# yang-0201/MAF-YOLO

Hardware: AMD Instinct MI355X
Metric: images/sec MAF-YOLO-n 640x640 bs=32 infer (Model.forward + non_max_suppression) (higher is better)
Workload: dtype f16

## Files before the change

include/mafyolo_hip.h:

```cpp
#ifndef MAFYOLO_HIP_H
#define MAFYOLO_HIP_H

#include <stdint.h>

#ifdef __cplusplus
extern "C" {
#endif

typedef void* maf_stream_t;

enum { MAF_F16 = 0, MAF_F32 = 1, MAF_U8 = 2 };
enum { MAF_ACT_NONE = 0, MAF_ACT_RELU = 1, MAF_ACT_SILU = 2, MAF_ACT_SIGMOID = 3 };
enum { MAF_SRC_DIRECT = 0,
       MAF_SRC_UP2 = 1,
       MAF_SRC_POOL2 = 2,
       MAF_SRC_SUB2 = 3,
       MAF_SRC_PAIRS = 4 };
enum { MAF_OP_STEM = 0,
       MAF_OP_CONV1X1 = 1,
       MAF_OP_CONV3X3S2 = 2,
       MAF_OP_DWCONV = 3,
       MAF_OP_SPPF_POOL = 4,
       MAF_OP_DECODE = 5,
       MAF_OP_BOTTLENECK = 6,
       MAF_OP_CONV1DW = 7,
       MAF_OP_HEADTAIL = 8,
       MAF_OP_STEM2 = 9,
       MAF_OP_CONV3X3S2_DGRAD = 10 };
enum { MAF_CONV_GENERIC = 1,
       MAF_CONV_LDS = 2,
       MAF_CONV_STREAM = 3,
       MAF_CONV_SPLITK = 4,
       MAF_CONV_STREAM_LDS = 5,
       MAF_CONV3_LDS = 6,
       MAF_CONV3_WREG = 7,
       MAF_CONV_DMA = 8 };
enum { MAF_DW_MFMA = -1, MAF_DW_DOT2 = -2, MAF_DW_PAIRS = -4 };
enum { MAF_DW_P2_STAGED = 128 };
#define MAF_DW_TILE_ROWS(tile_k) ((tile_k) >> 8)
enum { MAF_E_ARG = -1, MAF_E_UNSUPPORTED = -2, MAF_E_HIP = -3 };

typedef struct {
    const void* ptr;
    int32_t C;
    int32_t stride;
    int32_t coff;
    int32_t mode;
} maf_src_t;

typedef struct {
    int32_t kind, dtype, in_dtype, act;
    int32_t B, H, W;
    int32_t Hin, Win;
    int32_t Cin, Cout, ksize;
    int32_t nsrc;
    maf_src_t src[4];
    void* out;
    int32_t out_stride, out_coff;
    int32_t out_f32;
    int32_t tile_p, tile_c;
    int32_t tile_k;
    const void* w;
    const float* bias;
    const void* reg[3];
    int32_t lvl_h[3], lvl_w[3];
    int32_t reg_stride, nc, reg_max;
    float lvl_stride[3];
    const void* aux[4];
    int32_t lane;
    int32_t n_wait;
    int32_t wait[8];
    int32_t out_pairs;
    int32_t reserved0;
} maf_op_t;

const char* maf_last_error(void);
int maf_version(void);
int maf_op_size(void);
int64_t maf_bottleneck_record_bytes(int32_t k, int32_t Cin, int32_t Cout);
int64_t maf_bottleneck_tail_record_bytes(int32_t c, int32_t nsrc, int32_t C3);
int maf_bottleneck_tail_supported(int32_t k, int32_t c, int32_t nsrc, int32_t C3);
int64_t maf_conv1dw_record_bytes(int32_t k, int32_t Cin);
int64_t maf_head_tail_record_bytes(int32_t C);
int64_t maf_stem2_record_bytes(int32_t C0, int32_t C1, int32_t C3);
int64_t maf_conv3s2_lds_record_bytes(int32_t Cin, int32_t Cout);
int64_t maf_mprep_lds_record_bytes(int32_t Cin, int32_t Cout, int32_t C1);
int64_t maf_mprep_wreg_record_bytes(int32_t Cin, int32_t Cout, int32_t C1);
int64_t maf_conv3s2_wreg_record_bytes(int32_t Cin, int32_t Cout);
int maf_conv1x1_stats_supported(int32_t ksteps, int32_t tile_c);

int maf_op_launch(const maf_op_t* op, maf_stream_t stream);

typedef struct maf_engine maf_engine_t;
int maf_engine_create(const maf_op_t* ops, int32_t n_ops, maf_engine_t** out);
int maf_engine_num_ops(const maf_engine_t* e);
int maf_engine_run(maf_engine_t* e, const void* image, void* pred, maf_stream_t stream);
int maf_engine_run_filtered(maf_engine_t* e, const void* image, void* pred, maf_stream_t stream, void* nms_workspace, double conf_thres);
int maf_engine_run_graph(maf_engine_t* e, const void* image, void* pred, maf_stream_t stream);
int maf_engine_run_timed(maf_engine_t* e, const void* image, void* pred, maf_stream_t stream, float* ms_per_op);
void maf_engine_destroy(maf_engine_t* e);

enum { MAF_NMS_FLOAT_THRESHOLD = 1, MAF_NMS_SINGLE_LAUNCH = 2, MAF_NMS_PRECOLLECTED = 4, MAF_NMS_MATRIX = 8 };
enum { MAF_NMS_CNT_STRIDE = 64 };
int64_t maf_nms_workspace_bytes(int32_t B, int32_t N, int32_t nc);
int maf_nms(const float* pred, int32_t B, int32_t N, int32_t nc, double conf_thres, double iou_thres,
            const int32_t* classes, int32_t n_classes, int32_t agnostic, int32_t multi_label,
            int32_t max_det, void* workspace, int64_t workspace_bytes,
            float* out_rows, int64_t* out_idx, int32_t* out_count, maf_stream_t stream);
int maf_nms_ex(const float* pred, int32_t B, int32_t N, int32_t nc, double conf_thres, double iou_thres,
               const int32_t* classes, int32_t n_classes, int32_t agnostic, int32_t multi_label,
               int32_t max_det, void* workspace, int64_t workspace_bytes,
               float* out_rows, int64_t* out_idx, int32_t* out_count, int32_t flags, maf_stream_t stream);

int64_t maf_pack_w1x1_bytes(int32_t Cout, int32_t Cin, int32_t transpose, int32_t dtype, int32_t tile_c);
int maf_pack_w1x1(const float* w, int32_t Cout, int32_t Cin, int32_t transpose, int32_t dtype, int32_t tile_c, void* out, maf_stream_t stream);
int maf_pack_dw(const float* w, int32_t C, int32_t k, int32_t flip, int32_t dtype, void* out, maf_stream_t stream);
int maf_tal_targets(const float* targets, int32_t T, int32_t B, float img_size, float* gts, int32_t* gt_image, int32_t* offsets, maf_stream_t stream);
int maf_tal_assign(const void* pd_scores, int32_t score_dtype, const float* pd_bboxes, const float* anchor_points, const float* gts,
                   const int32_t* gt_image, const int32_t* offsets, int32_t T, int32_t B, int32_t A, int32_t nc, int32_t topk,
                   float alpha, float beta, float eps, int32_t n_levels, const int32_t* level_hw, const float* level_stride, float cell_offset,
                   int32_t* cand_scratch, int32_t* out_gt, float* out_norm, maf_stream_t stream);
int maf_atss_assign(const float* pd_bboxes, const float* anchor_points, const float* gts, const int32_t* gt_image, const int32_t* offsets,
                    int32_t T, int32_t B, int32_t A, int32_t topk, int32_t n_levels, const int32_t* level_hw, const float* level_stride,
                    float cell_offset, float cell_size, int32_t* cand_scratch, int32_t* out_gt, float* out_norm, maf_stream_t stream);
int64_t maf_loss_partial_rows(int32_t B, int32_t A, int32_t nc);
int maf_loss_decode(const void* pred_distri, int32_t dtype, const float* anchor_points, const float* anchor_strides, int32_t B, int32_t A,
                    int32_t reg_max, float* out_boxes, maf_stream_t stream);
int maf_loss_terms(const void* pred_scores, const void* pred_distri, int32_t dtype, const float* anchor_points, const float* anchor_strides,
                   const float* gts, const int32_t* assigned_gt, const float* norm, int32_t B, int32_t A, int32_t nc, int32_t reg_max,
                   float w_cls, float w_iou, float w_dfl, float* partials, float* out, const float* upstream, void* grad_scores,
                   void* grad_distri, maf_stream_t stream);

int maf_bn_forward(const void* x, int32_t x_stride, int32_t M, int32_t C, int32_t dtype, const float* gamma, const float* beta,
                   float eps, float momentum, float* running_mean, float* running_var, int64_t* num_batches_tracked, int32_t act, void* y,
                   int32_t y_stride, float* save_mean, float* save_rstd, float* part, int32_t R, int32_t phase, const void* residual, int32_t res_stride,
                   maf_stream_t stream);
int maf_bn_backward(const void* x, int32_t x_stride, const void* dz, int32_t dz_stride, int32_t M, int32_t C, int32_t dtype,
                    const float* gamma, const float* beta, const float* save_mean, const float* save_rstd, int32_t act,
                    void* dx, int32_t dx_stride, float* dgamma, float* dbeta, float* part, int32_t R, int32_t phase,
                    const void* residual, int32_t res_stride, void* dres, int32_t dres_stride, maf_stream_t stream);
int maf_dw_branches_stats(const void* const* src, const int32_t* src_stride, void* const* dst, const int32_t* dst_stride, const void* const* w,
                          int32_t nb, int32_t k0, int32_t B, int32_t H, int32_t W, int32_t C, int32_t dtype, float* const* stats, int32_t replicas, maf_stream_t stream);
int maf_dw_branches(const void* const* src, const int32_t* src_stride, void* const* dst, const int32_t* dst_stride, const void* const* w,
                    int32_t nb, int32_t k0, int32_t B, int32_t H, int32_t W, int32_t C, int32_t dtype, int32_t dgrad, maf_stream_t stream);
int maf_bn_forward_ex(const void* x, int32_t x_stride, int32_t M, int32_t C, int32_t dtype, const float* gamma, const float* beta,
                      float eps, float momentum, float* running_mean, float* running_var, int64_t* num_batches_tracked, int32_t act, void* y,
                      int32_t y_stride, float* save_mean, float* save_rstd, float* part, int32_t R, int32_t phase, const void* residual, int32_t res_stride,
                      int32_t stats_ready, maf_stream_t stream);
int32_t maf_bn_replicas(int32_t C, int32_t R);
int maf_bn_stats(const void* x, int32_t x_stride, int32_t M, int32_t C, int32_t dtype, float* part, int32_t R, int32_t phase, maf_stream_t stream);
int maf_bn_sum_forward(const void* const* z, const int32_t* z_stride, int32_t nb, int32_t M, int32_t C, int32_t dtype,
                       const float* const* gamma, const float* const* beta, float eps, float momentum,
                       float* const* running_mean, float* const* running_var, int64_t* const* num_batches_tracked,
                       void* out, int32_t out_stride, float* const* save_mean, float* const* save_rstd,
                       float* const* part, int32_t R, const int32_t* phase, int32_t act, maf_stream_t stream);
int maf_bn_sum_forward_stats(const void* const* z, const int32_t* z_stride, int32_t nb, int32_t M, int32_t C, int32_t dtype,
                             const float* const* gamma, const float* const* beta, float eps, float momentum,
                             float* const* running_mean, float* const* running_var, int64_t* const* num_batches_tracked,
                             void* out, int32_t out_stride, float* const* save_mean, float* const* save_rstd,
                             float* const* part, int32_t R, const int32_t* phase, int32_t act,
                             float* next_part, int32_t next_R, int32_t next_phase, maf_stream_t stream);
int maf_bn_sum_backward(const void* dy, int32_t dy_stride, const void* const* z, const int32_t* z_stride, int32_t nb, int32_t M, int32_t C, int32_t dtype,
                        const float* const* gamma, const float* const* beta, const float* const* save_mean, const float* const* save_rstd,
                        void* const* dz, const int32_t* dz_stride, float* const* dgamma, float* const* dbeta, int32_t accumulate_affine,
                        float* bpart, int32_t R, int32_t phase, int32_t act, maf_stream_t stream);
int maf_bn_backward_acc(const void* x, int32_t x_stride, const void* dz, int32_t dz_stride, int32_t M, int32_t C, int32_t dtype,
                        const float* gamma, const float* beta, const float* save_mean, const float* save_rstd, int32_t act,
                        void* dx, int32_t dx_stride, float* dgamma, float* dbeta, float* part, int32_t R, int32_t phase,
                        const void* residual, int32_t res_stride, void* dres, int32_t dres_stride, int32_t accumulate_affine, maf_stream_t stream);
int maf_set_deterministic(int32_t on);
int maf_conv1x1_wgrad(const void* x, int32_t x_stride, const void* dy, int32_t dy_stride, int32_t M, int32_t Cin, int32_t Cout,
                      int32_t dtype, float* dw, maf_stream_t stream);
int maf_conv_wgrad(const void* x, int32_t x_stride, const void* dy, int32_t dy_stride, int32_t B, int32_t Ho, int32_t Wo, int32_t Hs, int32_t Ws,
                   int32_t Cin, int32_t Cout, int32_t ksize, int32_t stride, int32_t dtype, float* dw, maf_stream_t stream);
int maf_dw_wgrad(const void* x, int32_t x_stride, const void* dy, int32_t dy_stride, int32_t B, int32_t H, int32_t W, int32_t C,
                 int32_t k, int32_t dtype, float* dw, int32_t replicas, maf_stream_t stream);
int maf_stem_train(const void* img, int32_t img_stride, int32_t B, int32_t Hin, int32_t Win, const float* w3, const float* w1, int32_t Cout,
                   void* z3, void* z1, maf_stream_t stream);
int maf_image_to_nhwc8(const void* x, int32_t dtype, int32_t B, int32_t H, int32_t W, void* out, maf_stream_t stream);
int maf_dw_wgrad31(const void* x, int32_t x_stride, const void* dya, int32_t dya_stride, const void* dyb, int32_t dyb_stride, const void* dy1, int32_t dy1_stride,
                   int32_t B, int32_t H, int32_t W, int32_t C, int32_t dtype, float* dwa, float* dwb, float* dw1, int32_t replicas, maf_stream_t stream);

int maf_grad_fold(const float* src, int32_t taps, int32_t Cout_p, int32_t Cin_p, float* dst, int32_t Cout, int32_t Cin, int32_t accumulate,
                  maf_stream_t stream);
int maf_add_sub2(const void* src, int32_t src_stride, void* dst, int32_t dst_stride, int32_t B, int32_t Ho, int32_t Wo, int32_t C, int32_t dtype, maf_stream_t stream);
int maf_colsum(const void* x, int32_t x_stride, int64_t M, int32_t C, int32_t dtype, float* out, maf_stream_t stream);

int maf_zero(void* p, int64_t bytes, maf_stream_t stream);

int maf_maxpool_forward(const void* x, int32_t x_stride, int32_t B, int32_t H, int32_t W, int32_t C, int32_t k, int32_t stride, int32_t pad,
                        int32_t dtype, void* y, int32_t y_stride, uint8_t* idx, maf_stream_t stream);
int maf_maxpool_backward(const void* dy, int32_t dy_stride, const uint8_t* idx, int32_t B, int32_t H, int32_t W, int32_t C, int32_t k,
                         int32_t stride, int32_t pad, int32_t dtype, void* dx, int32_t dx_stride, maf_stream_t stream);
int maf_upsample2x_forward(const void* x, int32_t x_stride, int32_t B, int32_t H, int32_t W, int32_t C, int32_t dtype, void* y, int32_t y_stride, maf_stream_t stream);
int maf_upsample2x_backward(const void* dy, int32_t dy_stride, int32_t B, int32_t H, int32_t W, int32_t C, int32_t dtype, void* dx, int32_t dx_stride, maf_stream_t stream);

typedef struct maf_pack_desc {
    const void* src; void* dst;
    int64_t total;
    int32_t kind, dtype;
    int32_t Cout, Cin, taps, transpose;
    int32_t CT, steps, Kp, flip;
    int32_t block0, reserved;
} maf_pack_desc_t;
int maf_pack_batch(const maf_pack_desc_t* descs_dev, int32_t n, int32_t nblocks, maf_stream_t stream);
int32_t maf_pack_desc_size(void);

typedef struct maf_ema_desc {
    void* dst; const void* src;
    int64_t total;
    int32_t block0, reserved;
} maf_ema_desc_t;
int maf_ema_update(const maf_ema_desc_t* descs_dev, int32_t n, int32_t nblocks, float decay, float one_minus_decay, maf_stream_t stream);
int32_t maf_ema_desc_size(void);

#define MAF_SGD_MAX_GROUPS 8
typedef struct maf_sgd_desc {
    void* param; void* grad; void* buf;
    int64_t total;
    int32_t block0, group;
} maf_sgd_desc_t;
int maf_sgd_update(const maf_sgd_desc_t* descs_dev, int32_t n, int32_t nblocks, int32_t ngroups, const double* lr, const double* weight_decay, const double* momentum,
                   const int32_t* nesterov, const float* found_inf, const float* grad_scale, maf_stream_t stream);
int32_t maf_sgd_desc_size(void);

typedef struct maf_range_desc {
    const void* ptr;
    int64_t total;
    int32_t block0, reserved;
} maf_range_desc_t;
int maf_nonfinite_check(const maf_range_desc_t* descs_dev, int32_t n, int32_t nblocks, float* found_inf, maf_stream_t stream);
int32_t maf_range_desc_size(void);


int maf_nhwc_sum(const void* const* src, const int32_t* src_stride, int32_t n, void* dst, int32_t dst_stride, int64_t M, int32_t C, int32_t dtype,
                 int32_t accumulate, maf_stream_t stream);
int maf_detect_join(const void* const* cls, const int32_t* cls_stride, const void* const* reg, const int32_t* reg_stride, const int32_t* level_pixels,
                    int32_t n_levels, int32_t B, int32_t nc, int32_t nreg, int32_t dtype, void* cls_out, void* reg_out, maf_stream_t stream);
int maf_detect_join_backward(const void* d_cls, const void* d_reg, const void* cls_out, const int32_t* level_pixels, int32_t n_levels, int32_t B, int32_t nc,
                             int32_t nreg, int32_t dtype, void* const* dcls, const int32_t* dcls_stride, void* const* dreg, const int32_t* dreg_stride,
                             int32_t nc_pad, int32_t nreg_pad, maf_stream_t stream);
int maf_stream_fork(maf_stream_t main, maf_stream_t side);
int maf_stream_join(maf_stream_t main, maf_stream_t side);

int maf_stream_create_masked(const uint32_t* mask_words, int32_t n_words, maf_stream_t* out);
int maf_stream_destroy(maf_stream_t s);

#define MAF_TAPE_MAX_ARGS 28
#define MAF_TAPE_FORK (-1)
typedef struct maf_tape_rec {
    int32_t fn, stream;
    uint64_t a[MAF_TAPE_MAX_ARGS];
} maf_tape_rec_t;
typedef struct maf_tape_toggle {
    void* addr; uint64_t mask; int32_t width, reserved;
} maf_tape_toggle_t;
int32_t maf_tape_fn_id(const char* name);
int32_t maf_tape_fn_nargs(int32_t fn);
int32_t maf_tape_rec_size(void);
int maf_tape_run(const maf_tape_rec_t* recs, int32_t first, int32_t last, const maf_stream_t* streams, int32_t n_streams, int32_t* failed_at);
int maf_tape_toggle(const maf_tape_toggle_t* t, int32_t n);

int maf_coco_rows(const float* rows, const int32_t* count, int32_t B, int32_t max_det, const float* img_params,
                  const int32_t* ids, int32_t n_ids, float* out, int32_t* out_total, maf_stream_t stream);

#define MAF_LETTERBOX_KARG_MAX 64
typedef struct {
    const uint8_t* ptr; int64_t pitch;
    int32_t h, w;
    int32_t new_h, new_w, top, left;
} maf_letterbox_image_t;
int64_t maf_letterbox_lds_bytes(const maf_letterbox_image_t* imgs, int32_t B, int32_t W);
int maf_letterbox(const maf_letterbox_image_t* imgs, const maf_letterbox_image_t* imgs_dev, int32_t B, int32_t H, int32_t W,
                  const uint8_t* color, int32_t bgr, uint8_t* out, maf_stream_t stream);

int maf_rescale_boxes(float* rows, const int32_t* count, int32_t B, int32_t max_det, int32_t row_stride, const float* params,
                      int32_t do_round, maf_stream_t stream);

typedef struct {
    const uint8_t* src; int64_t src_pitch;
    int32_t h, w;
    uint8_t* dst;
    int32_t new_h, new_w;
} maf_augment_frame_t;
int maf_augment_resize(const maf_augment_frame_t* frames, const maf_augment_frame_t* frames_dev, int32_t n, maf_stream_t stream);

#define MAF_AUGMENT_MAX_TILES 4
typedef struct {
    const uint8_t* ptr; int64_t pitch;
    int32_t h, w;
    int32_t x0, y0, x1, y1;
    int32_t dx, dy;
} maf_augment_tile_t;
typedef struct {
    double minv[2][6];
    double r;
    int32_t ntiles[2];
    int32_t hsv, flipud, fliplr, reserved;
    maf_augment_tile_t tile[2][MAF_AUGMENT_MAX_TILES];
    uint8_t lut[3][256];
} maf_augment_sample_t;
int32_t maf_augment_sample_size(void);
int maf_mosaic_affine(const maf_augment_sample_t* samples, const maf_augment_sample_t* samples_dev, int32_t B, int32_t S, uint8_t* out,
                      maf_stream_t stream);

#define MAF_AREA_FAST2 0
#define MAF_AREA_FASTN 1
#define MAF_AREA_GENERAL 2
typedef struct {
    const uint8_t* src; int64_t src_pitch;
    int32_t h, w;
    uint8_t* dst;
    int32_t new_h, new_w;
    int32_t path;
    int32_t iscale_x, iscale_y;
    float inv_area;
    int32_t x_start, x_pairs;
    int32_t y_start, y_pairs;
} maf_area_frame_t;
int maf_area_struct_sizes(int32_t* frame_size);
int maf_resize_area(const maf_area_frame_t* frames, const maf_area_frame_t* frames_dev, int32_t n, const void* tables, const void* tables_dev,
                    int64_t table_words, maf_stream_t stream);

#define MAF_PR_MAX_DET 1024
#define MAF_PR_MAX_LABELS 1024
#define MAF_PR_MAX_CLASSES 1024
#define MAF_PR_HEADER 16
#define MAF_PR_LABELS_XYXY 1
#define MAF_PR_CONFUSION 2
#define MAF_PR_ERR_CLASS 1
#define MAF_PR_ERR_LABELS 2
#define MAF_PR_ERR_CAPACITY 4
int64_t maf_pr_state_ints(int32_t nc);
int64_t maf_pr_out_doubles(int32_t nc, int32_t niou);
int64_t maf_pr_workspace_bytes(int32_t nc, int32_t niou, int64_t capacity);
int maf_pr_match(const float* rows, const int32_t* count, int32_t B, int32_t max_det, const float* targets, int32_t n_targets,
                 const float* img_params, int32_t H, int32_t W, const float* iouv, int32_t niou, int32_t nc, int32_t flags,
                 float cm_conf, float cm_iou, const int64_t* offs_in, int64_t* offs_out, int64_t* keys, uint16_t* masks,
                 int64_t capacity, int32_t* state, maf_stream_t stream);
int maf_pr_curves(const int64_t* sorted_keys, const int64_t* perm, const uint16_t* masks, int64_t capacity, const int32_t* state,
                  int32_t nc, int32_t niou, void* workspace, int64_t workspace_bytes, double* out, maf_stream_t stream);

#define MAF_COCO_T 10
#define MAF_COCO_R 101
#define MAF_COCO_A 4
#define MAF_COCO_M 3
#define MAF_COCO_MAX_DETS 100
#define MAF_COCO_MAX_GT 256
#define MAF_COCO_GT_CROWD 1
#define MAF_COCO_GT_IDNZ 2
int maf_coco_append(const float* packed, const int32_t* total, int64_t rows, const int32_t* img_index, int32_t B, const int32_t* cat_lut,
                    int32_t n_lut, int32_t* det_img, int32_t* det_cat, double* det_box, double* det_score, maf_stream_t stream);
int maf_coco_match(const double* gt_box, const double* gt_area, const uint8_t* gt_flags, const int64_t* gt_off, const int64_t* cell_keys,
                   const int64_t* order, const double* det_box, int64_t n, const uint8_t* img_sel, const int32_t* cat_map, int32_t I, int32_t K,
                   const double* iou_thrs, const double* area_rng, int32_t* rank, uint64_t* mbits, uint64_t* ibits, int32_t* npig,
                   maf_stream_t stream);
int maf_coco_accumulate(const int64_t* cat_keys, const int32_t* rank, const uint64_t* mbits, const uint64_t* ibits, const double* score, int64_t n,
                        const int32_t* npig, const uint8_t* img_sel, const int32_t* cat_of, int32_t I, int32_t K, int32_t Kp,
                        const double* rec_thrs, const int32_t* max_dets, double* precision, double* recall, double* scores, maf_stream_t stream);

#define MAF_JPEG_GROUP 64
#define MAF_JPEG_SCAN_PAD 64
#define MAF_JPEG_HUFF_TABLE_BYTES 1424
#define MAF_JPEG_ST_BAD_CODE 1
#define MAF_JPEG_ST_BAD_INDEX 2
#define MAF_JPEG_ST_SHORT_SCAN 4
#define MAF_JPEG_ST_REFINE_PAST_SE 8
#define MAF_JPEG_STAGE_ENTROPY 1
#define MAF_JPEG_STAGE_IDCT 2
#define MAF_JPEG_STAGE_COLOR 4
#define MAF_JPEG_STAGE_ALL 7
typedef struct {
    int32_t n_images, n_lanes, n_tabsets;
    int32_t group;
    int64_t images_off, lanes_off, huff_off, quant_off, scan_off;
    int64_t scan_bytes;
    int64_t total_bytes;
    int64_t coef_elems, plane_bytes, out_bytes;
    int32_t n_scans, n_slanes, n_rounds;
    int32_t sgroup;
    int64_t scans_off, slanes_off, rounds_off;
} maf_jpeg_header_t;
typedef struct {
    int64_t coef_off;
    int64_t plane_off;
    int64_t out_off;
    int32_t w, h, ncomp;
    int32_t hs, vs;
    int32_t mcux, mcuy;
    int32_t quant;
    int32_t dc_tab[3], ac_tab[3];
    int32_t reserved[2];
} maf_jpeg_image_t;
typedef struct {
    int64_t begin, end;
    int32_t image;
    int32_t first_mcu, n_mcu;
    int32_t tabset;
} maf_jpeg_lane_t;
typedef struct {
    int32_t image;
    int32_t round;
    int32_t ncomp;
    int32_t comp[3];
    int32_t ss, se, ah, al;
    int32_t dc_tab[3];
    int32_t ac_tab;
    int32_t bw, bh;
} maf_jpeg_scan_t;
int maf_jpeg_struct_sizes(int32_t* header_image_lane);
int maf_jpeg_progressive_struct_sizes(int32_t* scan);
int maf_jpeg_decode(const void* blob_host, const void* blob_dev, int16_t* coef, uint8_t* planes, uint8_t* out, int32_t* status,
                    int32_t stages, maf_stream_t stream);

int maf_nms_debug(uint64_t* host8);

int maf_timer_create(void** timer);
int maf_timer_start(void* timer, maf_stream_t stream);
int maf_timer_stop(void* timer, maf_stream_t stream);
int maf_timer_elapsed_ms(void* timer, float* ms);
void maf_timer_destroy(void* timer);

#ifdef __cplusplus
}
#endif
#endif
```

maf-yolo_amd/config.py:

```python
import os

SWITCHES = {
    "dw_stage":          ("MAF_DW_STAGE", True, "tuner: offer dwconv_p2's staged-store form (tile_k + 128) as a candidate"),
    "fuse_mprep":        ("MAF_FUSE_MPREP", True, "MPRep's two branches as one launch where the kernel exists (tuned plans)"),
    "fuse_tail":         ("MAF_FUSE_TAIL", 1, "what Model.fuse_tail = 'auto' means: 0 off, 1 blocks of one bottleneck (default), 3 every instantiation (s / m opt-in)"),
    "split_cat":         ("MAF_SPLIT_CAT", True, "RepHDW behind the fused stem: one dense tensor per concat slot"),
    "mprep_wreg_min":    ("MAF_MPREP_WREG_MIN", 65536, "output pixels from which MPRep takes the register-weight 3x3 kernel"),
    "head_tail_256_max": ("MAF_HEAD_TAIL_256_MAX", 16384, "largest level (B * H * W pixels) whose 256-channel head runs as the fused tail (weights streamed through LDS per 16-pixel unit)"),
    "nms_single_max_batch": ("MAF_NMS_SINGLE_MAX_BATCH", 0, "largest batch the single-launch NMS kernel serves (0: never — the seven-launch path is faster, DESIGN.md 8)"),
    "nms_matrix":        ("MAF_NMS_MATRIX", "auto", "all-pairs NMS: 1 = suppression matrix + row scan, 0 = kept-list scan, auto = kept-list under other work (async), matrix alone up to 32 images"),
    "step_tape":         ("MAF_STEP_TAPE", True, "replay the recorded launch lists of a train step (tape.py) once a batch shape has been seen three times"),
    "stage_native":      ("MAF_STAGE_NATIVE", True, "step tape: the image batch into the static NHWC8 input by one native pass"),
    "train_lanes":       ("MAF_TRAIN_LANES", 2, "lanes (extra streams) a recorded step may put independent branches on"),
    "wgrad_stream":      ("MAF_WGRAD_STREAM", True, "weight gradients on a side stream"),
    "bn_affine_direct":  ("MAF_BN_AFFINE_DIRECT", True, "BatchNorm dgamma / dbeta straight into the exchange's bucket slices"),
    "conv_bn_stats":     ("MAF_CONV_BN_STATS", True, "BatchNorm statistics out of the 1x1 conv's epilogue"),
    "train_tune":        ("MAF_TRAIN_TUNE", True, "time the conv tile variants per shape on first use"),
    "train_tune3":       ("MAF_TRAIN_TUNE3", True, "... the 3x3 stride-2 launches too"),
    "stem_train":        ("MAF_STEM_TRAIN", True, "the image's two RepVGG convs as one direct-conv launch"),
    "dw_wgrad31":        ("MAF_DW_WGRAD31", True, "the 3x3 (+3x3) + 1x1 depth-wise branches' weight gradients as one launch"),
    "dw_branches":       ("MAF_DW_BRANCHES", True, "one launch per direction for the branches of a DilatedReparamBlock"),
    "dw_branch_stats":   ("MAF_DW_BRANCH_STATS", True, "the branches' BatchNorm statistics out of the depth-wise kernel's epilogue"),
    "cat_free":          ("MAF_CAT_FREE", True, "concat nodes without a copy (producers store into their slot)"),
    "bn_sum":            ("MAF_BN_SUM", True, "the branch BatchNorms of a DilatedReparamBlock as one apply pass per direction"),
    "bn_sum_stats":      ("MAF_BN_SUM_STATS", True, "that pass accumulates the statistics of the BatchNorm behind it"),
    "ema_native":        ("MAF_EMA_NATIVE", True, "ModelEMA.update as one launch"),
    "sgd_native":        ("MAF_SGD_NATIVE", True, "the SGD step as one launch"),
    "inf_check_native":  ("MAF_INF_CHECK_NATIVE", True, "GradScaler's inf check as one launch"),
    "exchange_debug":    ("MAF_EXCHANGE_DEBUG", False, "GradExchange keeps the Python stack of every gradient arrival"),
    "hip_lib":           ("MAF_HIP_LIB", "", "path of another build of libmafyolo_hip.so (make prof / ko / var); empty: the in-tree product library"),
}


LIBRARY_SWEEP_HOOKS = {
    "MAF_WGRAD_GX / MAF_WGRAD_R / MAF_WGRAD_TAP_PER_WG": "csrc/wgrad.hip: grid width / replica count / one tap per workgroup of the conv weight gradient (tools/wgrad_sweep.py)",
    "MAF_WGRAD3_GX / MAF_WGRAD3_R / MAF_WGRAD3_PATCH": "csrc/wgrad.hip: the same for the 3x3 patch kernel",
    "MAF_DWWG / MAF_DWWG31 / MAF_DWWG_MFMA / MAF_DWMF_WG": "csrc/train_ops.hip, dw_wgrad_mfma.hip: tiles of the depth-wise weight gradients (tools/dw_wgrad_sweep.py, dw_wgrad31_sweep.py, dw_wgrad_ab.py)",
    "MAF_DWB_TILE / MAF_DWB_TILE_DGRAD": "csrc/dw_branches.hip: tile of the merged depth-wise branches (tools/dwb_sweep.py)",
    "MAF_DGRAD3_ALL_TAPS": "csrc/conv_mfma.hip: A/B of the 3x3 data gradient's tap split",
}


class Config:
    def __init__(self, environ=None):
        environ = os.environ if environ is None else environ
        for attr, (env, default, _) in SWITCHES.items():
            raw = environ.get(env)
            if raw is None:
                val = default
            elif isinstance(default, bool):
                val = raw != "0"
            elif isinstance(default, int):
                val = int(raw)
            else:
                val = raw
            setattr(self, attr, val)

    def overridden(self):
        return {a: getattr(self, a) for a, (_, d, _m) in SWITCHES.items() if getattr(self, a) != d}

    def table(self):
        rows = ["%-22s %-26s %-10s %s" % ("attribute", "environment", "value", "meaning")]
        for a, (env, d, meaning) in SWITCHES.items():
            v = getattr(self, a)
            rows.append("%-22s %-26s %-10s %s%s" % (a, env, repr(v), meaning, "" if v == d else "   [default %r]" % (d,)))
        return "\n".join(rows)


cfg = Config()

if __name__ == "__main__":
    print(cfg.table())
```

maf-yolo_amd/csrc/capi.hip:

```cpp
#include <vector>
#include <string>
#include "maf_common.h"

static thread_local std::string g_err;

void maf_set_error(const std::string& msg) { g_err = msg; }

int maf_check_hip(hipError_t e, const char* what) {
    if (e == hipSuccess) return 0;
    g_err = std::string(what) + ": " + hipGetErrorString(e);
    return MAF_E_HIP;
}

extern "C" const char* maf_last_error(void) { return g_err.c_str(); }
extern "C" int maf_zero(void* p, int64_t bytes, maf_stream_t stream) {
    MAF_REQUIRE(p && bytes >= 0, "maf_zero: bad arguments");
    return maf_check_hip(hipMemsetAsync(p, 0, (size_t)bytes, static_cast<hipStream_t>(stream)), "maf_zero");
}

extern "C" int maf_version(void) { return 200; }
extern "C" int maf_op_size(void) { return (int)sizeof(maf_op_t); }

extern "C" int maf_op_launch(const maf_op_t* op, maf_stream_t stream) {
    if (!op) { maf_set_error("maf_op_launch: null op"); return MAF_E_ARG; }
    hipStream_t s = static_cast<hipStream_t>(stream);
    switch (op->kind) {
        case MAF_OP_STEM: return maf_launch_stem(op, s);
        case MAF_OP_CONV1X1:
        case MAF_OP_CONV3X3S2:
        case MAF_OP_CONV3X3S2_DGRAD: return maf_launch_conv_mfma(op, s);
        case MAF_OP_DWCONV: return maf_launch_dwconv(op, s);
        case MAF_OP_SPPF_POOL: return maf_launch_sppf_pool(op, s);
        case MAF_OP_DECODE: return maf_launch_decode(op, s);
        case MAF_OP_BOTTLENECK: return maf_launch_bottleneck(op, s);
        case MAF_OP_CONV1DW: return maf_launch_conv1dw(op, s);
        case MAF_OP_HEADTAIL: return maf_launch_head_tail(op, s);
        case MAF_OP_STEM2: return maf_launch_stem2(op, s);
        default: maf_set_error("maf_op_launch: unknown op kind"); return MAF_E_UNSUPPORTED;
    }
}

constexpr int kMaxLanes = 8;

struct maf_engine {
    std::vector<maf_op_t> ops;
    hipGraph_t graph = nullptr;
    hipGraphExec_t exec = nullptr;
    const void* g_image = nullptr;
    void* g_pred = nullptr;
    int n_lanes = 1;
    hipStream_t side[kMaxLanes] = {};
    std::vector<hipEvent_t> done;
    std::vector<char> signal;
    hipEvent_t fork = nullptr, join[kMaxLanes] = {};
    bool lanes_ready = false;
};

static int engine_prepare_lanes(maf_engine* e) {
    if (e->lanes_ready) return 0;
    const size_t n = e->ops.size();
    e->signal.assign(n, 0);
    e->done.assign(n, nullptr);
    e->n_lanes = 1;
    for (size_t i = 0; i < n; ++i) {
        const maf_op_t& o = e->ops[i];
        if (o.lane < 0 || o.lane >= kMaxLanes) { maf_set_error("engine: op lane out of range (0..7)"); return MAF_E_ARG; }
        if (o.n_wait < 0 || o.n_wait > 8) { maf_set_error("engine: n_wait out of range (0..8)"); return MAF_E_ARG; }
        if (o.lane + 1 > e->n_lanes) e->n_lanes = o.lane + 1;
        for (int k = 0; k < o.n_wait; ++k) {
            if (o.wait[k] < 0 || (size_t)o.wait[k] >= i) { maf_set_error("engine: an op may only wait for earlier ops"); return MAF_E_ARG; }
            e->signal[o.wait[k]] = 1;
        }
    }
    int rc = 0;
    for (int l = 1; l < e->n_lanes && !rc; ++l) {
        rc = maf_check_hip(hipStreamCreateWithFlags(&e->side[l], hipStreamNonBlocking), "hipStreamCreate");
        if (!rc) rc = maf_check_hip(hipEventCreateWithFlags(&e->join[l], hipEventDisableTiming), "hipEventCreate");
    }
    if (!rc && e->n_lanes > 1) rc = maf_check_hip(hipEventCreateWithFlags(&e->fork, hipEventDisableTiming), "hipEventCreate");
    for (size_t i = 0; i < n && !rc; ++i)
        if (e->signal[i]) rc = maf_check_hip(hipEventCreateWithFlags(&e->done[i], hipEventDisableTiming), "hipEventCreate");
    if (!rc) e->lanes_ready = true;
    return rc;
}

extern "C" int maf_engine_create(const maf_op_t* ops, int32_t n_ops, maf_engine_t** out) {
    if (!ops || n_ops <= 0 || !out) { maf_set_error("maf_engine_create: bad arguments"); return MAF_E_ARG; }
    maf_engine* e = new maf_engine();
    e->ops.assign(ops, ops + n_ops);
    *out = e;
    return 0;
}

extern "C" int maf_engine_num_ops(const maf_engine_t* e) { return e ? (int)e->ops.size() : 0; }

static long long nms_cap_pow2(long long v) { long long p = 1; while (p < v) p <<= 1; return p; }

static int engine_launch_all(maf_engine* e, const void* image, void* pred, hipStream_t s, void* cand_ws = nullptr, float cand_conf = 0.f, bool one_stream = false) {
    int rc = engine_prepare_lanes(e);
    if (rc) return rc;
    const bool multi = e->n_lanes > 1 && !one_stream;
    int* cand_cnt = nullptr; unsigned long long* cand_keys = nullptr; long long cand_cap = 0;
    if (cand_ws) {
        int B = 0, A = 0, nc = 0, tails = 0;
        for (const maf_op_t& o : e->ops) {
            if (o.kind == MAF_OP_DECODE) { maf_set_error("maf_engine_run_filtered: a level of this plan is decoded by MAF_OP_DECODE (no fused tail)"); return MAF_E_UNSUPPORTED; }
            if (o.kind == MAF_OP_HEADTAIL) { B = o.B; A = o.Win; nc = o.nc; ++tails; }
        }
        if (!tails) { maf_set_error("maf_engine_run_filtered: the plan has no MAF_OP_HEADTAIL"); return MAF_E_UNSUPPORTED; }
        cand_cnt = static_cast<int*>(cand_ws);
        cand_keys = reinterpret_cast<unsigned long long*>(static_cast<char*>(cand_ws) + 256 + (long long)B * MAF_NMS_CNT_STRIDE * 4);
        cand_cap = nms_cap_pow2((long long)A * nc);
        rc = maf_check_hip(hipMemsetAsync(cand_cnt, 0, (size_t)B * MAF_NMS_CNT_STRIDE * 4, s), "candidate counter reset");
        if (rc) return rc;
    }
    if (multi) {
        rc = maf_check_hip(hipEventRecord(e->fork, s), "hipEventRecord(fork)");
        for (int l = 1; l < e->n_lanes && !rc; ++l) rc = maf_check_hip(hipStreamWaitEvent(e->side[l], e->fork, 0), "hipStreamWaitEvent(fork)");
        if (rc) return rc;
    }
    for (size_t i = 0; i < e->ops.size(); ++i) {
        maf_op_t op = e->ops[i];
        if ((op.kind == MAF_OP_STEM || op.kind == MAF_OP_STEM2) && image) op.src[0].ptr = image;
        if ((op.kind == MAF_OP_DECODE || op.kind == MAF_OP_HEADTAIL) && pred) op.out = pred;
        if (op.kind == MAF_OP_HEADTAIL && cand_ws) { op.aux[1] = cand_cnt; op.aux[2] = cand_keys; op.lvl_h[0] = (int32_t)cand_cap; op.lvl_stride[1] = cand_conf; }
        hipStream_t st = (op.lane == 0 || one_stream) ? s : e->side[op.lane];
        for (int k = 0; k < op.n_wait && !one_stream && !rc; ++k) rc = maf_check_hip(hipStreamWaitEvent(st, e->done[op.wait[k]], 0), "hipStreamWaitEvent");
        if (!rc) rc = maf_op_launch(&op, st);
        if (!rc && !one_stream && e->signal[i]) rc = maf_check_hip(hipEventRecord(e->done[i], st), "hipEventRecord");
        if (rc) {
            g_err = "op " + std::to_string(i) + ": " + g_err;
            return rc;
        }
    }
    if (multi) {
        for (int l = 1; l < e->n_lanes && !rc; ++l) {
            rc = maf_check_hip(hipEventRecord(e->join[l], e->side[l]), "hipEventRecord(join)");
            if (!rc) rc = maf_check_hip(hipStreamWaitEvent(s, e->join[l], 0), "hipStreamWaitEvent(join)");
        }
    }
    return rc;
}

extern "C" int maf_engine_run(maf_engine_t* e, const void* image, void* pred, maf_stream_t stream) {
    if (!e) { maf_set_error("maf_engine_run: null engine"); return MAF_E_ARG; }
    return engine_launch_all(e, image, pred, static_cast<hipStream_t>(stream));
}

extern "C" int maf_engine_run_filtered(maf_engine_t* e, const void* image, void* pred, maf_stream_t stream, void* nms_workspace, double conf_thres) {
    if (!e || !nms_workspace || !pred) { maf_set_error("maf_engine_run_filtered: null argument"); return MAF_E_ARG; }
    if (!(conf_thres >= 0.0 && conf_thres < 1.0)) { maf_set_error("maf_engine_run_filtered: conf_thres must be in [0, 1)"); return MAF_E_ARG; }
    return engine_launch_all(e, image, pred, static_cast<hipStream_t>(stream), nms_workspace, (float)conf_thres);
}

extern "C" int maf_engine_run_graph(maf_engine_t* e, const void* image, void* pred, maf_stream_t stream) {
    if (!e) { maf_set_error("maf_engine_run_graph: null engine"); return MAF_E_ARG; }
    hipStream_t s = static_cast<hipStream_t>(stream);
    if (e->exec && (e->g_image != image || e->g_pred != pred)) {
        (void)hipGraphExecDestroy(e->exec); (void)hipGraphDestroy(e->graph);
        e->exec = nullptr; e->graph = nullptr;
    }
    if (!e->exec) {
        int rc = maf_check_hip(hipStreamBeginCapture(s, hipStreamCaptureModeThreadLocal), "hipStreamBeginCapture");
        if (rc) return rc;
        rc = engine_launch_all(e, image, pred, s, nullptr, 0.f, true);
        hipError_t ce = hipStreamEndCapture(s, &e->graph);
        if (rc) return rc;
        rc = maf_check_hip(ce, "hipStreamEndCapture");
        if (rc) return rc;
        rc = maf_check_hip(hipGraphInstantiate(&e->exec, e->graph, nullptr, nullptr, 0), "hipGraphInstantiate");
        if (rc) return rc;
        e->g_image = image; e->g_pred = pred;
    }
    return maf_check_hip(hipGraphLaunch(e->exec, s), "hipGraphLaunch");
}

extern "C" int maf_engine_run_timed(maf_engine_t* e, const void* image, void* pred, maf_stream_t stream, float* ms_per_op) {
    if (!e || !ms_per_op) { maf_set_error("maf_engine_run_timed: bad arguments"); return MAF_E_ARG; }
    hipStream_t s = static_cast<hipStream_t>(stream);
    const size_t n = e->ops.size();
    std::vector<hipEvent_t> ev(n + 1);
    int rc = 0;
    for (size_t i = 0; i <= n && !rc; ++i) rc = maf_check_hip(hipEventCreate(&ev[i]), "hipEventCreate");
    if (!rc) rc = maf_check_hip(hipEventRecord(ev[0], s), "hipEventRecord");
    for (size_t i = 0; i < n && !rc; ++i) {
        maf_op_t op = e->ops[i];
        if ((op.kind == MAF_OP_STEM || op.kind == MAF_OP_STEM2) && image) op.src[0].ptr = image;
        if ((op.kind == MAF_OP_DECODE || op.kind == MAF_OP_HEADTAIL) && pred) op.out = pred;
        rc = maf_op_launch(&op, s);
        if (!rc) rc = maf_check_hip(hipEventRecord(ev[i + 1], s), "hipEventRecord");
    }
    if (!rc) rc = maf_check_hip(hipEventSynchronize(ev[n]), "hipEventSynchronize");
    for (size_t i = 0; i < n && !rc; ++i) rc = maf_check_hip(hipEventElapsedTime(&ms_per_op[i], ev[i], ev[i + 1]), "hipEventElapsedTime");
    for (size_t i = 0; i <= n; ++i) (void)hipEventDestroy(ev[i]);
    return rc;
}

extern "C" void maf_engine_destroy(maf_engine_t* e) {
    if (!e) return;
    if (e->exec) (void)hipGraphExecDestroy(e->exec);
    if (e->graph) (void)hipGraphDestroy(e->graph);
    for (int l = 1; l < kMaxLanes; ++l) {
        if (e->join[l]) (void)hipEventDestroy(e->join[l]);
        if (e->side[l]) (void)hipStreamDestroy(e->side[l]);
    }
    if (e->fork) (void)hipEventDestroy(e->fork);
    for (hipEvent_t ev : e->done) if (ev) (void)hipEventDestroy(ev);
    delete e;
}

struct maf_timer { hipEvent_t a, b; };

extern "C" int maf_timer_create(void** t) {
    if (!t) return MAF_E_ARG;
    maf_timer* m = new maf_timer();
    int rc = maf_check_hip(hipEventCreate(&m->a), "hipEventCreate");
    if (!rc) rc = maf_check_hip(hipEventCreate(&m->b), "hipEventCreate");
    if (rc) { delete m; return rc; }
    *t = m;
    return 0;
}
extern "C" int maf_timer_start(void* t, maf_stream_t s) { return maf_check_hip(hipEventRecord(static_cast<maf_timer*>(t)->a, static_cast<hipStream_t>(s)), "hipEventRecord"); }
extern "C" int maf_timer_stop(void* t, maf_stream_t s) { return maf_check_hip(hipEventRecord(static_cast<maf_timer*>(t)->b, static_cast<hipStream_t>(s)), "hipEventRecord"); }
extern "C" int maf_timer_elapsed_ms(void* t, float* ms) {
    maf_timer* m = static_cast<maf_timer*>(t);
    int rc = maf_check_hip(hipEventSynchronize(m->b), "hipEventSynchronize");
    if (rc) return rc;
    return maf_check_hip(hipEventElapsedTime(ms, m->a, m->b), "hipEventElapsedTime");
}
extern "C" void maf_timer_destroy(void* t) {
    maf_timer* m = static_cast<maf_timer*>(t);
    if (!m) return;
    (void)hipEventDestroy(m->a); (void)hipEventDestroy(m->b);
    delete m;
}

extern "C" int maf_stream_create_masked(const uint32_t* mask_words, int32_t n_words, maf_stream_t* out) {
    if (!mask_words || n_words <= 0 || !out) { maf_set_error("stream_create_masked: bad arguments"); return MAF_E_ARG; }
    hipStream_t s = nullptr;
    if (int rc = maf_check_hip(hipExtStreamCreateWithCUMask(&s, (uint32_t)n_words, mask_words), "hipExtStreamCreateWithCUMask")) return rc;
    *out = s;
    return 0;
}
extern "C" int maf_stream_destroy(maf_stream_t s) { return maf_check_hip(hipStreamDestroy(static_cast<hipStream_t>(s)), "hipStreamDestroy"); }
```

maf-yolo_amd/csrc/maf_common.h:

```cpp
#pragma once
#include <hip/hip_runtime.h>
#include <stdint.h>
#include <string>
#include "../../include/mafyolo_hip.h"

typedef _Float16 half_t;
typedef _Float16 half8_t __attribute__((ext_vector_type(8)));
typedef _Float16 half4_t __attribute__((ext_vector_type(4)));
typedef _Float16 half2_t __attribute__((ext_vector_type(2)));
typedef float f32x4_t __attribute__((ext_vector_type(4)));
typedef float f32x2_t __attribute__((ext_vector_type(2)));
typedef uint32_t u32x4_t __attribute__((ext_vector_type(4)));
typedef uint32_t u32x2_t __attribute__((ext_vector_type(2)));

void maf_set_error(const std::string& msg);
int maf_check_hip(hipError_t e, const char* what);

#define MAF_REQUIRE(cond, msg)                          \
    do {                                                \
        if (!(cond)) {                                  \
            maf_set_error(std::string(msg));            \
            return MAF_E_ARG;                           \
        }                                               \
    } while (0)

int maf_launch_conv_mfma(const maf_op_t* op, hipStream_t s);
int maf_launch_stem(const maf_op_t* op, hipStream_t s);
int maf_launch_dwconv(const maf_op_t* op, hipStream_t s);
int maf_launch_sppf_pool(const maf_op_t* op, hipStream_t s);
int maf_launch_decode(const maf_op_t* op, hipStream_t s);
int maf_launch_bottleneck(const maf_op_t* op, hipStream_t s);
int maf_launch_conv1dw(const maf_op_t* op, hipStream_t s);
int maf_launch_head_tail(const maf_op_t* op, hipStream_t s);
int maf_launch_stem2(const maf_op_t* op, hipStream_t s);
int maf_launch_conv3s2_lds(const maf_op_t* op, hipStream_t s);
int maf_launch_conv3s2_wreg(const maf_op_t* op, hipStream_t s);
int maf_dw_wgrad_mfma(const void* x, int x_stride, const void* dy, int dy_stride, int B, int H, int W, int C, int k, float* dw, int replicas, hipStream_t s);

template <int ACT>
__device__ __forceinline__ float maf_act(float x) {
    if (ACT == MAF_ACT_RELU) return x > 0.f ? x : 0.f;
    if (ACT == MAF_ACT_SILU) return x * __builtin_amdgcn_rcpf(1.f + __expf(-x));
    if (ACT == MAF_ACT_SIGMOID) return __builtin_amdgcn_rcpf(1.f + __expf(-x));
    return x;
}
__device__ __forceinline__ float maf_act_rt(float x, int act) {
    switch (act) {
        case MAF_ACT_RELU: return x > 0.f ? x : 0.f;
        case MAF_ACT_SILU: return x * __builtin_amdgcn_rcpf(1.f + __expf(-x));
        case MAF_ACT_SIGMOID: return __builtin_amdgcn_rcpf(1.f + __expf(-x));
        default: return x;
    }
}

static inline int maf_cdiv(int a, int b) { return (a + b - 1) / b; }
```

maf-yolo_amd/engine.py:

```python
import ctypes as C
import os

import torch

from .config import cfg
from . import lib, pack
from .layers import (RepVGGBlock, RepHDW, MPRep, SPPF, ConvWrapper, Head_DepthUni)

_ESIZE = {lib.F16: 2, lib.F32: 4}


from .conv_variants import stream_lds_ok
from .tuner import _TUNE_CACHE, choose_fusion, save_tune_cache, load_tune_cache, p2_wave_bytes
from . import tuner as _tuner, plan_report as _report

_TORCH_DT = {lib.F16: torch.float16, lib.F32: torch.float32}


def _raw(*ts):
    return tuple(t.detach().float().cpu() for t in ts)


class Buf:

    def __init__(self, off, H, W, stride, esize, C=None):
        self.off, self.H, self.W, self.stride, self.esize = off, H, W, stride, esize
        self.C = stride if C is None else C


class Seg:
    def __init__(self, buf, C, coff=0, mode=lib.SRC_DIRECT):
        self.buf, self.C, self.coff, self.mode = buf, C, coff, mode


class TV:

    def __init__(self, segs, H, W):
        self.segs, self.H, self.W = segs, H, W

    @property
    def C(self):
        return sum(s.C for s in self.segs)


class Plan:
    def __init__(self, model, B, Hin, Win, dtype, in_dtype, device, fuse=None, fuse_head=None, fuse_tail=None):
        assert Hin % 32 == 0 and Win % 32 == 0, "image sides must be multiples of 32 (stride of P5)"
        self.B, self.Hin, self.Win, self.dtype, self.in_dtype, self.device = B, Hin, Win, dtype, in_dtype, device
        self.es = _ESIZE[dtype]
        self._arena_size = 0
        self._wblobs = []
        self._wsize = 0
        self._ops = []
        self.nc = model.nc
        self.reg_max = model.detect.reg_max
        self.strides = [float(s) for s in model.detect.stride.tolist()]
        self.fuse = getattr(model, "fuse_bottlenecks", "auto") if fuse is None else fuse
        fh = getattr(model, "fuse_head", "auto") if fuse_head is None else fuse_head
        self.fuse_head = bool(fh) and dtype == lib.F16 and model.nc == 80 and model.detect.reg_max == 16
        fs = getattr(model, "fuse_stem", True)
        self.fuse_stem = (2 if fs is True else int(fs or 0)) if dtype == lib.F16 else 0
        self._stem2 = self._stem3 = None
        fm = getattr(model, "fuse_mprep", "auto")
        self.fuse_mprep = (bool(getattr(model, "autotune", False)) if fm == "auto" else bool(fm)) and cfg.fuse_mprep
        ft = getattr(model, "fuse_tail", "auto") if fuse_tail is None else fuse_tail
        env_ft = str(cfg.fuse_tail)
        deep = 3 if env_ft == "3" else 1
        self.fuse_tail = (deep if ft == "auto" else 3 if ft else 0) if (env_ft != "0" and dtype == lib.F16) else 0
        self.split_cat = bool(getattr(model, "split_cat", cfg.split_cat))
        self.lanes = getattr(model, "multi_stream", False)
        if isinstance(self.lanes, bool):
            self.lanes = 2 if self.lanes else 0
        with torch.no_grad():
            self._build(model)
        self._finalize()

    def _fuse_mode(self, name, k, c):
        if self.dtype != lib.F16 or c % 8:
            return 0
        f = self.fuse
        if isinstance(f, dict):
            m = f.get(name, 0)
        elif isinstance(f, (set, frozenset, list, tuple)):
            m = 1 if name in f else 0
        elif f == "auto":
            m = 1 if k <= 5 else 0
        elif f is True:
            m = 1
        else:
            m = int(f or 0)
        if m == 1 and c > 64:
            m = 2 if (f is True or isinstance(f, dict)) else 0
        if m == 2 and c > 512:
            m = 0
        return m

    def _alloc(self, H, W, C, esize=None):
        esize = esize or self.es
        off = self._arena_size
        self._arena_size += (self.B * H * W * C * esize + 255) // 256 * 256
        return Buf(off, H, W, C, esize)

    def _wput(self, t):
        t = t.contiguous()
        off = self._wsize
        self._wsize += (t.numel() * t.element_size() + 255) // 256 * 256
        self._wblobs.append((off, t))
        return off

    def _conv1x1(self, name, w, b, src, out, out_coff, act, out_f32=False):
        cout = w.shape[0]
        M = self.B * src.H * src.W
        pt, ct = pack.tile_for(cout, M)
        srcC = [s.C for s in src.segs]
        assert len(src.segs) <= 4, "%s: more than 4 concat sources" % name
        self._ops.append(dict(kind=lib.OP_CONV1X1, name=name, act=act, H=src.H, W=src.W, Cin=src.C, Cout=cout, raw=(w.detach().float().cpu(), b.detach().float().cpu(), srcC),
                              segs=src.segs, out=out, out_coff=out_coff, out_f32=int(out_f32), pt=pt, ct=ct,
                              w=self._wput(pack.pack_conv1x1(w, srcC, ct, self.dtype)), b=self._wput(pack.pack_bias(b, ct))))

    def _conv3x3s2(self, name, w, b, src, out, out_coff, act, twin=None):
        assert len(src.segs) == 1 and src.segs[0].mode == lib.SRC_DIRECT, "%s: 3x3 s2 conv needs a materialised input" % name
        cout = w.shape[0]
        H, W = src.H // 2, src.W // 2
        pt, ct = pack.tile_for(cout, self.B * H * W)
        rec = dict(kind=lib.OP_CONV3X3S2, name=name, act=act, H=H, W=W, Hin=src.H, Win=src.W, Cin=src.C, Cout=cout, raw=(w.detach().float().cpu(), b.detach().float().cpu(), None),
                   segs=src.segs, out=out, out_coff=out_coff, out_f32=0, pt=pt, ct=ct,
                   w=self._wput(pack.pack_conv3x3(w, ct, self.dtype)), b=self._wput(pack.pack_bias(b, ct)))
        if twin is not None:
            name2, w2, b2, src2, out2 = twin
            s1, s2 = src.segs[0], src2.segs[0]
            assert len(src2.segs) == 1 and s2.mode == lib.SRC_DIRECT and (s2.buf.stride, s2.coff, s2.C) == (s1.buf.stride, s1.coff, s1.C) and w2.shape == w.shape \
                and (out2.stride, out2.H, out2.W) == (out.stride, out.H, out.W) and out_coff == 0
            rec.update(name=name + "+" + name2, twin=dict(seg=s2, out=out2, raw=(w2.detach().float().cpu(), b2.detach().float().cpu()),
                                                          w=self._wput(pack.pack_conv3x3(w2, ct, self.dtype)), b=self._wput(pack.pack_bias(b2, ct))))
        self._ops.append(rec)

    def _dw(self, name, w, b, src, out, act):
        assert len(src.segs) == 1 and src.segs[0].mode == lib.SRC_DIRECT
        self._ops.append(dict(kind=lib.OP_DWCONV, name=name, act=act, H=src.H, W=src.W, Cin=src.C, Cout=src.C, ksize=w.shape[-1], raw=(w.detach().float().cpu(), b.detach().float().cpu()),
                              segs=src.segs, out=out, out_coff=0, w=self._wput(pack.pack_dw(w, self.dtype)),
                              b=self._wput(b.float().cpu()),
                              aux=[self._wput(pack.pack_dw_toeplitz(w)), self._wput(pack.pack_dw_pairs(w)) if src.C % 8 == 0 else None] if self.dtype == lib.F16 else []))

    def _build(self, model):
        B = self.B
        y = []
        self.head_bufs = []
        self.fuse_head = self.fuse_head and not self.lanes
        n_side = n_head = 0
        twins_done = {}
        for node, m in zip(model.nodes, model.backbone):
            if node.i > 0:
                self._tag(tag_from, tag_node, tag_lane, tag_after)
            tag_from, tag_node, tag_lane, tag_after = len(self._ops), node.i, 0, None
            p = "backbone.%d" % node.i
            srcs = [y[j] for j in node.sources()] if node.i > 0 else None
            x = srcs[0] if srcs else None
            if self.lanes >= 2 and node.kind == "cw" and node.sources()[0] != node.i - 1:
                tag_lane = 1 + (n_side % 2)
                n_side += 1
            if self.lanes and node.kind == "head":
                tag_lane = (3, 5, 0)[n_head % 3]
                tag_after = node.sources()[0]
                n_head += 1
            if node.kind == "repvgg" and node.i == 1 and self._stem2 is not None:
                w0, b0, c0 = self._stem2
                w, b = m.fused()
                nxt = model.nodes[2] if len(model.nodes) > 2 else None
                m2 = model.backbone[2] if nxt is not None else None
                if (nxt is not None and nxt.kind == "rephdw" and list(nxt.sources()) == [1] and not any(1 in n_.sources() for n_ in model.nodes[3:])
                        and m2.conv1.fused()[0].shape[0] == node.cout and self.fuse_stem >= 2):
                    self._stem3 = (w0, b0, c0, w, b, node.cout)
                    y.append(TV([], self.Hin // 4, self.Win // 4))
                    continue
                out = self._alloc(self.Hin // 4, self.Win // 4, node.cout)
                self._ops.append(dict(kind=lib.OP_STEM2, name="backbone.0+1", act=lib.ACT_RELU, H=out.H, W=out.W, Hin=self.Hin, Win=self.Win,
                                      Cin=3, Cout=node.cout, ksize=c0, segs=[], out=out, out_coff=0, raw=_raw(w0, b0, w, b),
                                      w=self._wput(pack.pack_stem2(w0, b0, w, b)), b=0))
                y.append(TV([Seg(out, node.cout)], out.H, out.W))
            elif node.kind == "repvgg":
                w, b = m.fused()
                if node.i == 0 and self.fuse_stem and len(model.nodes) > 1 and model.nodes[1].kind == "repvgg" and list(model.nodes[1].sources()) == [0] \
                        and (node.cout, model.nodes[1].cout) in ((24, 48), (32, 64), (48, 96)) and not any(0 in n_.sources() for n_ in model.nodes[2:]):
                    self._stem2 = (w, b, node.cout)
                    y.append(None)
                    continue
                if node.i == 0:
                    H, W = self.Hin // 2, self.Win // 2
                    out = self._alloc(H, W, node.cout)
                    self._ops.append(dict(kind=lib.OP_STEM, name=p, act=lib.ACT_RELU, H=H, W=W, Hin=self.Hin, Win=self.Win,
                                          Cin=3, Cout=node.cout, segs=[], out=out, out_coff=0,
                                          w=self._wput(pack.pack_stem(w)), b=self._wput(b.float().cpu())))
                else:
                    out = self._alloc(x.H // 2, x.W // 2, node.cout)
                    self._conv3x3s2(p, w, b, x, out, 0, lib.ACT_RELU)
                y.append(TV([Seg(out, node.cout)], out.H, out.W))
            elif node.kind == "rephdw":
                c_, depth = m.c_, len(m.m)
                split = (node.i == 2 and self._stem3 is not None and self.split_cat and depth + 2 <= 4 and c_ % 8 == 0
                         and (c_ * self.es) % 128 != 0 and m.conv1.fused()[0].shape[0] == 2 * c_)
                kl = m.m[-1].conv2.dwconv.kernel_size
                tail = (depth <= self.fuse_tail and self._fuse_mode("%s.m.%d" % (p, depth - 1), kl, c_) == 1 and 2 <= depth + 1 <= 3
                        and m.conv2.fused()[0].shape[1] == (depth + 2) * c_
                        and lib.load().maf_bottleneck_tail_supported(kl, c_, depth + 1, node.cout) == 1)
                nslot = depth + 1 if tail else depth + 2
                if split:
                    slot = [(self._alloc(x.H, x.W, c_), 0) for _ in range(nslot)]
                else:
                    cat = self._alloc(x.H, x.W, c_ * nslot)
                    slot = [(cat, j * c_) for j in range(nslot)]
                if node.i == 2 and self._stem3 is not None:
                    w0, b0, c0, w1_, b1_, c1 = self._stem3
                    w3, b3 = m.conv1.fused()
                    self._ops.append(dict(kind=lib.OP_STEM2, name="backbone.0+1+2.conv1", act=lib.ACT_RELU, H=x.H, W=x.W, Hin=self.Hin, Win=self.Win,
                                          Cin=3, Cout=c1, ksize=c0, c3=w3.shape[0], segs=[], out=slot[0][0], out_coff=0, raw=_raw(w0, b0, w1_, b1_, w3, b3),
                                          w=self._wput(pack.pack_stem2(w0, b0, w1_, b1_, w3, b3)), b=0))
                    if split:
                        self._ops[-1]["out2"] = slot[1][0]
                else:
                    self._conv1x1(p + ".conv1", *m.conv1.fused(), x, cat, 0, lib.ACT_SILU)
                for d, blk in enumerate(m.m):
                    mid = blk.conv1.conv.out_channels
                    q = "%s.m.%d" % (p, d)
                    mode = self._fuse_mode(q, blk.conv2.dwconv.kernel_size, c_)
                    (ib, ic) = slot[d + 1]
                    if tail and d == depth - 1:
                        rec, b2p, nmb, ct2 = pack.pack_bottleneck(*blk.conv1.fused(), *blk.conv2.fused(), *blk.one_conv.fused())
                        w3, b3 = m.conv2.fused()
                        out = self._alloc(x.H, x.W, node.cout)
                        self._ops.append(dict(kind=lib.OP_BOTTLENECK, name=q + "+conv2", act=lib.ACT_SILU, H=x.H, W=x.W, Cin=c_, Cout=c_, ksize=kl, mid=mid,
                                              segs=[Seg(ib, c_, ic)] + [Seg(slot[j][0], c_, slot[j][1]) for j in range(depth)], out=out, out_coff=0, pt=16, ct=16, tk=nmb,
                                              tail_c3=node.cout, raw=_raw(*blk.conv1.fused(), *blk.conv2.fused(), *blk.one_conv.fused(), w3, b3),
                                              w=self._wput(rec), b=self._wput(b2p), aux=[self._wput(pack.pack_bottleneck_tail(w3, b3, c_, depth + 1))]))
                        continue
                    (ob, oc) = slot[d + 2]
                    if mode == 2:
                        rec, nmb = pack.pack_conv1dw(*blk.conv1.fused(), *blk.conv2.fused())
                        t2 = self._alloc(x.H, x.W, mid)
                        self._ops.append(dict(kind=lib.OP_CONV1DW, name=q + ".conv1dw", act=lib.ACT_SILU, H=x.H, W=x.W, Cin=c_, Cout=mid,
                                              ksize=blk.conv2.dwconv.kernel_size, segs=[Seg(ib, c_, ic)], out=t2, out_coff=0, raw=_raw(*blk.conv1.fused(), *blk.conv2.fused()), w=self._wput(rec),
                                              b=self._wput(torch.zeros(8))))
                        self._conv1x1(q + ".one_conv", *blk.one_conv.fused(), TV([Seg(t2, mid)], x.H, x.W), ob, oc, lib.ACT_SILU)
                        continue
                    if mode == 1:
                        rec, b2p, nmb, ct2 = pack.pack_bottleneck(*blk.conv1.fused(), *blk.conv2.fused(), *blk.one_conv.fused())
                        k = blk.conv2.dwconv.kernel_size
                        th, tw = 16, 16
                        self._ops.append(dict(kind=lib.OP_BOTTLENECK, name=q, act=lib.ACT_SILU, H=x.H, W=x.W, Cin=c_, Cout=c_, ksize=k, mid=mid,
                                              segs=[Seg(ib, c_, ic)], out=ob, out_coff=oc, pt=th, ct=tw, tk=nmb, raw=_raw(*blk.conv1.fused(), *blk.conv2.fused(), *blk.one_conv.fused()),
                                              w=self._wput(rec), b=self._wput(b2p), aux=[]))
                        continue
                    t1, t2 = self._alloc(x.H, x.W, mid), self._alloc(x.H, x.W, mid)
                    self._conv1x1(q + ".conv1", *blk.conv1.fused(), TV([Seg(ib, c_, ic)], x.H, x.W), t1, 0, lib.ACT_SILU)
                    self._dw(q + ".conv2", *blk.conv2.fused(), TV([Seg(t1, mid)], x.H, x.W), t2, lib.ACT_SILU)
                    self._conv1x1(q + ".one_conv", *blk.one_conv.fused(), TV([Seg(t2, mid)], x.H, x.W), ob, oc, lib.ACT_SILU)
                if not tail:
                    out = self._alloc(x.H, x.W, node.cout)
                    cat_tv = TV([Seg(b_, c_, 0) for b_, _ in slot], x.H, x.W) if split else TV([Seg(cat, c_ * (depth + 2))], x.H, x.W)
                    self._conv1x1(p + ".conv2", *m.conv2.fused(), cat_tv, out, 0, lib.ACT_SILU)
                y.append(TV([Seg(out, node.cout)], x.H, x.W))
            elif node.kind == "mprep":
                assert len(x.segs) == 1 and x.segs[0].mode == lib.SRC_DIRECT
                c_ = node.cout // 2
                out = self._alloc(x.H // 2, x.W // 2, node.cout)
                s0 = x.segs[0]
                w1_, b1_ = m.conv1.fused()
                if self.fuse_mprep and self.dtype == lib.F16 and (x.C, c_, w1_.shape[0]) in ((48, 48, 48), (64, 64, 64)) and x.H % 2 == 0 and x.W % 2 == 0 \
                        and self.B * (x.H // 2) * (x.W // 2) >= 65536:
                    w2_, b2_ = m.conv2.fused()
                    self._ops.append(dict(kind=lib.OP_CONV3X3S2, name=p + ".conv1+conv2", act=lib.ACT_RELU, H=x.H // 2, W=x.W // 2, Hin=x.H, Win=x.W, Cin=x.C, Cout=c_,
                                          raw=(w2_.detach().float().cpu(), b2_.detach().float().cpu(), None), pool1=(w1_.detach().float().cpu(), b1_.detach().float().cpu()),
                                          segs=x.segs, out=out, out_coff=c_, out_f32=0, pt=4, ct=4, w=self._wput(pack.pack_mprep_lds(w2_, b2_, w1_, b1_)), b=0))
                    y.append(TV([Seg(out, node.cout)], out.H, out.W))
                    continue
                if self.fuse_mprep and self.dtype == lib.F16 and (x.C, c_, w1_.shape[0]) == (96, 96, 96) and x.H % 2 == 0 and x.W % 2 == 0 \
                        and self.B * (x.H // 2) * (x.W // 2) >= cfg.mprep_wreg_min:
                    w2_, b2_ = m.conv2.fused()
                    self._ops.append(dict(kind=lib.OP_CONV3X3S2, name=p + ".conv1+conv2", act=lib.ACT_RELU, H=x.H // 2, W=x.W // 2, Hin=x.H, Win=x.W, Cin=x.C, Cout=c_,
                                          raw=(w2_.detach().float().cpu(), b2_.detach().float().cpu(), None), pool1=(w1_.detach().float().cpu(), b1_.detach().float().cpu()), pool1_tk=lib.CONV3_WREG,
                                          segs=x.segs, out=out, out_coff=c_, out_f32=0, pt=2, ct=8, w=self._wput(pack.pack_mprep_wreg(w2_, b2_, w1_, b1_)), b=0))
                    y.append(TV([Seg(out, node.cout)], out.H, out.W))
                    continue
                pooled = TV([Seg(s0.buf, s0.C, s0.coff, lib.SRC_POOL2)], x.H // 2, x.W // 2)
                self._conv1x1(p + ".conv1", *m.conv1.fused(), pooled, out, 0, lib.ACT_SILU)
                self._conv3x3s2(p + ".conv2", *m.conv2.fused(), x, out, c_, lib.ACT_RELU)
                y.append(TV([Seg(out, node.cout)], out.H, out.W))
            elif node.kind == "sppf":
                c_ = m.cv1.conv.out_channels
                cat = self._alloc(x.H, x.W, 4 * c_)
                self._conv1x1(p + ".cv1", *m.cv1.fused(), x, cat, 0, lib.ACT_SILU)
                self._ops.append(dict(kind=lib.OP_SPPF_POOL, name=p + ".m", act=0, H=x.H, W=x.W, Cin=c_, Cout=3 * c_,
                                      segs=[Seg(cat, c_, 0)], out=cat, out_coff=c_, raw=()))
                out = self._alloc(x.H, x.W, node.cout)
                self._conv1x1(p + ".cv2", *m.cv2.fused(), TV([Seg(cat, 4 * c_)], x.H, x.W), out, 0, lib.ACT_SILU)
                y.append(TV([Seg(out, node.cout)], x.H, x.W))
            elif node.kind == "cw":
                if node.i in twins_done:
                    y.append(twins_done.pop(node.i))
                    continue
                out = self._alloc(x.H // 2, x.W // 2, node.cout)
                twin = None
                nxt = model.nodes[node.i + 1] if node.i + 1 < len(model.nodes) else None
                if getattr(model, "twin_convs", True) and not self.lanes and nxt is not None and nxt.kind == "cw" and (nxt.cin, nxt.cout) == (node.cin, node.cout) \
                        and node.i not in nxt.sources() and all(j < node.i for j in nxt.sources()):
                    x2 = y[nxt.sources()[0]]
                    if (x2.H, x2.W) == (x.H, x.W) and len(x2.segs) == 1 and len(x.segs) == 1 and x2.segs[0].mode == x.segs[0].mode == lib.SRC_DIRECT \
                            and (x2.segs[0].buf.stride, x2.segs[0].coff) == (x.segs[0].buf.stride, x.segs[0].coff):
                        out2 = self._alloc(x.H // 2, x.W // 2, nxt.cout)
                        twin = ("backbone.%d.block" % nxt.i, *model.backbone[nxt.i].block.fused(), x2, out2)
                        twins_done[nxt.i] = TV([Seg(out2, nxt.cout)], out2.H, out2.W)
                self._conv3x3s2(p + ".block", *m.block.fused(), x, out, 0, lib.ACT_SILU, twin=twin)
                y.append(TV([Seg(out, node.cout)], out.H, out.W))
            elif node.kind == "concat":
                H, W = srcs[0].H, srcs[0].W
                segs = []
                for s in srcs:
                    assert (s.H, s.W) == (H, W), "concat of different grids at node %d" % node.i
                    segs += s.segs
                y.append(TV(segs, H, W))
            elif node.kind == "up":
                assert all(s.mode == lib.SRC_DIRECT for s in x.segs), "upsample of a non-materialised tensor"
                y.append(TV([Seg(s.buf, s.C, s.coff, lib.SRC_UP2) for s in x.segs], x.H * 2, x.W * 2))
            elif node.kind == "head":
                c = node.cout
                t = self._alloc(x.H, x.W, c)
                self._conv1x1(p + ".stem", *m.stem.fused(), x, t, 0, lib.ACT_SILU)
                tv = TV([Seg(t, c)], x.H, x.W)
                if self.fuse_head and (c in (64, 128, 192) or (c == 256 and self.B * x.H * x.W <= cfg.head_tail_256_max)):
                    (wc, bc), (wr, brg) = m.cls_conv.fused(), m.reg_conv.fused()
                    assert wc.shape == wr.shape
                    u = self._alloc(x.H, x.W, 2 * c)
                    self._ops.append(dict(kind=lib.OP_DWCONV, name=p + ".cls_reg_conv", act=lib.ACT_NONE, H=x.H, W=x.W, Cin=c, Cout=2 * c, ksize=wc.shape[-1],
                                          raw=(torch.cat([wc, wr], 0).detach().float().cpu(), torch.cat([bc, brg], 0).detach().float().cpu()),
                                          segs=tv.segs, out=u, out_coff=0, w=self._wput(pack.pack_dw(torch.cat([wc, wr], 0), self.dtype)),
                                          b=self._wput(torch.cat([bc, brg], 0).float().cpu()),
                                          aux=[None, self._wput(pack.pack_dw_pairs(torch.cat([wc, wr], 0)))] if self.dtype == lib.F16 and c % 8 == 0 else []))
                    us = [(u, 0), (u, c)]
                    recs = [pack.pack_head_tail(*getattr(m, br + "_conv_s").fused(), pr.weight.detach(), pr.bias.detach())
                            for br, pr in (("cls", m.cls_pred), ("reg", m.reg_pred))]
                    raw = sum((_raw(*getattr(m, br + "_conv_s").fused(), pr.weight, pr.bias) for br, pr in (("cls", m.cls_pred), ("reg", m.reg_pred))), ())
                    self._ops.append(dict(kind=lib.OP_HEADTAIL, name=p + ".tail", act=0, H=x.H, W=x.W, Cin=c, Cout=5 + self.nc,
                                          segs=[Seg(us[0][0], c, us[0][1]), Seg(us[1][0], c, us[1][1])], out=None, out_coff=0, w=self._wput(recs[0]), b=0,
                                          aux=[self._wput(recs[1])], level=len(self.head_bufs), raw=raw))
                    self.head_bufs.append((t, None, None))
                    y.append(None)
                    continue
                outs = []
                u2 = None
                if self.dtype == lib.F16 and c % 8 == 0:
                    (wc, bc), (wr, brg) = m.cls_conv.fused(), m.reg_conv.fused()
                    if wc.shape == wr.shape:
                        u2 = self._alloc(x.H, x.W, 2 * c)
                        self._ops.append(dict(kind=lib.OP_DWCONV, name=p + ".cls_reg_conv", act=lib.ACT_NONE, H=x.H, W=x.W, Cin=c, Cout=2 * c, ksize=wc.shape[-1],
                                              raw=(torch.cat([wc, wr], 0).detach().float().cpu(), torch.cat([bc, brg], 0).detach().float().cpu()),
                                              segs=tv.segs, out=u2, out_coff=0, w=self._wput(pack.pack_dw(torch.cat([wc, wr], 0), self.dtype)),
                                              b=self._wput(torch.cat([bc, brg], 0).float().cpu()),
                                              aux=[None, self._wput(pack.pack_dw_pairs(torch.cat([wc, wr], 0)))]))
                for bi, (br, pred, act, cpred) in enumerate((("cls", m.cls_pred, lib.ACT_SIGMOID, self.nc), ("reg", m.reg_pred, lib.ACT_NONE, 4 * (self.reg_max + 1)))):
                    u, v = (None if u2 is not None else self._alloc(x.H, x.W, c)), self._alloc(x.H, x.W, c)
                    cpad = -(-cpred // 4) * 4
                    o = self._alloc(x.H, x.W, cpad, 4)
                    o.C = cpred
                    pw, pb = pred.weight.detach(), pred.bias.detach()
                    if cpad != cpred:
                        pw = torch.cat([pw, pw.new_zeros(cpad - cpred, *pw.shape[1:])], 0)
                        pb = torch.cat([pb, pb.new_zeros(cpad - cpred)], 0)
                    if u2 is None:
                        self._dw("%s.%s_conv" % (p, br), *getattr(m, br + "_conv").fused(), tv, u, lib.ACT_NONE)
                    self._conv1x1("%s.%s_conv_s" % (p, br), *getattr(m, br + "_conv_s").fused(),
                                  TV([Seg(u, c)] if u2 is None else [Seg(u2, c, bi * c)], x.H, x.W), v, 0, lib.ACT_SILU)
                    self._conv1x1("%s.%s_pred" % (p, br), pw, pb, TV([Seg(v, c)], x.H, x.W), o, 0, act, out_f32=True)
                    outs.append(o)
                self.head_bufs.append((t, outs[0], outs[1]))
                y.append(None)
            elif node.kind == "out":
                y.append(None)
            else:
                raise NotImplementedError(node.kind)
        self._tag(tag_from, tag_node, tag_lane, tag_after)
        assert len(self.head_bufs) == 3, "MAF-YOLO has three detection levels"
        self.A = sum(t.H * t.W for t, _, _ in self.head_bufs)
        fused = [c is None for _, c, _ in self.head_bufs]
        if not all(fused):
            self._ops.append(dict(kind=lib.OP_DECODE, name="detect", act=0, H=0, W=0, Cin=0, Cout=0, segs=[], out=None, out_coff=0))

    def _tag(self, first, node_i, lane, after):
        for r in self._ops[first:]:
            r["node"], r["after"] = node_i, after
            r["lane"] = lane
            if lane is not None and ".reg_" in r["name"] and self.lanes:
                r["lane"] = 7 if lane == 0 else lane + 1

    def _schedule(self):
        ops = self._ops
        if self.lanes:
            rest = [r for r in ops if r.get("after") is None]
            for src_node in sorted({r["after"] for r in ops if r.get("after") is not None}):
                grp = [r for r in ops if r.get("after") == src_node]
                anchor = max(i for i, q in enumerate(rest) if q.get("node") == src_node)
                rest[anchor + 1:anchor + 1] = grp
            ops = self._ops = rest
        writes = {}
        seen = {}
        last_on_lane = {}
        for i, r in enumerate(ops):
            lane = r.get("lane", 0) if self.lanes else 0
            r["lane"] = lane
            deps = set()
            if r["kind"] == lib.OP_DECODE:
                deps = set(last_on_lane.values())
            for s_ in r["segs"]:
                for lo, hi, j in writes.get(id(s_.buf), []):
                    if lo < s_.coff + s_.C and s_.coff < hi:
                        deps.add(j)
            latest = {}
            for j in deps:
                lj = ops[j]["lane"]
                if lj != lane and j > seen.setdefault(lane, {}).get(lj, -1):
                    latest[lj] = max(latest.get(lj, -1), j)
            for lj, j in latest.items():
                seen[lane][lj] = j
                for lk, jk in seen.get(lj, {}).items():
                    if lk != lane:
                        seen[lane][lk] = max(seen[lane].get(lk, -1), min(jk, j))
            r["wait"] = sorted(latest.values())
            assert len(r["wait"]) <= 8
            if r["out"] is not None:
                writes.setdefault(id(r["out"]), []).append((r["out_coff"], r["out_coff"] + r["Cout"], i))
            if "twin" in r:
                writes.setdefault(id(r["twin"]["out"]), []).append((0, r["Cout"], i))
            if "out2" in r:
                writes.setdefault(id(r["out2"]), []).append((0, r["Cout"], i))
            if "pool1" in r:
                writes.setdefault(id(r["out"]), []).append((0, r["pool1"][0].shape[0], i))
            last_on_lane[lane] = i

    def _finalize(self):
        self._schedule()
        dev = self.device
        self.arena = torch.empty(self._arena_size + 256, dtype=torch.uint8, device=dev)
        wcpu = torch.zeros(self._wsize + 256, dtype=torch.uint8)
        for off, t in self._wblobs:
            wcpu[off:off + t.numel() * t.element_size()] = t.reshape(-1).view(torch.uint8)
        self.weights = wcpu.to(dev)
        self._wblobs = None
        abase, wbase = self.arena.data_ptr(), self.weights.data_ptr()
        abase += (-abase) % 256
        self._abase = abase
        ops = (lib.MafOp * len(self._ops))()
        for o, r in zip(ops, self._ops):
            o.kind, o.dtype, o.in_dtype, o.act = r["kind"], self.dtype, self.in_dtype, r["act"]
            o.B, o.H, o.W = self.B, r["H"], r["W"]
            o.Hin, o.Win = r.get("Hin", 0), r.get("Win", 0)
            o.Cin, o.Cout, o.ksize = r["Cin"], r["Cout"], r.get("ksize", 0)
            o.nsrc = len(r["segs"])
            for i, s in enumerate(r["segs"]):
                o.src[i].ptr = abase + s.buf.off
                o.src[i].C, o.src[i].stride, o.src[i].coff, o.src[i].mode = s.C, s.buf.stride, s.coff, s.mode
            if r["out"] is not None:
                o.out = abase + r["out"].off
                o.out_stride = r["out"].stride
            o.out_coff = r["out_coff"]
            o.out_f32 = r.get("out_f32", 0)
            o.tile_p, o.tile_c, o.tile_k = r.get("pt", 0), r.get("ct", 0), (lib.CONV_GENERIC if r["kind"] in (lib.OP_CONV1X1, lib.OP_CONV3X3S2) else 0)
            o.ksize = r.get("ksize", 0)
            if "w" in r:
                o.w = wbase + r["w"]
                o.bias = wbase + r["b"]
            if r["kind"] == lib.OP_BOTTLENECK:
                o.tile_k = r["tk"]
                o.nc = r.get("tail_c3", 0)
            if "pool1" in r:
                o.tile_k, o.nc, o.reg_stride = r.get("pool1_tk", lib.CONV3_LDS), r["pool1"][0].shape[0], 0
            for k_, off in enumerate(r.get("aux", [])):
                if off is not None:
                    o.aux[k_] = wbase + off
            if "twin" in r:
                tw = r["twin"]
                o.aux[0], o.aux[1], o.aux[2], o.aux[3] = abase + tw["seg"].buf.off, wbase + tw["w"], wbase + tw["b"], abase + tw["out"].off
            o.lane, o.n_wait = r["lane"], len(r["wait"])
            for k_, j in enumerate(r["wait"]):
                o.wait[k_] = j
            if r["kind"] in (lib.OP_STEM, lib.OP_STEM2):
                o.nsrc = 1
                o.src[0].ptr = 0
                o.src[0].C = 3
            if r["kind"] == lib.OP_STEM2:
                o.nc = r.get("c3", 0)
                if "out2" in r:
                    o.aux[0] = abase + r["out2"].off
                    o.reg_stride = r["out2"].stride
            if r["kind"] == lib.OP_HEADTAIL:
                lvl = r["level"]
                o.Hin, o.Win = sum(t.H * t.W for t, _, _ in self.head_bufs[:lvl]), self.A
                o.lvl_stride[0], o.nc, o.reg_max = self.strides[lvl], self.nc, self.reg_max
            if r["kind"] == lib.OP_DECODE:
                o.nsrc = 3
                for l, (t, cls, reg) in enumerate(self.head_bufs):
                    if cls is not None:
                        o.src[l].ptr = abase + cls.off
                        o.src[l].stride = cls.stride
                        o.reg[l] = abase + reg.off
                    o.lvl_h[l], o.lvl_w[l], o.lvl_stride[l] = t.H, t.W, self.strides[l]
                o.reg_stride, o.nc, o.reg_max = -(-4 * (self.reg_max + 1) // 4) * 4, self.nc, self.reg_max
        self.ops = ops
        self.op_names = [r["name"] for r in self._ops]
        h = C.c_void_p()
        lib.check(lib.load().maf_engine_create(ops, len(self._ops), C.byref(h)))
        self._engine = h

    def _pairs_producer(self, i):
        o = self.ops[i]
        if i == 0 or self.dtype != lib.F16 or o.kind != lib.OP_DWCONV or not o.aux[1] or o.W % 2 or o.Cin % 8 or o.nsrc != 1 or o.src[0].mode not in (lib.SRC_DIRECT, lib.SRC_PAIRS):
            return None
        p = self.ops[i - 1]
        if p.kind != lib.OP_CONV1X1 or p.tile_k != lib.CONV_STREAM_LDS or p.out_f32 or "twin" in self._ops[i - 1] or p.out != o.src[0].ptr or p.out_coff or o.src[0].coff \
                or p.Cout != o.Cin or p.out_stride != o.src[0].stride or p.out_stride % 4 or (p.B, p.H, p.W) != (o.B, o.H, o.W):
            return None
        for j, q in enumerate(self.ops):
            if j in (i, i - 1):
                continue
            if q.out == p.out or any(q.src[k].ptr == p.out for k in range(q.nsrc)) or any(q.aux[k] == p.out for k in range(4)):
                return None
        return p

    def autotune(self, x, reps=5, verbose=False):
        return _tuner.autotune(self, x, reps, verbose)

    def run(self, x, graph=False):
        pred = torch.empty(self.B, self.A, 5 + self.nc, dtype=torch.float32, device=self.device)
        return self.run_into(x, pred, graph)

    def filter_ok(self):
        tails = [o for o in self.ops if o.kind == lib.OP_HEADTAIL]
        return len(tails) == 3 and not any(o.kind == lib.OP_DECODE for o in self.ops) and all((o.H * o.W) % 16 == 0 for o in tails)

    def run_into(self, x, pred, graph=False, cand=None):
        cur = torch.cuda.current_stream(self.device)
        if not graph:
            if cand is not None:
                lib.check(lib.load().maf_engine_run_filtered(self._engine, x.data_ptr(), pred.data_ptr(), cur.cuda_stream, cand[0].data_ptr(), float(cand[1])))
            else:
                lib.check(lib.load().maf_engine_run(self._engine, x.data_ptr(), pred.data_ptr(), cur.cuda_stream))
            return pred
        gs = getattr(self, "_gstream", None)
        if gs is None:
            gs = self._gstream = torch.cuda.Stream(self.device)
        gs.wait_stream(cur)
        lib.check(lib.load().maf_engine_run_graph(self._engine, x.data_ptr(), pred.data_ptr(), gs.cuda_stream))
        cur.wait_stream(gs)
        return pred

    def run_timed(self, x, pred):
        ms = (C.c_float * len(self.ops))()
        stream = torch.cuda.current_stream(self.device).cuda_stream
        lib.check(lib.load().maf_engine_run_timed(self._engine, x.data_ptr(), pred.data_ptr(), stream, ms))
        return list(ms)

    def kernel_name(self, idx):
        return _report.kernel_name(self, idx)

    def algorithmic_bytes(self, idx):
        return _report.algorithmic_bytes(self, idx)

    def flops(self, idx):
        return _report.flops(self, idx)

    def launch_op(self, idx, image_ptr=None, pred_ptr=None):
        op = self.ops[idx]
        if op.kind in (lib.OP_STEM, lib.OP_STEM2) and image_ptr is not None:
            op.src[0].ptr = image_ptr
        if op.kind in (lib.OP_DECODE, lib.OP_HEADTAIL) and pred_ptr is not None:
            op.out = pred_ptr
        stream = torch.cuda.current_stream(self.device).cuda_stream
        lib.check(lib.load().maf_op_launch(C.byref(op), stream))

    def view(self, buf):
        dt = torch.float32 if buf.esize == 4 else torch.float16
        start = buf.off + (self._abase - self.arena.data_ptr())
        n = self.B * buf.H * buf.W * buf.stride * buf.esize
        return self.arena[start:start + n].view(dt).view(self.B, buf.H, buf.W, buf.stride)

    def featmaps(self):
        return [tuple(None if b is None else self.view(b)[..., :b.C].permute(0, 3, 1, 2) for b in hb) for hb in self.head_bufs]

    def __del__(self):
        try:
            if getattr(self, "_engine", None):
                lib.load().maf_engine_destroy(self._engine)
        except Exception:
            pass
```

maf-yolo_amd/lib.py:

```python
import ctypes as C
import os

from .config import cfg

_HERE = os.path.dirname(os.path.abspath(__file__))
LIB_PATH = cfg.hip_lib or os.path.join(_HERE, "libmafyolo_hip.so")

F16, F32, U8 = 0, 1, 2
NMS_FLOAT_THRESHOLD = 1
NMS_PRECOLLECTED = 4
NMS_CNT_STRIDE = 64
NMS_MATRIX = 8
NMS_SINGLE_LAUNCH = 2
ACT_NONE, ACT_RELU, ACT_SILU, ACT_SIGMOID = 0, 1, 2, 3
SRC_DIRECT, SRC_UP2, SRC_POOL2, SRC_SUB2, SRC_PAIRS = 0, 1, 2, 3, 4
OP_STEM, OP_CONV1X1, OP_CONV3X3S2, OP_DWCONV, OP_SPPF_POOL, OP_DECODE, OP_BOTTLENECK, OP_CONV1DW, OP_HEADTAIL, OP_STEM2, OP_CONV3X3S2_DGRAD = range(11)
CONV_GENERIC, CONV_LDS, CONV_STREAM, CONV_SPLITK, CONV_STREAM_LDS, CONV3_LDS, CONV3_WREG, CONV_DMA = range(1, 9)
CONV_VARIANT_NAMES = {CONV_GENERIC: "generic", CONV_LDS: "lds", CONV_STREAM: "stream", CONV_SPLITK: "k4", CONV_STREAM_LDS: "streamlds", CONV3_LDS: "ldsall",
                      CONV3_WREG: "wreg", CONV_DMA: "dma"}
DW_MFMA, DW_DOT2, DW_PAIRS = -1, -2, -4
DW_P2_STAGED = 128


def dw_tile_k(rows, low, staged=False):
    return rows * 256 + low + (DW_P2_STAGED if staged else 0)


def dw_tile_k_split(tile_k):
    return tile_k >> 8, tile_k & (DW_P2_STAGED - 1), bool(tile_k & DW_P2_STAGED)


class MafSrc(C.Structure):
    _fields_ = [("ptr", C.c_void_p), ("C", C.c_int32), ("stride", C.c_int32), ("coff", C.c_int32), ("mode", C.c_int32)]


class MafPackDesc(C.Structure):
    _fields_ = [("src", C.c_void_p), ("dst", C.c_void_p), ("total", C.c_int64), ("kind", C.c_int32), ("dtype", C.c_int32),
                ("Cout", C.c_int32), ("Cin", C.c_int32), ("taps", C.c_int32), ("transpose", C.c_int32),
                ("CT", C.c_int32), ("steps", C.c_int32), ("Kp", C.c_int32), ("flip", C.c_int32), ("block0", C.c_int32), ("reserved", C.c_int32)]


class MafLetterboxImage(C.Structure):
    _fields_ = [("ptr", C.c_void_p), ("pitch", C.c_int64), ("h", C.c_int32), ("w", C.c_int32),
                ("new_h", C.c_int32), ("new_w", C.c_int32), ("top", C.c_int32), ("left", C.c_int32)]


LETTERBOX_KARG_MAX = 64


class MafAugmentFrame(C.Structure):
    _fields_ = [("src", C.c_void_p), ("src_pitch", C.c_int64), ("h", C.c_int32), ("w", C.c_int32),
                ("dst", C.c_void_p), ("new_h", C.c_int32), ("new_w", C.c_int32)]


AREA_FAST2, AREA_FASTN, AREA_GENERAL = 0, 1, 2
AUGMENT_MAX_TILES = 4


class MafAugmentTile(C.Structure):
    _fields_ = [("ptr", C.c_void_p), ("pitch", C.c_int64), ("h", C.c_int32), ("w", C.c_int32),
                ("x0", C.c_int32), ("y0", C.c_int32), ("x1", C.c_int32), ("y1", C.c_int32), ("dx", C.c_int32), ("dy", C.c_int32)]


class MafAugmentSample(C.Structure):
    _fields_ = [("minv", (C.c_double * 6) * 2), ("r", C.c_double), ("ntiles", C.c_int32 * 2), ("hsv", C.c_int32), ("flipud", C.c_int32),
                ("fliplr", C.c_int32), ("reserved", C.c_int32), ("tile", (MafAugmentTile * AUGMENT_MAX_TILES) * 2), ("lut", (C.c_uint8 * 256) * 3)]


PR_MAX_DET = 1024
PR_MAX_LABELS = 1024
PR_MAX_CLASSES = 1024
PR_HEADER = 16
PR_LABELS_XYXY, PR_CONFUSION = 1, 2
PR_ERR_CLASS, PR_ERR_LABELS, PR_ERR_CAPACITY = 1, 2, 4
COCO_T, COCO_R, COCO_A, COCO_M = 10, 101, 4, 3
COCO_MAX_DETS = 100
COCO_MAX_GT = 256
COCO_GT_CROWD, COCO_GT_IDNZ = 1, 2


class MafEmaDesc(C.Structure):
    _fields_ = [("dst", C.c_void_p), ("src", C.c_void_p), ("total", C.c_int64), ("block0", C.c_int32), ("reserved", C.c_int32)]


class MafSgdDesc(C.Structure):
    _fields_ = [("param", C.c_void_p), ("grad", C.c_void_p), ("buf", C.c_void_p), ("total", C.c_int64), ("block0", C.c_int32), ("group", C.c_int32)]


class MafRangeDesc(C.Structure):
    _fields_ = [("ptr", C.c_void_p), ("total", C.c_int64), ("block0", C.c_int32), ("reserved", C.c_int32)]


class Phase(int):
    """The `phase` argument of a BatchNorm scratch (csrc/bn_act.hip: which half this call accumulates into) as a step tape sees it: a word that alternates
    from replay to replay (tape.py registers a toggle for the argument slot it is passed in)."""


TAPE_MAX_ARGS = 28


class MafTapeRec(C.Structure):
    _fields_ = [("fn", C.c_int32), ("stream", C.c_int32), ("a", C.c_uint64 * TAPE_MAX_ARGS)]


class MafTapeToggle(C.Structure):
    _fields_ = [("addr", C.c_void_p), ("mask", C.c_uint64), ("width", C.c_int32), ("reserved", C.c_int32)]


class MafOp(C.Structure):
    _fields_ = [("kind", C.c_int32), ("dtype", C.c_int32), ("in_dtype", C.c_int32), ("act", C.c_int32),
                ("B", C.c_int32), ("H", C.c_int32), ("W", C.c_int32), ("Hin", C.c_int32), ("Win", C.c_int32),
                ("Cin", C.c_int32), ("Cout", C.c_int32), ("ksize", C.c_int32), ("nsrc", C.c_int32),
                ("src", MafSrc * 4), ("out", C.c_void_p), ("out_stride", C.c_int32), ("out_coff", C.c_int32),
                ("out_f32", C.c_int32), ("tile_p", C.c_int32), ("tile_c", C.c_int32), ("tile_k", C.c_int32),
                ("w", C.c_void_p), ("bias", C.c_void_p),
                ("reg", C.c_void_p * 3), ("lvl_h", C.c_int32 * 3), ("lvl_w", C.c_int32 * 3),
                ("reg_stride", C.c_int32), ("nc", C.c_int32), ("reg_max", C.c_int32), ("lvl_stride", C.c_float * 3),
                ("aux", C.c_void_p * 4), ("lane", C.c_int32), ("n_wait", C.c_int32), ("wait", C.c_int32 * 8),
                ("out_pairs", C.c_int32), ("reserved0", C.c_int32)]


EXPORTS = ["maf_last_error", "maf_version", "maf_op_size", "maf_op_launch", "maf_engine_create", "maf_engine_num_ops",
           "maf_engine_run", "maf_engine_run_filtered", "maf_engine_run_graph", "maf_engine_run_timed", "maf_engine_destroy", "maf_nms_workspace_bytes", "maf_nms", "maf_nms_ex", "maf_nms_debug", "maf_pack_w1x1_bytes", "maf_pack_w1x1", "maf_pack_dw", "maf_pack_batch", "maf_pack_desc_size", "maf_ema_update", "maf_ema_desc_size", "maf_sgd_update", "maf_sgd_desc_size", "maf_nonfinite_check", "maf_range_desc_size", "maf_maxpool_forward", "maf_maxpool_backward", "maf_upsample2x_forward", "maf_upsample2x_backward", "maf_zero", "maf_grad_fold", "maf_add_sub2", "maf_colsum", "maf_dw_wgrad", "maf_dw_wgrad31", "maf_stem_train", "maf_image_to_nhwc8", "maf_bottleneck_record_bytes", "maf_bottleneck_tail_record_bytes", "maf_bottleneck_tail_supported", "maf_conv1dw_record_bytes", "maf_head_tail_record_bytes", "maf_stem2_record_bytes", "maf_conv3s2_lds_record_bytes", "maf_mprep_lds_record_bytes", "maf_mprep_wreg_record_bytes", "maf_conv3s2_wreg_record_bytes", "maf_conv1x1_stats_supported", "maf_coco_rows", "maf_conv1x1_wgrad", "maf_conv_wgrad", "maf_bn_forward", "maf_bn_backward", "maf_bn_backward_acc", "maf_set_deterministic", "maf_dw_branches", "maf_dw_branches_stats", "maf_bn_forward_ex", "maf_bn_replicas", "maf_bn_stats", "maf_bn_sum_forward", "maf_bn_sum_forward_stats", "maf_bn_sum_backward", "maf_tal_targets", "maf_tal_assign", "maf_atss_assign", "maf_loss_partial_rows", "maf_loss_decode", "maf_loss_terms",
           "maf_detect_join", "maf_detect_join_backward", "maf_nhwc_sum", "maf_stream_fork", "maf_stream_join", "maf_tape_fn_id", "maf_tape_fn_nargs", "maf_tape_rec_size", "maf_tape_run", "maf_tape_toggle",
           "maf_stream_create_masked", "maf_stream_destroy", "maf_letterbox", "maf_letterbox_lds_bytes", "maf_rescale_boxes",
           "maf_augment_resize", "maf_mosaic_affine", "maf_augment_sample_size", "maf_area_struct_sizes", "maf_resize_area",
           "maf_pr_state_ints", "maf_pr_out_doubles", "maf_pr_workspace_bytes", "maf_pr_match", "maf_pr_curves",
           "maf_coco_append", "maf_coco_match", "maf_coco_accumulate", "maf_jpeg_struct_sizes", "maf_jpeg_progressive_struct_sizes", "maf_jpeg_decode",
           "maf_timer_create", "maf_timer_start", "maf_timer_stop", "maf_timer_elapsed_ms", "maf_timer_destroy"]

_lib = None
_recorder = None


class MafError(RuntimeError):
    pass


def load():
    global _lib
    if _recorder is not None:
        return _recorder
    if _lib is not None:
        return _lib
    if not os.path.exists(LIB_PATH):
        raise MafError("libmafyolo_hip.so not found at %s — the HIP extension is not built; "
                       "run `python -c 'import __graft_entry__ as g; g.build()'` (there is no CPU fallback)" % LIB_PATH)
    lib = C.CDLL(LIB_PATH)
    lib.maf_last_error.restype = C.c_char_p
    lib.maf_version.restype = C.c_int
    if not hasattr(lib, "maf_op_size") or lib.maf_op_size() != C.sizeof(MafOp):
        raise MafError("libmafyolo_hip.so was built for a maf_op_t of %s bytes, this binding declares %d: rebuild (__graft_entry__.build())"
                       % (lib.maf_op_size() if hasattr(lib, "maf_op_size") else "?", C.sizeof(MafOp)))
    lib.maf_op_launch.argtypes = [C.POINTER(MafOp), C.c_void_p]
    lib.maf_engine_create.argtypes = [C.POINTER(MafOp), C.c_int32, C.POINTER(C.c_void_p)]
    lib.maf_engine_num_ops.argtypes = [C.c_void_p]
    lib.maf_engine_run.argtypes = [C.c_void_p, C.c_void_p, C.c_void_p, C.c_void_p]
    lib.maf_engine_run_graph.argtypes = [C.c_void_p, C.c_void_p, C.c_void_p, C.c_void_p]
    lib.maf_engine_run_timed.argtypes = [C.c_void_p, C.c_void_p, C.c_void_p, C.c_void_p, C.POINTER(C.c_float)]
    lib.maf_engine_destroy.argtypes = [C.c_void_p]
    lib.maf_engine_destroy.restype = None
    lib.maf_engine_run_filtered.argtypes = [C.c_void_p, C.c_void_p, C.c_void_p, C.c_void_p, C.c_void_p, C.c_double]
    lib.maf_nms_workspace_bytes.argtypes = [C.c_int32, C.c_int32, C.c_int32]
    lib.maf_nms_workspace_bytes.restype = C.c_int64
    lib.maf_nms.argtypes = [C.c_void_p, C.c_int32, C.c_int32, C.c_int32, C.c_double, C.c_double, C.c_void_p, C.c_int32,
                            C.c_int32, C.c_int32, C.c_int32, C.c_void_p, C.c_int64, C.c_void_p, C.c_void_p, C.c_void_p,
                            C.c_void_p]
    lib.maf_nms_ex.argtypes = [C.c_void_p, C.c_int32, C.c_int32, C.c_int32, C.c_double, C.c_double, C.c_void_p, C.c_int32,
                               C.c_int32, C.c_int32, C.c_int32, C.c_void_p, C.c_int64, C.c_void_p, C.c_void_p, C.c_void_p, C.c_int32, C.c_void_p]
    lib.maf_nms_debug.argtypes = [C.POINTER(C.c_uint64)]
    lib.maf_conv1x1_wgrad.argtypes = [C.c_void_p, C.c_int32, C.c_void_p, C.c_int32, C.c_int32, C.c_int32, C.c_int32, C.c_int32, C.c_void_p, C.c_void_p]
    lib.maf_conv_wgrad.argtypes = [C.c_void_p, C.c_int32, C.c_void_p, C.c_int32] + [C.c_int32] * 10 + [C.c_void_p, C.c_void_p]
    lib.maf_tal_assign.argtypes = ([C.c_void_p, C.c_int32] + [C.c_void_p] * 5 + [C.c_int32] * 5 + [C.c_float] * 3 + [C.c_int32, C.c_void_p, C.c_void_p, C.c_float]
                                   + [C.c_void_p] * 4)
    lib.maf_atss_assign.argtypes = [C.c_void_p] * 5 + [C.c_int32] * 5 + [C.c_void_p, C.c_void_p, C.c_float, C.c_float] + [C.c_void_p] * 4
    lib.maf_loss_partial_rows.argtypes = [C.c_int32] * 3
    lib.maf_loss_partial_rows.restype = C.c_int64
    lib.maf_loss_decode.argtypes = [C.c_void_p, C.c_int32, C.c_void_p, C.c_void_p] + [C.c_int32] * 3 + [C.c_void_p] * 2
    lib.maf_loss_terms.argtypes = [C.c_void_p, C.c_void_p, C.c_int32] + [C.c_void_p] * 5 + [C.c_int32] * 4 + [C.c_float] * 3 + [C.c_void_p] * 6
    lib.maf_tal_targets.argtypes = [C.c_void_p, C.c_int32, C.c_int32, C.c_float] + [C.c_void_p] * 4
    lib.maf_bn_forward.argtypes = [C.c_void_p, C.c_int32, C.c_int32, C.c_int32, C.c_int32, C.c_void_p, C.c_void_p, C.c_float, C.c_float, C.c_void_p, C.c_void_p,
                                   C.c_void_p, C.c_int32, C.c_void_p, C.c_int32, C.c_void_p, C.c_void_p, C.c_void_p, C.c_int32, C.c_int32, C.c_void_p, C.c_int32, C.c_void_p]
    lib.maf_bn_backward.argtypes = [C.c_void_p, C.c_int32, C.c_void_p, C.c_int32, C.c_int32, C.c_int32, C.c_int32, C.c_void_p, C.c_void_p, C.c_void_p, C.c_void_p,
                                    C.c_int32, C.c_void_p, C.c_int32, C.c_void_p, C.c_void_p, C.c_void_p, C.c_int32, C.c_int32, C.c_void_p, C.c_int32, C.c_void_p, C.c_int32, C.c_void_p]
    lib.maf_bn_backward_acc.argtypes = [C.c_void_p, C.c_int32, C.c_void_p, C.c_int32, C.c_int32, C.c_int32, C.c_int32, C.c_void_p, C.c_void_p, C.c_void_p, C.c_void_p,
                                        C.c_int32, C.c_void_p, C.c_int32, C.c_void_p, C.c_void_p, C.c_void_p, C.c_int32, C.c_int32, C.c_void_p, C.c_int32, C.c_void_p, C.c_int32, C.c_int32, C.c_void_p]
    lib.maf_set_deterministic.argtypes = [C.c_int32]
    lib.maf_dw_branches.argtypes = [C.c_void_p] * 5 + [C.c_int32] * 8 + [C.c_void_p]
    lib.maf_dw_branches_stats.argtypes = [C.c_void_p] * 5 + [C.c_int32] * 7 + [C.c_void_p, C.c_int32, C.c_void_p]
    lib.maf_bn_forward_ex.argtypes = [C.c_void_p, C.c_int32, C.c_int32, C.c_int32, C.c_int32, C.c_void_p, C.c_void_p, C.c_float, C.c_float, C.c_void_p, C.c_void_p,
                                      C.c_void_p, C.c_int32, C.c_void_p, C.c_int32, C.c_void_p, C.c_void_p, C.c_void_p, C.c_int32, C.c_int32, C.c_void_p, C.c_int32, C.c_int32, C.c_void_p]
    lib.maf_bn_stats.argtypes = [C.c_void_p, C.c_int32, C.c_int32, C.c_int32, C.c_int32, C.c_void_p, C.c_int32, C.c_int32, C.c_void_p]
    lib.maf_bn_sum_forward.argtypes = [C.c_void_p, C.c_void_p, C.c_int32, C.c_int32, C.c_int32, C.c_int32, C.c_void_p, C.c_void_p, C.c_float, C.c_float,
                                       C.c_void_p, C.c_void_p, C.c_void_p, C.c_void_p, C.c_int32, C.c_void_p, C.c_void_p, C.c_void_p, C.c_int32, C.c_void_p, C.c_int32, C.c_void_p]
    lib.maf_bn_sum_forward_stats.argtypes = [C.c_void_p, C.c_void_p, C.c_int32, C.c_int32, C.c_int32, C.c_int32, C.c_void_p, C.c_void_p, C.c_float, C.c_float,
                                             C.c_void_p, C.c_void_p, C.c_void_p, C.c_void_p, C.c_int32, C.c_void_p, C.c_void_p, C.c_void_p, C.c_int32, C.c_void_p, C.c_int32,
                                             C.c_void_p, C.c_int32, C.c_int32, C.c_void_p]
    lib.maf_bn_sum_backward.argtypes = [C.c_void_p, C.c_int32, C.c_void_p, C.c_void_p, C.c_int32, C.c_int32, C.c_int32, C.c_int32, C.c_void_p, C.c_void_p, C.c_void_p, C.c_void_p,
                                        C.c_void_p, C.c_void_p, C.c_void_p, C.c_void_p, C.c_int32, C.c_void_p, C.c_int32, C.c_int32, C.c_int32, C.c_void_p]
    lib.maf_bn_replicas.argtypes = [C.c_int32, C.c_int32]
    lib.maf_bn_replicas.restype = C.c_int32
    lib.maf_conv1x1_stats_supported.argtypes = [C.c_int32, C.c_int32]
    lib.maf_conv1x1_stats_supported.restype = C.c_int
    lib.maf_coco_rows.argtypes = [C.c_void_p, C.c_void_p, C.c_int32, C.c_int32, C.c_void_p, C.c_void_p, C.c_int32, C.c_void_p, C.c_void_p, C.c_void_p]
    lib.maf_conv1dw_record_bytes.argtypes = [C.c_int32] * 2
    lib.maf_conv1dw_record_bytes.restype = C.c_int64
    lib.maf_head_tail_record_bytes.argtypes = [C.c_int32]
    lib.maf_head_tail_record_bytes.restype = C.c_int64
    lib.maf_stem2_record_bytes.argtypes = [C.c_int32, C.c_int32, C.c_int32]
    lib.maf_stem2_record_bytes.restype = C.c_int64
    lib.maf_conv3s2_lds_record_bytes.argtypes = [C.c_int32, C.c_int32]
    lib.maf_conv3s2_lds_record_bytes.restype = C.c_int64
    lib.maf_mprep_lds_record_bytes.argtypes = [C.c_int32, C.c_int32, C.c_int32]
    lib.maf_mprep_lds_record_bytes.restype = C.c_int64
    lib.maf_mprep_wreg_record_bytes.argtypes = [C.c_int32, C.c_int32, C.c_int32]
    lib.maf_mprep_wreg_record_bytes.restype = C.c_int64
    lib.maf_conv3s2_wreg_record_bytes.argtypes = [C.c_int32, C.c_int32]
    lib.maf_conv3s2_wreg_record_bytes.restype = C.c_int64
    lib.maf_bottleneck_record_bytes.argtypes = [C.c_int32] * 3
    lib.maf_bottleneck_record_bytes.restype = C.c_int64
    lib.maf_bottleneck_tail_record_bytes.argtypes = [C.c_int32] * 3
    lib.maf_bottleneck_tail_record_bytes.restype = C.c_int64
    lib.maf_bottleneck_tail_supported.argtypes = [C.c_int32] * 4
    lib.maf_pack_w1x1_bytes.argtypes = [C.c_int32] * 5
    lib.maf_pack_w1x1_bytes.restype = C.c_int64
    lib.maf_pack_w1x1.argtypes = [C.c_void_p, C.c_int32, C.c_int32, C.c_int32, C.c_int32, C.c_int32, C.c_void_p, C.c_void_p]
    lib.maf_pack_dw.argtypes = [C.c_void_p, C.c_int32, C.c_int32, C.c_int32, C.c_int32, C.c_void_p, C.c_void_p]
    lib.maf_pack_batch.argtypes = [C.c_void_p, C.c_int32, C.c_int32, C.c_void_p]
    lib.maf_pack_desc_size.argtypes = []
    lib.maf_ema_update.argtypes = [C.c_void_p, C.c_int32, C.c_int32, C.c_float, C.c_float, C.c_void_p]
    lib.maf_ema_desc_size.argtypes = []
    lib.maf_sgd_update.argtypes = [C.c_void_p, C.c_int32, C.c_int32, C.c_int32, C.POINTER(C.c_double), C.POINTER(C.c_double), C.POINTER(C.c_double), C.POINTER(C.c_int32),
                                   C.c_void_p, C.c_void_p, C.c_void_p]
    lib.maf_sgd_desc_size.argtypes = []
    lib.maf_nonfinite_check.argtypes = [C.c_void_p, C.c_int32, C.c_int32, C.c_void_p, C.c_void_p]
    lib.maf_range_desc_size.argtypes = []
    lib.maf_zero.argtypes = [C.c_void_p, C.c_int64, C.c_void_p]
    lib.maf_grad_fold.argtypes = [C.c_void_p, C.c_int32, C.c_int32, C.c_int32, C.c_void_p, C.c_int32, C.c_int32, C.c_int32, C.c_void_p]
    lib.maf_upsample2x_forward.argtypes = [C.c_void_p] + [C.c_int32] * 6 + [C.c_void_p, C.c_int32, C.c_void_p]
    lib.maf_upsample2x_backward.argtypes = [C.c_void_p] + [C.c_int32] * 6 + [C.c_void_p, C.c_int32, C.c_void_p]
    lib.maf_add_sub2.argtypes = [C.c_void_p, C.c_int32, C.c_void_p] + [C.c_int32] * 6 + [C.c_void_p]
    lib.maf_colsum.argtypes = [C.c_void_p, C.c_int32, C.c_int64, C.c_int32, C.c_int32, C.c_void_p, C.c_void_p]
    lib.maf_maxpool_forward.argtypes = [C.c_void_p] + [C.c_int32] * 9 + [C.c_void_p, C.c_int32, C.c_void_p, C.c_void_p]
    lib.maf_maxpool_backward.argtypes = [C.c_void_p, C.c_int32, C.c_void_p] + [C.c_int32] * 8 + [C.c_void_p, C.c_int32, C.c_void_p]
    lib.maf_pack_desc_size.restype = C.c_int32
    lib.maf_ema_desc_size.restype = C.c_int32
    lib.maf_sgd_desc_size.restype = C.c_int32
    lib.maf_range_desc_size.restype = C.c_int32
    lib.maf_dw_wgrad.argtypes = [C.c_void_p, C.c_int32, C.c_void_p, C.c_int32, C.c_int32, C.c_int32, C.c_int32, C.c_int32, C.c_int32, C.c_int32, C.c_void_p, C.c_int32, C.c_void_p]
    lib.maf_image_to_nhwc8.argtypes = [C.c_void_p, C.c_int32, C.c_int32, C.c_int32, C.c_int32, C.c_void_p, C.c_void_p]
    lib.maf_stem_train.argtypes = [C.c_void_p, C.c_int32, C.c_int32, C.c_int32, C.c_int32, C.c_void_p, C.c_void_p, C.c_int32, C.c_void_p, C.c_void_p, C.c_void_p]
    lib.maf_dw_wgrad31.argtypes = [C.c_void_p, C.c_int32] * 4 + [C.c_int32] * 5 + [C.c_void_p] * 3 + [C.c_int32, C.c_void_p]
    lib.maf_detect_join.argtypes = [C.c_void_p, C.c_void_p, C.c_void_p, C.c_void_p, C.c_void_p] + [C.c_int32] * 5 + [C.c_void_p] * 3
    lib.maf_detect_join_backward.argtypes = [C.c_void_p, C.c_void_p, C.c_void_p, C.c_void_p] + [C.c_int32] * 5 + [C.c_void_p] * 4 + [C.c_int32, C.c_int32, C.c_void_p]
    lib.maf_nhwc_sum.argtypes = [C.c_void_p, C.c_void_p, C.c_int32, C.c_void_p, C.c_int32, C.c_int64, C.c_int32, C.c_int32, C.c_int32, C.c_void_p]
    lib.maf_stream_fork.argtypes = [C.c_void_p, C.c_void_p]
    lib.maf_stream_join.argtypes = [C.c_void_p, C.c_void_p]
    lib.maf_stream_create_masked.argtypes = [C.c_void_p, C.c_int32, C.POINTER(C.c_void_p)]
    lib.maf_stream_destroy.argtypes = [C.c_void_p]
    lib.maf_tape_fn_id.argtypes = [C.c_char_p]
    lib.maf_tape_fn_id.restype = C.c_int32
    lib.maf_tape_fn_nargs.argtypes = [C.c_int32]
    lib.maf_tape_fn_nargs.restype = C.c_int32
    lib.maf_tape_rec_size.restype = C.c_int32
    lib.maf_tape_run.argtypes = [C.c_void_p, C.c_int32, C.c_int32, C.c_void_p, C.c_int32, C.POINTER(C.c_int32)]
    lib.maf_tape_toggle.argtypes = [C.c_void_p, C.c_int32]
    if lib.maf_tape_rec_size() != C.sizeof(MafTapeRec):
        raise MafError("libmafyolo_hip.so was built for a maf_tape_rec_t of %d bytes, this binding declares %d: rebuild" % (lib.maf_tape_rec_size(), C.sizeof(MafTapeRec)))
    lib.maf_letterbox.argtypes = [C.POINTER(MafLetterboxImage), C.c_void_p, C.c_int32, C.c_int32, C.c_int32, C.POINTER(C.c_uint8), C.c_int32, C.c_void_p, C.c_void_p]
    lib.maf_letterbox_lds_bytes.argtypes = [C.POINTER(MafLetterboxImage), C.c_int32, C.c_int32]
    lib.maf_letterbox_lds_bytes.restype = C.c_int64
    lib.maf_rescale_boxes.argtypes = [C.c_void_p, C.c_void_p, C.c_int32, C.c_int32, C.c_int32, C.c_void_p, C.c_int32, C.c_void_p]
    lib.maf_augment_resize.argtypes = [C.c_void_p, C.c_void_p, C.c_int32, C.c_void_p]
    lib.maf_mosaic_affine.argtypes = [C.c_void_p, C.c_void_p, C.c_int32, C.c_int32, C.c_void_p, C.c_void_p]
    lib.maf_augment_sample_size.restype = C.c_int32
    if lib.maf_augment_sample_size() != C.sizeof(MafAugmentSample):
        raise MafError("libmafyolo_hip.so was built for a maf_augment_sample_t of %d bytes, this binding declares %d: rebuild" % (lib.maf_augment_sample_size(), C.sizeof(MafAugmentSample)))
    lib.maf_area_struct_sizes.argtypes = [C.POINTER(C.c_int32)]
    lib.maf_resize_area.argtypes = [C.c_void_p, C.c_void_p, C.c_int32, C.c_void_p, C.c_void_p, C.c_int64, C.c_void_p]
    lib.maf_pr_state_ints.argtypes = [C.c_int32]
    lib.maf_pr_state_ints.restype = C.c_int64
    lib.maf_pr_out_doubles.argtypes = [C.c_int32, C.c_int32]
    lib.maf_pr_out_doubles.restype = C.c_int64
    lib.maf_pr_workspace_bytes.argtypes = [C.c_int32, C.c_int32, C.c_int64]
    lib.maf_pr_workspace_bytes.restype = C.c_int64
    lib.maf_pr_match.argtypes = [C.c_void_p, C.c_void_p, C.c_int32, C.c_int32, C.c_void_p, C.c_int32, C.c_void_p, C.c_int32, C.c_int32,
                                 C.c_void_p, C.c_int32, C.c_int32, C.c_int32, C.c_float, C.c_float, C.c_void_p, C.c_void_p, C.c_void_p,
                                 C.c_void_p, C.c_int64, C.c_void_p, C.c_void_p]
    lib.maf_pr_curves.argtypes = [C.c_void_p, C.c_void_p, C.c_void_p, C.c_int64, C.c_void_p, C.c_int32, C.c_int32, C.c_void_p, C.c_int64,
                                  C.c_void_p, C.c_void_p]
    lib.maf_coco_append.argtypes = [C.c_void_p, C.c_void_p, C.c_int64, C.c_void_p, C.c_int32, C.c_void_p, C.c_int32, C.c_void_p, C.c_void_p,
                                    C.c_void_p, C.c_void_p, C.c_void_p]
    lib.maf_coco_match.argtypes = [C.c_void_p, C.c_void_p, C.c_void_p, C.c_void_p, C.c_void_p, C.c_void_p, C.c_void_p, C.c_int64, C.c_void_p,
                                   C.c_void_p, C.c_int32, C.c_int32, C.c_void_p, C.c_void_p, C.c_void_p, C.c_void_p, C.c_void_p, C.c_void_p,
                                   C.c_void_p]
    lib.maf_coco_accumulate.argtypes = [C.c_void_p, C.c_void_p, C.c_void_p, C.c_void_p, C.c_void_p, C.c_int64, C.c_void_p, C.c_void_p,
                                        C.c_void_p, C.c_int32, C.c_int32, C.c_int32, C.c_void_p, C.c_void_p, C.c_void_p, C.c_void_p,
                                        C.c_void_p, C.c_void_p]
    lib.maf_jpeg_struct_sizes.argtypes = [C.POINTER(C.c_int32)]
    lib.maf_jpeg_progressive_struct_sizes.argtypes = [C.POINTER(C.c_int32)]
    lib.maf_jpeg_decode.argtypes = [C.c_void_p, C.c_void_p, C.c_void_p, C.c_void_p, C.c_void_p, C.c_void_p, C.c_int32, C.c_void_p]
    lib.maf_timer_create.argtypes = [C.POINTER(C.c_void_p)]
    lib.maf_timer_start.argtypes = [C.c_void_p, C.c_void_p]
    lib.maf_timer_stop.argtypes = [C.c_void_p, C.c_void_p]
    lib.maf_timer_elapsed_ms.argtypes = [C.c_void_p, C.POINTER(C.c_float)]
    lib.maf_timer_destroy.argtypes = [C.c_void_p]
    lib.maf_timer_destroy.restype = None
    _lib = lib
    return lib


def check(rc):
    if rc != 0:
        raise MafError("libmafyolo_hip: %s (code %d)" % (load().maf_last_error().decode(), rc))


class Timer:

    def __init__(self):
        self._h = C.c_void_p()
        check(load().maf_timer_create(C.byref(self._h)))

    def start(self, stream):
        check(load().maf_timer_start(self._h, stream))

    def stop(self, stream):
        check(load().maf_timer_stop(self._h, stream))

    def elapsed_ms(self):
        ms = C.c_float()
        check(load().maf_timer_elapsed_ms(self._h, C.byref(ms)))
        return ms.value

    def __del__(self):
        try:
            if self._h:
                load().maf_timer_destroy(self._h)
        except Exception:
            pass
```

maf-yolo_amd/model.py:

```python
import copy
import itertools
from operator import attrgetter

import torch
import torch.nn as nn

from .config import cfg
from . import arch, lib, train_ops
from .engine import Plan
from .layers import (RepVGGBlock, RepHDW, MPRep, SPPF, ConvWrapper, Concat, Head_DepthUni, Out)


class Upsample(nn.Upsample):

    def forward(self, x, out=None):
        if self.scale_factor == 2 and self.mode == "nearest" and x.is_cuda:
            return train_ops.upsample2x(x, out=out)
        with torch.autocast(device_type=x.device.type, enabled=False):
            return super().forward(x)


class Detect_yaml(nn.Module):

    def __init__(self, num_classes=80, anchors=1, num_layers=3, use_dfl=True, reg_max=16, stride=(8, 16, 32)):
        super().__init__()
        self.nc, self.no, self.nl = num_classes, num_classes + 5, num_layers
        self.na = anchors if not isinstance(anchors, (list, tuple)) else len(anchors[0]) // 2
        self.use_dfl, self.reg_max = use_dfl, reg_max
        self.register_buffer("stride", torch.tensor(list(stride), dtype=torch.float32), persistent=False)
        self.proj_conv = nn.Conv2d(reg_max + 1, 1, 1, bias=False)
        self.initialize_biases()

    def initialize_biases(self):
        self.proj = nn.Parameter(torch.linspace(0, self.reg_max, self.reg_max + 1), requires_grad=False)
        self.proj_conv.weight = nn.Parameter(self.proj.view(1, self.reg_max + 1, 1, 1).clone().detach(), requires_grad=False)

    def forward(self, heads, val_loss=False, logits=False):
        if logits:
            cls, reg = train_ops.detect_join(heads)
        else:
            cls = torch.cat([h[1].flatten(2).permute(0, 2, 1) for h in heads], 1)
            reg = torch.cat([h[2].flatten(2).permute(0, 2, 1) for h in heads], 1)
        return [h[0] for h in heads], cls, reg

    @staticmethod
    def level_views(feats, cls, reg):
        out, a0 = [], 0
        for f in feats:
            h, w = f.shape[-2:]
            out.append((f, cls[:, a0:a0 + h * w].permute(0, 2, 1).unflatten(2, (h, w)), reg[:, a0:a0 + h * w].permute(0, 2, 1).unflatten(2, (h, w))))
            a0 += h * w
        return out


def _nodes_from_config(config, num_classes):
    if isinstance(config, str) and config in ("n", "s", "m"):
        return arch.builtin(config, num_classes), dict(strides=(8, 16, 32), reg_max=16, use_dfl=True)
    if isinstance(config, dict) and "backbone" in config:
        return arch.nodes_from_yaml_dict(copy.deepcopy(config), 3, num_classes), dict(strides=(8, 16, 32), reg_max=16, use_dfl=True)
    model_cfg = getattr(config, "model", None)
    if model_cfg is not None and getattr(model_cfg, "yaml_file", None):
        import yaml
        with open(model_cfg.yaml_file, encoding="ascii", errors="ignore") as f:
            d = yaml.safe_load(f)
        head = model_cfg.head
        return (arch.nodes_from_yaml_dict(d, d.get("ch", 3), num_classes),
                dict(strides=tuple(head.strides), reg_max=getattr(head, "reg_max", 16), use_dfl=getattr(head, "use_dfl", True)))
    raise ValueError("Model(config): pass 'n' | 's' | 'm', a YAML dict in the reference's schema, or the reference's config object")


_VERSION = attrgetter("_version")


class _Aliases(list):
    """The aliases train_ops.fanout made of a node's output: every reader pops one."""


class Model(nn.Module):
    def __init__(self, config="n", channels=3, num_classes=80, anchors=1, precision=None, dispatch="engine"):
        super().__init__()
        self._maf_apply_gen = 0
        assert channels == 3, "MAF-YOLO takes 3-channel images"
        self.nodes, hcfg = _nodes_from_config(config, num_classes)
        assert hcfg["use_dfl"] and hcfg["reg_max"] == 16 or hcfg["use_dfl"], "DFL head expected (configs/MAF-YOLO-n.py:15-16)"
        layers = []
        for nd in self.nodes:
            a = nd.args
            if nd.kind == "repvgg":
                m = RepVGGBlock(nd.cin, nd.cout)
            elif nd.kind == "rephdw":
                m = RepHDW(nd.cin, nd.cout, a["depth"], a["expansion"], a["k"], a["depth_expansion"])
            elif nd.kind == "mprep":
                m = MPRep(nd.cin, nd.cout)
            elif nd.kind == "sppf":
                m = SPPF(nd.cin, nd.cout, a["k"])
            elif nd.kind == "cw":
                m = ConvWrapper(nd.cin, nd.cout, 3, 2)
            elif nd.kind == "concat":
                m = Concat(1)
            elif nd.kind == "up":
                m = Upsample(None, 2, "nearest")
            elif nd.kind == "head":
                m = Head_DepthUni(nd.cin, nd.cout, a["reg_max"], a["k"], a["nc"])
            elif nd.kind == "out":
                m = Out()
            else:
                raise NotImplementedError(nd.kind)
            m.i, m.f, m.type = nd.i, nd.f, type(m).__name__
            layers.append(m)
        self.backbone = nn.Sequential(*layers)
        self.save = sorted({s for nd in self.nodes for s in nd.sources() if nd.i > 0 and s != nd.i - 1} |
                           {s for nd in self.nodes if isinstance(nd.f, list) for s in nd.sources()})
        self.detect = Detect_yaml(num_classes, anchors, 3, hcfg["use_dfl"], hcfg["reg_max"], hcfg["strides"])
        self.nc = num_classes
        self.names = [str(i) for i in range(num_classes)]
        self.build_type = "yaml"
        self.precision = precision
        self._plans = {}
        self._plans_version = None
        self._fp_tensors = None
        self.fuse_bottlenecks = "auto"
        self.fuse_stem = True
        self.fuse_head = "auto"
        self.fuse_tail = "auto"
        self.fuse_mprep = "auto"
        self.twin_convs = True
        self.autotune = False
        self.multi_stream = False
        self.step_tape = "auto" if cfg.step_tape else False
        assert dispatch in ("engine", "ops")
        self.dispatch = dispatch

    @property
    def stride(self):
        return self.detect.stride

    def train(self, mode=True):
        if mode:
            self._plans = {}
        elif getattr(self, "training", False):
            self.release_tapes()
        return super().train(mode)

    def release_tapes(self):
        for ent in getattr(self, "_tapes", {}).values():
            tp = ent[1]
            if tp is not None:
                tp.release()
        self._tapes = {}

    def load_state_dict(self, *a, **k):
        self.invalidate()
        return super().load_state_dict(*a, **k)

    def invalidate(self):
        self._plans = {}
        self._plans_version = None
        self._fp_tensors = None
        self._pack_plan = None
        self.release_tapes()
        self._ops_weights = (None, None)

    def _apply(self, fn, *a, **k):
        self.invalidate()
        self._maf_apply_gen = getattr(self, "_maf_apply_gen", 0) + 1
        return super()._apply(fn, *a, **k)

    def weights_version(self):
        ts = self._fp_tensors
        if ts is None:
            ts = self._fp_tensors = list(itertools.chain(self.parameters(), self.buffers()))
        return sum(map(_VERSION, ts)) + len(ts)

    def half(self):
        self.precision = "fp16"
        return self

    def float(self):
        self.precision = None
        return super().float()

    def __deepcopy__(self, memo):
        plans, self._plans = self._plans, {}
        fpt, self._fp_tensors = self._fp_tensors, None
        pp, self._pack_plan = getattr(self, "_pack_plan", None), None
        tp, self._tapes = getattr(self, "_tapes", {}), {}
        try:
            cls = self.__class__
            new = cls.__new__(cls)
            memo[id(self)] = new
            for k, v in self.__dict__.items():
                new.__dict__[k] = copy.deepcopy(v, memo)
        finally:
            self._plans, self._fp_tensors, self._pack_plan, self._tapes = plans, fpt, pp, tp
        return new

    def __getstate__(self):
        d = dict(self.__dict__)
        d["_plans"] = {}
        d["_fp_tensors"] = d["_plans_version"] = d["_pack_plan"] = None
        d["_tapes"] = {}
        return d

    def _forward_train_form(self, x, raw_heads=False, logits=False):
        if getattr(self, "_pack_plan", None) is None:
            self._pack_plan = train_ops.PackPlan()
        train_ops.begin_step(self._pack_plan, x.device)
        res = getattr(self, "_cat_residents", None)
        if res is None:
            res = self._cat_residents = {}
            for nd, m in zip(self.nodes, self.backbone):
                if isinstance(m, Concat) and m.d == 1:
                    srcs = nd.sources()
                    widths = [self.nodes[s].cout for s in srcs]
                    for slot, s in enumerate(srcs):
                        if s not in res and isinstance(self.backbone[s], (ConvWrapper, RepHDW, SPPF, Upsample)) and srcs.count(s) == 1:
                            res[s] = (nd.i, slot, widths)
        bufs = {}

        def slot_of(j, slot, widths):
            def f(z):
                cb = bufs.get(j)
                if cb is None:
                    cb = bufs[j] = train_ops.CatBuffer(z, widths)
                return cb.slot(slot)
            return f

        uses = getattr(self, "_node_uses", None)
        if uses is None:
            uses = self._node_uses = {}
            for nd in self.nodes:
                if nd.i > 0:
                    for j in nd.sources():
                        uses[j] = uses.get(j, 0) + 1
        y = []
        n_head, n_cw, on_lane = 0, 0, {}
        for nd, m in zip(self.nodes, self.backbone):
            if nd.i > 0:
                for j in nd.sources():
                    if j in on_lane:
                        y[j] = train_ops.lane_join(y[j], on_lane.pop(j))
                src = [y[j].pop() if isinstance(y[j], _Aliases) else y[j] for j in nd.sources()]
                x = src if isinstance(nd.f, list) else src[0]
            r = res.get(nd.i) if train_ops.cat_free else None
            if raw_heads and isinstance(m, ConvWrapper) and isinstance(x, torch.Tensor):
                n_cw += 1
                out_ = None if r is None else slot_of(*r)
                x, ln = train_ops.lane_run(n_cw % 2, (lambda t, m=m, o=out_: m(t) if o is None else m(t, out=o)), x)
                if ln and uses.get(nd.i, 0) > 1:
                    x = train_ops.lane_join(x, ln)
                elif ln:
                    on_lane[nd.i] = ln
            elif r is not None:
                x = m(x, out=slot_of(*r))
            elif nd.i in bufs:
                x = train_ops.join(bufs.pop(nd.i), x)
            elif raw_heads and isinstance(m, Head_DepthUni):
                x = m(x, raw=True, lanes=(2 * n_head + 1, 2 * n_head + 2))
                n_head += 1
            elif logits and isinstance(m, Head_DepthUni):
                x = m(x, raw=True)
            else:
                x = m(x)
            n_use = uses.get(nd.i, 0)
            if n_use > 1 and isinstance(x, torch.Tensor) and x.is_cuda and x.requires_grad and train_ops.cat_free:
                x = _Aliases(train_ops.fanout(x, n_use))
            y.append(x)
        if raw_heads:
            x = [(h[0], train_ops.lane_join(h[1], h[3]), train_ops.lane_join(h[2], h[4])) for h in x]
        return x

    def _train_out(self, x):
        tape = self._tape_for(x)
        if tape is None:
            native = x.is_cuda and not train_ops.framework_ops
            if x.is_cuda:
                x = x.contiguous(memory_format=torch.channels_last)
            return tuple(self.detect(self._forward_train_form(x, logits=native), logits=native))
        if tape.ready:
            return tape.replay_forward(x)
        return tape.record_forward(self, x)

    def _tape_for(self, x):
        from . import exchange, tape as _tape
        ex = exchange.current
        if (not getattr(self, "step_tape", "auto") or ex is None or not x.is_cuda or x.dim() != 4 or x.shape[1] != 3 or not torch.is_grad_enabled()
                or train_ops.profile is not None or train_ops.framework_ops or train_ops._deterministic or not train_ops.cat_free or train_ops._rec is not None):
            return None
        half = x.dtype == torch.float16 or (torch.is_autocast_enabled("cuda") and torch.get_autocast_dtype("cuda") == torch.float16)
        if not half or x.dtype not in (torch.float16, torch.float32) or x.shape[2] % 32 or x.shape[3] % 32:
            return None
        if not hasattr(self, "_tapes"):
            self._tapes = {}
        key = (tuple(x.shape), x.dtype, x.device.index, id(ex), train_ops._stream(x.device), train_ops.wgrad_stream)
        ent = self._tapes.get(key)
        if ent is None:
            if len(self._tapes) >= 4:
                old = self._tapes.pop(next(iter(self._tapes)))
                if old[1] is not None:
                    old[1].release()
            ent = self._tapes[key] = [0, None, 0]
        ent[0] += 1
        tp = ent[1]
        if tp is not None:
            if tp.ready:
                if tp.pending_backward:
                    if tp.graph_alive():
                        train_ops.stats["tape_busy_eager"] = train_ops.stats.get("tape_busy_eager", 0) + 1
                        return None
                    tp.drop_pending()
                return tp
            if tp.failed is not None or tp.phase is not None:
                return None
            ent[1] = tp = None
        pp = getattr(self, "_pack_plan", None)
        if (ent[0] < _tape.RECORD_AT or ent[2] >= 2 or pp is None or pp.dirty or pp.table is None
                or any(not p_.is_cuda for p_ in self.parameters())):
            return None
        ent[2] += 1
        ent[1] = _tape.StepTape(ex, x.device)
        return ent[1]

    def plan_for(self, x, head_feats=False, slot=0):
        if not x.is_cuda:
            raise lib.MafError("MAF-YOLO eval forward runs on the HIP engine only: got a %s tensor (no CPU fallback)" % x.device)
        B, ch, H, W = x.shape
        assert ch == 3
        if x.dtype == torch.uint8:
            in_dt = lib.U8
        elif x.dtype == torch.float16:
            in_dt = lib.F16
        elif x.dtype == torch.float32:
            in_dt = lib.F32
        else:
            raise TypeError("image dtype must be uint8, float16 or float32")
        if self.precision == "fp16":
            dt = lib.F16
        elif self.precision == "fp32":
            dt = lib.F32
        else:
            dt = lib.F32 if x.dtype == torch.float32 else lib.F16
        fuse_head = bool(getattr(self, "fuse_head", True)) and not head_feats
        key = (B, H, W, dt, in_dt, x.device.index, fuse_head, slot, repr(getattr(self, "fuse_stem", True)), repr(self.fuse_bottlenecks), repr(getattr(self, "fuse_tail", "auto")), self.multi_stream, bool(getattr(self, "twin_convs", True)))
        ver = self.weights_version()
        if ver != self._plans_version:
            self._plans = {}
            self._plans_version = ver
        plan = self._plans.get(key)
        if plan is None:
            if len(self._plans) >= 8:
                self._plans.pop(next(iter(self._plans)))
            fuse = None
            if self.autotune and dt == lib.F16 and self.fuse_bottlenecks == "auto":
                from .engine import choose_fusion
                fuse = choose_fusion(self, B, H, W, dt, in_dt, x.device, x.contiguous())
            plan = Plan(self, B, H, W, dt, in_dt, x.device, fuse=fuse, fuse_head=fuse_head)
            if self.autotune and dt == lib.F16:
                plan.autotune(x.contiguous())
            self._plans[key] = plan
        return plan

    def traceable(self, dtype=torch.float16):
        from . import ops_forward, torch_ops
        weights = ops_forward.deploy_weights(self, dtype)
        ops = torch_ops.load()
        strides = [float(s) for s in self.detect.stride.tolist()]

        def f(x):
            return ops_forward.forward(self, x, weights, ops, strides)[0]
        return f

    def forward(self, x, val_loss=False, slot=0):
        if self.training:
            out = self._train_out(x)
            return [out, self.detect.level_views(*out)]
        if getattr(self, "dispatch", "engine") == "ops" and not val_loss:
            from . import ops_forward
            if not x.is_cuda:
                raise lib.MafError("MAF-YOLO eval forward runs on the HIP device only: got a %s tensor (no CPU fallback)" % x.device)
            dt = torch.float32 if (self.precision == "fp32" or (self.precision is None and x.dtype == torch.float32)) else torch.float16
            ver = (self.weights_version(), dt)
            if getattr(self, "_ops_weights", (None, None))[0] != ver:
                self._ops_weights = (ver, ops_forward.deploy_weights(self, dt))
            xin = (x.to(dt) / 255 if x.dtype == torch.uint8 else x.to(dt)).contiguous(memory_format=torch.channels_last)
            pred, heads = ops_forward.forward(self, xin, self._ops_weights[1])
            return [pred, [tuple(h) for h in heads]]
        plan = self.plan_for(x, head_feats=val_loss, slot=slot)
        x = x.contiguous()
        with torch.cuda.device(x.device):
            conf = getattr(self, "nms_filter", None)
            if conf is not None and not val_loss and 0.0 <= conf < 1.0 and plan.filter_ok():
                from . import nms as _nms
                pred = torch.empty(plan.B, plan.A, 5 + plan.nc, dtype=torch.float32, device=plan.device)
                ws = _nms.candidate_workspace(plan.device, plan.B, plan.A, plan.nc, slot)
                plan.run_into(x, pred, cand=(ws, conf))
                pred._maf_cand = (ws, float(conf), ws._maf_gen, pred._version)
            else:
                pred = plan.run(x, graph=False)
        feats = plan.featmaps()
        if val_loss:
            return [self.detect(feats), feats]
        return [pred, feats]
```

maf-yolo_amd/pack.py:

```python
import torch

from . import lib


def tile_for(cout, m_pixels):
    best = None
    for ct in (8, 6, 4, 2):
        n_tiles = -(-cout // (16 * ct))
        padded = n_tiles * 16 * ct
        key = (padded, n_tiles)
        if best is None or key < best[0]:
            best = (key, ct, n_tiles)
    ct, n_tiles = best[1], best[2]
    pt = 2 if (-(-m_pixels // 128)) * n_tiles >= 1024 else 1
    return pt, ct


def _steps(c, ks):
    return -(-c // ks)


def pack_matrix(w2d_segments, ct, dtype):
    ks = 32 if dtype == lib.F16 else 16
    ch = ks // 4
    cout = w2d_segments[0].shape[0]
    n_tiles = -(-cout // (16 * ct))
    npad = n_tiles * 16 * ct
    cols = []
    for seg in w2d_segments:
        s = _steps(seg.shape[1], ks)
        blk = torch.zeros(npad, s * ks, dtype=torch.float32)
        blk[:cout, :seg.shape[1]] = seg
        cols.append(blk)
    wp = torch.cat(cols, 1)
    S = wp.shape[1] // ks
    wp = wp.reshape(n_tiles, 16, ct, S, 4, ch)
    wp = wp.permute(0, 2, 3, 4, 1, 5).contiguous()
    wp = wp.reshape(n_tiles * ct, S, 64, ch)
    return wp.to(torch.float16 if dtype == lib.F16 else torch.float32).contiguous()


def pack_conv1x1(w, src_channels, ct, dtype):
    w2 = w.reshape(w.shape[0], -1).float().cpu()
    segs, o = [], 0
    for c in src_channels:
        segs.append(w2[:, o:o + c])
        o += c
    assert o == w2.shape[1], "source channels do not add up to Cin"
    return pack_matrix(segs, ct, dtype)


def pack_conv3x3(w, ct, dtype):
    w = w.float().cpu()
    return pack_matrix([w[:, :, ky, kx] for ky in range(3) for kx in range(3)], ct, dtype)


def pack_bias(b, ct):
    cout = b.shape[0]
    npad = -(-cout // (16 * ct)) * 16 * ct
    out = torch.zeros(npad, dtype=torch.float32)
    out[:cout] = b.float().cpu()
    return out


def pack_dw(w, dtype):
    c, _, k, _ = w.shape
    return w.float().cpu().reshape(c, k * k).t().contiguous().to(torch.float16 if dtype == lib.F16 else torch.float32)


def pack_dw_pairs(w):
    c, _, k, _ = w.shape
    assert c % 8 == 0
    npair = (k + 1) // 2
    wd = w.float().cpu().reshape(c // 8, 2, 4, k, k)
    wz = torch.zeros(c // 8, 2, 4, k, k + 3)
    wz[..., 1:k + 1] = wd
    out = torch.zeros(c // 8, k, 2, 2, npair, 4, 2)
    for m in range(npair):
        for st, u0 in ((0, 2 * m), (1, 2 * m - 1)):
            out[:, :, :, st, m, :, 0] = wz[..., u0 + 1].permute(0, 3, 1, 2)
            out[:, :, :, st, m, :, 1] = wz[..., u0 + 2].permute(0, 3, 1, 2)
    return out.to(torch.float16).contiguous()


def pairs_from_nhwc(x):
    b, h, w_, c = x.shape
    assert w_ % 2 == 0
    return x.reshape(b, h, w_ // 2, 2, c).transpose(3, 4).contiguous()


def pack_conv1dw(w1, b1, wdw, bdw):
    mid, c = w1.shape[0], w1.shape[1]
    k = wdw.shape[-1]
    nmb = -(-mid // 32)
    mp = nmb * 32
    perm = torch.tensor([8 * (pl % 4) + pl // 4 for pl in range(32)])
    w1p = torch.zeros(mp, c); w1p[:mid] = w1.reshape(mid, c).float().cpu()
    b1p = torch.zeros(mp); b1p[:mid] = b1.float().cpu()
    w1p = w1p.reshape(nmb, 32, c)[:, perm].reshape(mp, c)
    b1q = b1p.reshape(nmb, 32)[:, perm]
    W1 = torch.cat([pack_matrix([w1p[m * 32:(m + 1) * 32]], 1, lib.F16) for m in range(nmb)], 0)
    wfull = torch.zeros(mp, 1, k, k); wfull[:mid] = wdw.float().cpu()
    toe = pack_dw_toeplitz(wfull)
    bdp = torch.zeros(mp); bdp[:mid] = bdw.float().cpu()

    def raw(t):
        return t.contiguous().view(torch.uint8).reshape(nmb, -1)
    rec = torch.cat([raw(W1.reshape(nmb, -1)), raw(b1q.contiguous()), raw(toe.reshape(nmb, -1)), raw(bdp.reshape(nmb, 32))], 1).contiguous()
    return rec, nmb


def pack_dw_toeplitz(w):
    c, _, k, _ = w.shape
    ncb = -(-c // 32)
    wd = torch.zeros(ncb * 32, k, k); wd[:c] = w.float().cpu().reshape(c, k, k)
    parts = 2 if k > 5 else 1
    toe = torch.zeros(ncb, 8, k, parts, 4, 4, 8)
    wv = wd.reshape(ncb, 4, 8, k, k)
    for part in range(parts):
        for r in range(4):
            for j in range(8):
                kx = j - r + 4 * part
                if kx < 0 or kx >= k or (part == 0 and kx > 4) or (part == 1 and kx < 5):
                    continue
                toe[:, :, :, part, :, r, j] = wv[:, :, :, :, kx].permute(0, 2, 3, 1)
    return toe.reshape(ncb, 8, k, parts, 16, 8).to(torch.float16).contiguous()


def pack_stem(w):
    return w.float().cpu().reshape(w.shape[0], 27).t().contiguous()


def pack_bottleneck(w1, b1, wdw, bdw, w2, b2):
    mid, c = w1.shape[0], w1.shape[1]
    k = wdw.shape[-1]
    nmb = -(-mid // 32)
    mp = nmb * 32
    L2E = 1.4426950408889634
    w1, b1, bdw, w2 = w1.float() * L2E, b1.float() * L2E, bdw.float() * L2E, w2.float() / L2E
    w1p = torch.zeros(mp, c); w1p[:mid] = w1.reshape(mid, c).float().cpu()
    W1 = torch.cat([pack_matrix([w1p[m * 32:(m + 1) * 32]], 1, lib.F16) for m in range(nmb)], 0)
    b1p = torch.zeros(mp); b1p[:mid] = b1.float().cpu()
    wd = torch.zeros(mp, k, k); wd[:mid] = wdw.float().cpu().reshape(mid, k, k)
    parts = 2 if k > 5 else 1
    toe = torch.zeros(nmb, 8, k, parts, 4, 4, 8)
    wv = wd.reshape(nmb, 8, 4, k, k)
    for part in range(parts):
        for r in range(4):
            for j in range(8):
                kx = j - r + 4 * part
                if kx < 0 or kx >= k or (part == 0 and kx > 4) or (part == 1 and kx < 5):
                    continue
                toe[:, :, :, part, :, r, j] = wv[:, :, :, :, kx].permute(0, 1, 3, 2)
    bdp = torch.zeros(mp); bdp[:mid] = bdw.float().cpu()
    bdp = bdp.reshape(nmb, 8, 4).permute(0, 2, 1).contiguous().reshape(mp)
    ct2 = 2 if c <= 32 else 4
    w2f = torch.zeros(c, mp); w2f[:, :mid] = w2.reshape(c, mid).float().cpu()
    w2f = w2f.reshape(c, nmb, 8, 4).permute(0, 1, 3, 2).reshape(c, mp)
    W2 = torch.cat([pack_matrix([w2f[:, m * 32:(m + 1) * 32]], ct2, lib.F16) for m in range(nmb)], 0)
    b2p = torch.zeros(16 * ct2); b2p[:c] = b2.float().cpu()
    def raw(t):
        return t.contiguous().view(torch.uint8).reshape(nmb, -1)
    rec = torch.cat([raw(W1.reshape(nmb, -1)), raw(b1p.reshape(nmb, 32)), raw(toe.reshape(nmb, -1).to(torch.float16)),
                     raw(W2.reshape(nmb, -1)), raw(bdp.reshape(nmb, 32))], 1).contiguous()
    return rec, b2p, nmb, ct2


def pack_bottleneck_tail(w3, b3, c, nsrc):
    C3 = w3.shape[0]
    assert C3 % 16 == 0 and w3.reshape(C3, -1).shape[1] == (nsrc + 1) * c and c % 8 == 0 and c <= 64
    c3t, s1, ct2 = C3 // 16, -(-c // 32), (2 if c <= 32 else 4)
    ys = ct2 // 2
    nv = 4 * c3t
    P = 8 if nv % 8 == 0 else 4
    w = w3.detach().reshape(C3, -1).float().cpu()
    cols = []
    for s_ in range(nsrc):
        for ks in range(s1):
            for gl in range(4):
                for j in range(8):
                    ch = 32 * ks + 8 * gl + j
                    cols.append(s_ * c + ch if ch < c else -1)
    for j2 in range(ys):
        for gl in range(4):
            for j in range(8):
                ch = 16 * gl + 8 * j2 + j if ct2 == 4 else 8 * gl + j
                cols.append(nsrc * c + ch if ch < c else -1)
    cols = torch.tensor(cols)
    wk = torch.zeros(C3, cols.numel())
    ok = cols >= 0
    wk[:, ok] = w[:, cols[ok]]
    g_, rr_, t_ = torch.meshgrid(torch.arange(4), torch.arange(4), torch.arange(c3t), indexing="ij")
    v = rr_ * c3t + t_
    ch_out = (v // P) * (4 * P) + g_ * P + v % P
    assert sorted(ch_out.reshape(-1).tolist()) == list(range(C3))
    nst = cols.numel() // 32
    rows = ch_out.permute(2, 0, 1).reshape(c3t, 16)
    fr = wk[rows.reshape(-1)].reshape(c3t, 16, nst, 4, 8)
    fr = fr.permute(2, 0, 3, 1, 4).contiguous().half()
    b3p = b3.detach().float().cpu()[ch_out.permute(0, 2, 1).reshape(-1)].contiguous()
    rec = torch.cat([fr.reshape(-1).view(torch.uint8), b3p.view(torch.uint8)])
    assert rec.numel() == nst * c3t * 1024 + 64 * c3t
    return rec


def pack_head_tail(w1, b1, w2, b2):
    w1 = w1.detach().float().cpu().reshape(w1.shape[0], -1)
    w2 = w2.detach().float().cpu().reshape(w2.shape[0], -1)
    C = w1.shape[0]
    assert w1.shape == (C, C) and w2.shape[1] == C and w2.shape[0] <= 80 and C % 32 == 0
    ks, t1 = C // 32, C // 16
    f1 = w1.view(t1, 16, ks, 4, 8).permute(0, 2, 3, 1, 4).contiguous().half()
    w2p = torch.zeros(80, C)
    w2p[:w2.shape[0]] = w2
    j, g, q = torch.meshgrid(torch.arange(ks), torch.arange(4), torch.arange(8), indexing="ij")
    ch = 32 * j + torch.where(q < 4, 4 * g + q, 16 + 4 * g + q - 4)
    f2 = w2p[:, ch.reshape(-1)].view(5, 16, ks, 4, 8).permute(0, 2, 3, 1, 4).contiguous().half()
    b2p = torch.zeros(80)
    b2p[:b2.numel()] = b2.detach().float().cpu()
    rec = torch.cat([f1.reshape(-1).view(torch.uint8), f2.reshape(-1).view(torch.uint8),
                     b1.detach().float().cpu().contiguous().view(torch.uint8), b2p.view(torch.uint8)])
    assert rec.numel() == C * C * 2 + 80 * C * 2 + C * 4 + 320
    return rec


def pack_stem2(w0, b0, w1, b1, w3=None, b3=None):
    w0 = w0.detach().float().cpu(); w1 = w1.detach().float().cpu()
    C0, C1 = w0.shape[0], w1.shape[0]
    assert w0.shape[1:] == (3, 3, 3) and w1.shape[1:] == (C0, 3, 3) and C0 % 8 == 0 and C0 <= 48 and C1 % 16 == 0
    nt0 = 2 if C0 <= 32 else 3
    m0 = torch.zeros(32, 16 * nt0)
    m0[:27, :C0] = w0.reshape(C0, 27).t()
    f0 = m0.view(4, 8, nt0, 16).permute(2, 0, 3, 1).contiguous().half()
    gr = C0 // 8
    npair = 9 * gr
    ks1 = (npair + 3) // 4
    m1 = torch.zeros(ks1 * 4, 8, C1)
    for q in range(npair):
        tap, grp = divmod(q, gr)
        m1[q] = w1[:, 8 * grp:8 * grp + 8, tap // 3, tap % 3].t()
    f1 = m1.view(ks1, 4, 8, C1 // 16, 16).permute(0, 3, 1, 4, 2).contiguous().half()
    b0p = torch.zeros(16 * nt0); b0p[:C0] = b0.detach().float().cpu()
    parts = [f0.reshape(-1).view(torch.uint8), f1.reshape(-1).view(torch.uint8), b0p.view(torch.uint8), b1.detach().float().cpu().contiguous().view(torch.uint8)]
    n = nt0 * 1024 + ks1 * (C1 // 16) * 1024 + nt0 * 64 + C1 * 4
    if w3 is not None:
        w3 = w3.detach().float().cpu().reshape(w3.shape[0], -1)
        C3 = w3.shape[0]
        assert w3.shape[1] == C1 and C3 % 16 == 0
        ks3 = (C1 + 31) // 32
        w3p = torch.zeros(C3, ks3 * 32)
        w3p[:, :C1] = w3
        j, g, q = torch.meshgrid(torch.arange(ks3), torch.arange(4), torch.arange(8), indexing="ij")
        ch = 32 * j + torch.where(q < 4, 4 * g + q, 16 + 4 * g + q - 4)
        f3 = w3p[:, ch.reshape(-1)].view(C3 // 16, 16, ks3, 4, 8).permute(0, 2, 3, 1, 4).contiguous().half()
        parts += [f3.reshape(-1).view(torch.uint8), b3.detach().float().cpu().contiguous().view(torch.uint8)]
        n += ks3 * (C3 // 16) * 1024 + C3 * 4
    rec = torch.cat(parts)
    assert rec.numel() == n
    return rec


def pack_conv3x3_lds(w, b):
    w = w.detach().float().cpu()
    cout, cin = w.shape[:2]
    assert cin % 8 == 0 and cout % 16 == 0 and w.shape[2:] == (3, 3)
    gr = cin // 8
    npair = 9 * gr
    ks = (npair + 3) // 4
    m1 = torch.zeros(ks * 4, 8, cout)
    for q in range(npair):
        tap, grp = divmod(q, gr)
        m1[q] = w[:, 8 * grp:8 * grp + 8, tap // 3, tap % 3].t()
    f = m1.view(ks, 4, 8, cout // 16, 16).permute(0, 3, 1, 4, 2).contiguous().half()
    rec = torch.cat([f.reshape(-1).view(torch.uint8), b.detach().float().cpu().contiguous().view(torch.uint8)])
    assert rec.numel() == ks * (cout // 16) * 1024 + cout * 4
    return rec


def pack_mprep_lds(w, b, w1, b1):
    w1 = w1.detach().float().cpu().reshape(w1.shape[0], -1)
    c1, cin = w1.shape
    assert c1 % 16 == 0 and cin == w.shape[1]
    ks1 = -(-cin // 32)
    m1 = torch.zeros(ks1 * 32, c1)
    m1[:cin] = w1.t()
    f = m1.view(ks1, 4, 8, c1 // 16, 16).permute(0, 3, 1, 4, 2).contiguous().half()
    rec = torch.cat([pack_conv3x3_lds(w, b), f.reshape(-1).view(torch.uint8), b1.detach().float().cpu().contiguous().view(torch.uint8)])
    return rec


_WREG_SHAPES = {(128, 128): (8, 1), (96, 96): (6, 1), (96, 64): (4, 2), (64, 64): (4, 2), (64, 96): (6, 1), (128, 96): (6, 1)}


def conv3x3_wreg_shape(cin, cout):
    return _WREG_SHAPES.get((cin, cout))


def pack_mprep_wreg(w, b, w1, b1):
    w1 = w1.detach().float().cpu().reshape(w1.shape[0], -1)
    c1, cin = w1.shape
    assert c1 % 16 == 0 and cin % 32 == 0 and cin == w.shape[1]
    f = w1.t().contiguous().view(cin // 32, 4, 8, c1 // 16, 16).permute(3, 0, 1, 4, 2).contiguous().half()
    return torch.cat([pack_conv3x3_wreg(w, b), f.reshape(-1).view(torch.uint8), b1.detach().float().cpu().contiguous().view(torch.uint8)])


def pack_conv3x3_wreg(w, b):
    w = w.detach().float().cpu()
    cout, cin = w.shape[:2]
    assert (cin, cout) in _WREG_SHAPES and cin % 32 == 0 and cout % 16 == 0 and w.shape[2:] == (3, 3)
    gr = cin // 8
    ks = 9 * cin // 32
    m1 = torch.zeros(ks * 4, 8, cout)
    for q in range(9 * gr):
        tap, grp = divmod(q, gr)
        m1[q] = w[:, 8 * grp:8 * grp + 8, tap // 3, tap % 3].t()
    f = m1.view(ks, 4, 8, cout // 16, 16).permute(3, 0, 1, 4, 2).contiguous().half()
    rec = torch.cat([f.reshape(-1).view(torch.uint8), b.detach().float().cpu().contiguous().view(torch.uint8)])
    assert rec.numel() == (cout // 16) * ks * 1024 + cout * 4
    return rec
```

maf-yolo_amd/plan_report.py:

```python
from . import lib, pack

_ESIZE = {lib.F16: 2, lib.F32: 4}


def kernel_name(plan, idx):
    o = plan.ops[idx]
    T = "_Float16" if o.dtype == lib.F16 else "float"
    if o.kind in (lib.OP_CONV1X1, lib.OP_CONV3X3S2):
        if o.kind == lib.OP_CONV3X3S2:
            var = 3
        elif o.nsrc == 1 and o.src[0].mode == lib.SRC_POOL2:
            var = 2
        elif o.nsrc == 1 and o.src[0].mode == lib.SRC_DIRECT:
            var = 0
        else:
            var = 1
        outf32 = "true" if (o.out_f32 and o.dtype == lib.F16) else "false"
        if o.tile_k == lib.CONV_STREAM:
            return "conv1x1_stream_kernel<%d, %d, %d>" % (o.tile_p, o.tile_c, -(-o.Cin // 32))
        if o.tile_k == lib.CONV3_LDS:
            return "conv3s2_lds_kernel<%d, %d, 4, %d>" % (o.Cin, o.Cout, o.nc)
        if o.tile_k == lib.CONV3_WREG:
            return "conv3s2_wreg_kernel<%d, %d, %d, %d, %d, %d>" % ((o.Cin, o.Cout) + pack.conv3x3_wreg_shape(o.Cin, o.Cout) + (2 if o.tile_p == 2 else 3, o.nc))
        if o.tile_k == lib.CONV_STREAM_LDS:
            return "conv1x1_stream_lds_kernel<%d, %d, %s, %d, false>" % (o.tile_c, sum(-(-o.src[k].C // 32) for k in range(o.nsrc)), "true" if var == 1 else "false", 8 if o.tile_p == 2 else 4)
        return "conv_mfma_kernel<%s, %d, %d, %d, %s, %s, %s, %s>" % (T, o.tile_p, o.tile_c, var, outf32, "true" if o.tile_k == lib.CONV_SPLITK else "false", "true" if o.tile_k in (lib.CONV_LDS, lib.CONV_DMA) else "false",
                                                                     "true" if o.tile_k == lib.CONV_DMA else "false")
    if o.kind == lib.OP_DWCONV:
        if o.tile_p == lib.DW_MFMA:
            return "dwconv_mfma_kernel<%d, %d>" % (o.ksize, o.act)
        if o.tile_p == lib.DW_PAIRS:
            return "dwconv_p2_kernel<%d, %d, %d>" % (o.ksize, o.act, (o.Cout // o.Cin) if lib.dw_tile_k_split(o.tile_k)[2] else 0)
        if o.tile_p == lib.DW_DOT2:
            return "dwconv_dot2_kernel<%d, 8, %d, %d>" % (o.ksize, 2 if lib.dw_tile_k_split(o.tile_k)[0] % 2 == 0 else 1, o.act)
        return "dwconv_tile_kernel<%s, %d, %d>" % (T, o.ksize, o.act)
    if o.kind == lib.OP_BOTTLENECK:
        return "bottleneck_kernel<%d, %d, %d, %d, %d>" % (o.ksize, -(-o.Cin // 32), 2 if o.Cout <= 32 else 4, o.nc // 16, o.nsrc if o.nc else 0)
    if o.kind == lib.OP_CONV1DW:
        return "conv1dw_kernel<%d>" % o.ksize
    if o.kind == lib.OP_HEADTAIL:
        return "head_tail_kernel<%d, %d>" % (o.Cin, 2 if o.Cin <= 128 else 1)
    if o.kind == lib.OP_STEM2:
        return "stem2_kernel<%d, %d, %d>" % (o.ksize, o.Cout, o.nc)
    return {lib.OP_STEM: "stem_kernel", lib.OP_SPPF_POOL: "sppf_pool_lds_kernel", lib.OP_DECODE: "decode_kernel"}[o.kind]

def algorithmic_bytes(plan, idx):
    o = plan.ops[idx]
    es = plan.es
    px = plan.B * o.H * o.W
    if o.kind == lib.OP_STEM:
        ies = {lib.F16: 2, lib.F32: 4, lib.U8: 1}[o.in_dtype]
        return plan.B * 3 * o.Hin * o.Win * ies + px * o.Cout * es + 27 * o.Cout * 4
    if o.kind == lib.OP_STEM2:
        ies = {lib.F16: 2, lib.F32: 4, lib.U8: 1}[o.in_dtype]
        return plan.B * 3 * o.Hin * o.Win * ies + px * (o.nc or o.Cout) * es + (27 * o.ksize + 9 * o.ksize * o.Cout + o.Cout * o.nc) * es
    if o.kind == lib.OP_CONV1X1:
        rd = 0
        for i in range(o.nsrc):
            f = {lib.SRC_DIRECT: 1.0, lib.SRC_UP2: 0.25, lib.SRC_POOL2: 4.0}[o.src[i].mode]
            rd += px * f * o.src[i].C * es
        oes = 4 if o.out_f32 else es
        return int(rd) + px * o.Cout * oes + o.Cin * o.Cout * es
    if o.kind == lib.OP_CONV3X3S2:
        pooled = px * o.nc * es + o.Cin * o.nc * es if "pool1" in plan._ops[idx] else 0
        return (2 if "twin" in plan._ops[idx] else 1) * (plan.B * o.Hin * o.Win * o.Cin * es + px * o.Cout * es + 9 * o.Cin * o.Cout * es) + pooled
    if o.kind == lib.OP_DWCONV:
        return px * (o.Cin + o.Cout) * es + o.ksize * o.ksize * o.Cout * es
    if o.kind == lib.OP_CONV1DW:
        return px * (o.Cin + o.Cout) * es + (o.Cin * o.Cout + o.ksize * o.ksize * o.Cout) * es
    if o.kind == lib.OP_BOTTLENECK:
        mid = o.tile_k * 32
        wts = (o.Cin * mid + o.ksize * o.ksize * mid + mid * o.Cout) * es
        if o.nc:
            return px * (o.nsrc * o.Cin + o.nc) * es + wts + (o.nsrc + 1) * o.Cin * o.nc * es
        return px * (o.Cin + o.Cout) * es + wts
    if o.kind == lib.OP_SPPF_POOL:
        return 4 * px * o.src[0].C * es
    if o.kind == lib.OP_HEADTAIL:
        return px * (2 * o.Cin * es + (5 + plan.nc) * 4) + 2 * (o.Cin * o.Cin + 80 * o.Cin) * es
    if o.kind == lib.OP_DECODE:
        anchors = sum(t.H * t.W for t, c, _ in plan.head_bufs if c is not None)
        return plan.B * anchors * ((plan.nc + 4 * (plan.reg_max + 1)) * 4 + (5 + plan.nc) * 4)
    return 0

def flops(plan, idx):
    o = plan.ops[idx]
    px = plan.B * o.H * o.W
    if o.kind == lib.OP_STEM:
        return 2 * px * 27 * o.Cout
    if o.kind == lib.OP_STEM2:
        return 2 * (4 * px * 27 * o.ksize + px * 9 * o.ksize * o.Cout + px * o.Cout * o.nc)
    if o.kind == lib.OP_CONV1X1:
        return 2 * px * o.Cin * o.Cout
    if o.kind == lib.OP_CONV3X3S2:
        return (2 if "twin" in plan._ops[idx] else 1) * 2 * px * 9 * o.Cin * o.Cout + (2 * px * o.Cin * o.nc if "pool1" in plan._ops[idx] else 0)
    if o.kind == lib.OP_DWCONV:
        return 2 * px * o.ksize * o.ksize * o.Cout
    if o.kind == lib.OP_CONV1DW:
        return 2 * px * (o.Cin * o.Cout + o.ksize * o.ksize * o.Cout)
    if o.kind == lib.OP_BOTTLENECK:
        mid = plan._ops[idx]["mid"]
        return 2 * px * (o.Cin * mid + o.ksize * o.ksize * mid + mid * o.Cout + (o.nsrc + 1) * o.Cin * o.nc)
    if o.kind == lib.OP_HEADTAIL:
        return 2 * px * (2 * o.Cin * o.Cin + o.Cin * (plan.nc + 4 * (plan.reg_max + 1)))
    return 0
```

maf-yolo_amd/tuner.py:

```python
import ctypes as C
import os

import torch

from .config import cfg
from . import conv_variants, lib, pack
from .conv_variants import stream_lds_ok, time_candidates

_TUNE_CACHE = {}


def choose_fusion(model, B, H, W, dtype, in_dtype, device, x, reps=3):
    import numpy as np
    from .engine import Plan
    plan1 = Plan(model, B, H, W, dtype, in_dtype, device, fuse=True, fuse_tail=False)
    names, sigs = [], {}
    for i, o in enumerate(plan1.ops):
        nm = plan1.op_names[i]
        if o.kind == lib.OP_BOTTLENECK:
            names.append(nm); sigs[nm] = ("bn3", dtype, B, o.H, o.W, o.Cin, o.ksize)
        elif o.kind == lib.OP_CONV1DW:
            names.append(nm[:-len(".conv1dw")]); sigs[names[-1]] = ("bn3", dtype, B, o.H, o.W, o.Cin, o.ksize)
    if names and not all(sigs[n] in _TUNE_CACHE for n in names):
        pred = torch.empty(B, plan1.A, 5 + plan1.nc, dtype=torch.float32, device=device)

        def timed(plan):
            plan.autotune(x)
            plan.run_timed(x, pred)
            t = np.min([plan.run_timed(x, pred) for _ in range(reps)], 0)
            return dict(zip(plan.op_names, t))
        t0 = timed(Plan(model, B, H, W, dtype, in_dtype, device, fuse=False, fuse_tail=False))
        t1 = timed(plan1)
        t2 = timed(Plan(model, B, H, W, dtype, in_dtype, device, fuse=2, fuse_tail=False))
        for n in names:
            cost = {0: t0[n + ".conv1"] + t0[n + ".conv2"] + t0[n + ".one_conv"], 2: t2[n + ".conv1dw"] + t2[n + ".one_conv"]}
            if n in t1:
                cost[1] = t1[n]
            _TUNE_CACHE[sigs[n]] = (min(cost, key=cost.get),)
    del plan1
    return {n: _TUNE_CACHE[sigs[n]][0] for n in names}


def save_tune_cache(path):
    import json
    with open(path, "w") as f:
        json.dump({repr(k): list(v) for k, v in _TUNE_CACHE.items()}, f, indent=0, sort_keys=True)


def load_tune_cache(path):
    import ast
    import json
    with open(path) as f:
        for k, v in json.load(f).items():
            _TUNE_CACHE[ast.literal_eval(k)] = tuple(v)
    return len(_TUNE_CACHE)
_LANE_GROUPS = ((0, 1, 2, 3, 12, 13, 14, 15, 20, 21, 22, 23, 24, 25, 26, 27), (4, 5, 6, 7, 8, 9, 10, 11, 16, 17, 18, 19, 28, 29, 30, 31),
              (32, 33, 34, 35, 44, 45, 46, 47, 52, 53, 54, 55, 56, 57, 58, 59), (36, 37, 38, 39, 40, 41, 42, 43, 48, 49, 50, 51, 60, 61, 62, 63))


_P2_STAGE = cfg.dw_stage


def p2_wave_bytes(th, tw, k):
    p_ = k // 2
    pe = p_ + (p_ & 1)
    rwp, spr = tw // 2 + pe, tw // 4
    nstrips = th * spr
    best, bc = rwp, 1 << 30
    for pitch in range(rwp, rwp + 8):
        c = 0
        for g in _LANE_GROUPS:
            cnt = {}
            for lane in g:
                s_ = min(lane, nstrips - 1)
                slot = ((s_ // spr) * pitch + 2 * (s_ % spr)) & 15
                cnt[slot] = cnt.get(slot, 0) + 1
            c += max(cnt.values())
        if c < bc:
            best, bc = pitch, c
    return -(-(2 * (th + k - 1) * best) // 64) * 1024



_TUNED_KINDS = (lib.OP_STEM2, lib.OP_HEADTAIL, lib.OP_DWCONV, lib.OP_CONV1X1, lib.OP_CONV3X3S2)


class Candidate:
    __slots__ = ("tiles", "op", "keep", "pairs")

    def __init__(self, tiles, op, keep=(), pairs=False):
        self.tiles, self.op, self.keep, self.pairs = tuple(tiles), op, list(keep), pairs

    def __repr__(self):
        return "Candidate(%r%s)" % (self.tiles, ", pairs" if self.pairs else "")


def _feeds_pairs(plan, i):
    o = plan.ops[i]
    if not (o.kind == lib.OP_CONV1X1 and i + 1 < len(plan.ops) and plan.ops[i + 1].kind == lib.OP_DWCONV):
        return False
    keep_tk, o.tile_k = o.tile_k, lib.CONV_STREAM_LDS
    try:
        return plan._pairs_producer(i + 1) is not None
    finally:
        o.tile_k = keep_tk


def signature(plan, i):
    o, r = plan.ops[i], plan._ops[i]
    if o.kind == lib.OP_STEM2:
        return (o.kind, plan.dtype, plan.in_dtype, plan.B, o.H, o.W, o.ksize, o.Cout, o.nc)
    if o.kind == lib.OP_HEADTAIL:
        return (o.kind, plan.dtype, plan.B, o.H, o.W, o.Cin, "percu")
    if o.kind == lib.OP_DWCONV:
        return (o.kind, plan.dtype, plan.B, o.H, o.W, o.Cin, o.ksize, o.act) + ((o.Cout,) if o.Cout != o.Cin else ())
    if o.kind not in (lib.OP_CONV1X1, lib.OP_CONV3X3S2):
        return None
    M = plan.B * o.H * o.W
    return (o.kind, plan.dtype, M, o.Cin, o.Cout, o.nsrc, tuple(o.src[k].mode for k in range(o.nsrc)), int(o.out_f32)) + (("twin",) if r.get("twin") else ()) \
        + (("pool1",) if r.get("pool1") else ()) + (("pairs",) if _feeds_pairs(plan, i) else ())


_FUSED_3X3 = (lib.CONV3_LDS, lib.CONV3_WREG)


def packed(plan, i, wt, bt, ct, tk):
    o, r = plan.ops[i], plan._ops[i]
    pool1, srcC = r.get("pool1"), r["raw"][2]
    wreg = tk == lib.CONV3_WREG
    wp_ = ((pack.pack_mprep_wreg if wreg else pack.pack_mprep_lds)(wt, bt, *pool1) if pool1 else pack.pack_conv3x3_lds(wt, bt) if tk == lib.CONV3_LDS else pack.pack_conv3x3_wreg(wt, bt) if wreg
           else pack.pack_conv1x1(wt, srcC, ct, plan.dtype) if o.kind == lib.OP_CONV1X1 else pack.pack_conv3x3(wt, ct, plan.dtype)).to(plan.device)
    return wp_, pack.pack_bias(bt, ct if tk not in _FUSED_3X3 else 4).to(plan.device)


def conv_tiles(plan, i):
    o, r = plan.ops[i], plan._ops[i]
    return conv_variants.conv_tiles(o.kind, plan.dtype, plan.B * o.H * o.W, [(o.src[k].C, o.src[k].mode) for k in range(o.nsrc)], o.Cout, o.out_stride, bool(o.out_f32),
                                    bool(r.get("twin")), r.get("pool1_tk", lib.CONV3_LDS) if r.get("pool1") else None)


def dw_tiles(plan, i):
    o = plan.ops[i]
    n = 8 if plan.dtype == lib.F16 else 4
    out = []
    ths = sorted({4, 8, 16, 32} | {v for v in (o.H, o.H // 2) if 8 <= v <= 40})
    tws = sorted({8, 16, 32} | {v for v in (o.W, o.W // 2) if 8 <= v <= 40 and v % 4 == 0})
    for th in ths:
        for tw in tws:
            for cbm in (8, 4, 2):
                t_h, t_w, cb = min(th, o.H), min(tw, -(-o.W // 4) * 4), min(cbm * n, -(-o.Cin // n) * n)
                lds = ((t_h + o.ksize - 1) * (t_w + o.ksize - 1) * (cb // n + 2) + o.ksize * o.ksize * (cb // n)) * 16
                if lds > 96 * 1024 or (t_h, t_w, cb) in out:
                    continue
                out.append((t_h, t_w, cb))
    if plan.dtype == lib.F16:
        w8 = -(-o.W // 8) * 8
        for th in sorted({4, 8, 10, 16, 20} | ({o.H} if o.H <= 40 else set())):
            if th > o.H:
                continue
            for tw in sorted({16, 24, 32, 40} | ({w8} if w8 <= 40 else set())):
                if tw > w8:
                    continue
                for cb in (16, 32, 64):
                    cb = min(cb, o.Cin)
                    nq, np_ = cb // 4, (o.ksize + 1) // 2
                    lds = ((th + o.ksize - 1) * ((tw + o.ksize - 1) // 2) * (nq + 3) + o.ksize * 2 * np_ * nq) * 16
                    if lds > 96 * 1024 or (lib.DW_DOT2, tw, lib.dw_tile_k(th, cb)) in out:
                        continue
                    out.append((lib.DW_DOT2, tw, lib.dw_tile_k(th, cb)))
    if plan._pairs_producer(i) is not None:
        w4 = -(-o.W // 4) * 4
        for th in sorted({4, 5, 8, 10, 16, 20} | ({o.H} if o.H <= 40 else set())):
            if th > o.H:
                continue
            for tw in sorted({16, 20, 32, 40, 80} | ({w4} if w4 <= 80 else set())):
                if tw > w4:
                    continue
                plane = p2_wave_bytes(th, tw, o.ksize)
                if plane > 20 * 1024:
                    continue
                for nw, stg in ((2, False), (4, False), (8, False), (2, True), (4, True), (8, True)):
                    if stg and not ((o.Cin // 8) % nw == 0 and th * (tw // 4) <= 64 and plane >= 4160 and o.Cout <= 2 * o.Cin and _P2_STAGE):
                        continue
                    out.append((lib.DW_PAIRS, tw, lib.dw_tile_k(th, nw, stg)))
    if plan.dtype == lib.F16 and o.aux[0]:
        out.append((lib.DW_MFMA, 0, 0))
    return out


def candidates(plan, i):
    o, r = plan.ops[i], plan._ops[i]
    if o.kind == lib.OP_STEM2:
        out = []
        for rows in ((4,) if o.Cout == 96 else (8, 4)):
            for wgs in (256, 512, 768, 1024):
                op = lib.MafOp.from_buffer_copy(o)
                op.tile_p, op.tile_k = rows, wgs
                out.append(Candidate((rows, 0, wgs), op))
        return out
    if o.kind == lib.OP_HEADTAIL:
        out = []
        for iters in (1, 2, 3, 4, 6):
            op = lib.MafOp.from_buffer_copy(o)
            op.tile_k = iters
            out.append(Candidate((0, 0, iters), op))
        return out
    if o.kind == lib.OP_DWCONV:
        out = []
        for tp, tc, tk in dw_tiles(plan, i):
            op = lib.MafOp.from_buffer_copy(o)
            op.tile_p, op.tile_c, op.tile_k = tp, tc, tk
            op.src[0].mode = lib.SRC_PAIRS if tp == lib.DW_PAIRS else lib.SRC_DIRECT
            out.append(Candidate((tp, tc, tk), op, pairs=tp == lib.DW_PAIRS))
        return out
    if o.kind not in (lib.OP_CONV1X1, lib.OP_CONV3X3S2):
        return []
    w, b = r["raw"][:2]
    twin = r.get("twin")
    packs, out = {}, []
    for pt, ct, tk in conv_tiles(plan, i):
        form = (0, tk) if tk in _FUSED_3X3 else (ct, 0)
        if form not in packs:
            packs[form] = packed(plan, i, w, b, ct, tk) + (packed(plan, i, *twin["raw"], ct, tk) if twin else ())
        keep = packs[form]
        op = lib.MafOp.from_buffer_copy(o)
        op.tile_p, op.tile_c, op.tile_k, op.w, op.bias = pt, ct, tk, keep[0].data_ptr(), keep[1].data_ptr()
        op.out_pairs = 0
        if twin:
            op.aux[1], op.aux[2] = keep[2].data_ptr(), keep[3].data_ptr()
        out.append(Candidate((pt, ct, tk), op, keep))
    return out


def autotune(plan, x, reps=5, verbose=False):
    assert x.is_cuda
    L = lib.load()
    stream = torch.cuda.current_stream(plan.device)
    pred = torch.empty(plan.B, plan.A, 5 + plan.nc, dtype=torch.float32, device=plan.device)
    plan.run_into(x, pred)
    torch.cuda.synchronize(plan.device)
    plan._tuned = getattr(plan, "_tuned", [])
    changed = 0

    def timed(cands):
        res = time_candidates(lambda c_: lib.check(L.maf_op_launch(C.byref(c_.op), stream.cuda_stream)), cands, stream.cuda_stream, reps, "raise")
        return [(t,) + c_.tiles for t, c_ in res]

    for i, (o, r) in enumerate(zip(plan.ops, plan._ops)):
        sig = signature(plan, i)
        if sig is None:
            continue
        best = _TUNE_CACHE.get(sig)
        if o.kind == lib.OP_STEM2:
            if best is None:
                o.src[0].ptr = x.data_ptr()
                results = sorted((t, rows, wgs) for t, rows, _, wgs in timed(candidates(plan, i)))
                best = (results[0][1], 0, results[0][2])
                _TUNE_CACHE[sig] = best
                if verbose:
                    print("tune %-32s %dx%d: %s" % (plan.op_names[i], o.H, o.W, " ".join("(%d,%d)%.1fus" % (r_, w_, t * 1e3) for t, r_, w_ in results)))
            if (best[0], best[2]) != (o.tile_p, o.tile_k):
                o.tile_p, o.tile_k = best[0], best[2]
                changed += 1
            continue
        if o.kind == lib.OP_HEADTAIL:
            if best is None:
                o.out = pred.data_ptr()
                results = sorted((t, it) for t, _, _, it in timed(candidates(plan, i)))
                best = (0, 0, results[0][1])
                _TUNE_CACHE[sig] = best
                if verbose:
                    print("tune %-32s %dx%d C=%d: %s" % (plan.op_names[i], o.H, o.W, o.Cin, " ".join("(%d)%.1fus" % (it, t * 1e3) for t, it in results)))
            if best[2] != o.tile_k:
                o.tile_k = best[2]
                changed += 1
            continue
        if o.kind == lib.OP_DWCONV:
            if best is None:
                results = sorted(timed(candidates(plan, i)))
                best = results[0][1:]
                _TUNE_CACHE[sig] = best
                _TUNE_CACHE[sig + ("nhwc",)] = [r_ for r_ in results if r_[1] != lib.DW_PAIRS][0][1:]
                if verbose:
                    print("tune %-32s %dx%d C=%d k=%d: %s" % (plan.op_names[i], o.H, o.W, o.Cin, o.ksize, " ".join("(%d,%d,%d)%.1fus" % (a, b2, c2, t * 1e3) for t, a, b2, c2 in results[:6])))
                    p2 = [r_ for r_ in results if r_[1] == lib.DW_PAIRS]
                    if any(r_[3] & lib.DW_P2_STAGED for r_ in p2):
                        bu, bs = [r_ for r_ in p2 if not r_[3] & lib.DW_P2_STAGED][0], [r_ for r_ in p2 if r_[3] & lib.DW_P2_STAGED][0]
                        print("     dwconv_p2 stores  plain (%d,%d) %.1fus   staged (%d,%d) %.1fus" % (bu[2], bu[3], bu[0] * 1e3, bs[2], bs[3] - lib.DW_P2_STAGED, bs[0] * 1e3))
            prod = plan._pairs_producer(i)
            if best[0] == lib.DW_PAIRS and prod is None:
                best = _TUNE_CACHE.get(sig + ("nhwc",), (0, 0, 0))
            pairs = 1 if best[0] == lib.DW_PAIRS else 0
            if tuple(best) != (o.tile_p, o.tile_c, o.tile_k) or (prod is not None and prod.out_pairs != pairs):
                o.tile_p, o.tile_c, o.tile_k = best
                o.src[0].mode = lib.SRC_PAIRS if pairs else lib.SRC_DIRECT
                if prod is not None:
                    prod.out_pairs = pairs
                changed += 1
            continue
        twin, pool1 = r.get("twin"), r.get("pool1")
        if best is None:
            results = sorted(timed(candidates(plan, i)))
            best = (results[0][1], results[0][2], results[0][3])
            if sig[-1] == "pairs":
                five = [r_ for r_ in results if r_[3] == lib.CONV_STREAM_LDS]
                if five and five[0][0] <= 1.3 * results[0][0]:
                    best = (five[0][1], five[0][2], five[0][3])
            _TUNE_CACHE[sig] = best
            if verbose:
                M = plan.B * o.H * o.W
                print("tune %-32s M=%-7d %4d->%-4d: %s" % (plan.op_names[i], M, o.Cin, o.Cout, " ".join("(%d,%d%s)%.1fus" % (p, c, "," + lib.CONV_VARIANT_NAMES[k] if k > lib.CONV_GENERIC else "", t * 1e3) for t, p, c, k in results)))
        pt, ct, tk = best
        if pool1:
            if (pt, ct) != (o.tile_p, o.tile_c):
                o.tile_p, o.tile_c = pt, ct
                changed += 1
            continue
        if (pt, ct, tk) != (o.tile_p, o.tile_c, max(1, o.tile_k)):
            wp, bp = packed(plan, i, *r["raw"][:2], ct, tk)
            plan._tuned += [wp, bp]
            o.tile_p, o.tile_c, o.tile_k, o.w, o.bias = pt, ct, tk, wp.data_ptr(), bp.data_ptr()
            if twin:
                wp2, bp2 = packed(plan, i, *twin["raw"], ct, tk)
                plan._tuned += [wp2, bp2]
                o.aux[1], o.aux[2] = wp2.data_ptr(), bp2.data_ptr()
            changed += 1
    if changed:
        L.maf_engine_destroy(plan._engine)
        h = C.c_void_p()
        lib.check(L.maf_engine_create(plan.ops, len(plan.ops), C.byref(h)))
        plan._engine = h
    torch.cuda.synchronize(plan.device)
    return changed
```

Baseline: 17370.

## Chain a bottleneck's one_conv and the block's conv2 1x1 convs into one kernel

Adds a chain1x1 HIP kernel that computes a bottleneck's 3c-to-c one_conv with SiLU, keeps the result in registers, and feeds it straight into the block's concat 1x1 conv2 alongside the other concat slots. Both weight sets are staged into LDS through global_load_lds, and per-wave tiles are double-buffered. The aim is to remove one launch and the global write and re-read of the intermediate concat slot. In exchange it needs a large LDS footprint, which limits occupancy. It is only used when enabled by the environment setting or when the tuner measures it as faster than the two-launch pair.

```diff
diff --git a/include/mafyolo_hip.h b/include/mafyolo_hip.h
--- a/include/mafyolo_hip.h
+++ b/include/mafyolo_hip.h
@@ -26,7 +26,8 @@
        MAF_OP_CONV1DW = 7,
        MAF_OP_HEADTAIL = 8,
        MAF_OP_STEM2 = 9,
-       MAF_OP_CONV3X3S2_DGRAD = 10 };
+       MAF_OP_CONV3X3S2_DGRAD = 10,
+       MAF_OP_CHAIN1X1 = 11 };
 enum { MAF_CONV_GENERIC = 1,
        MAF_CONV_LDS = 2,
        MAF_CONV_STREAM = 3,
@@ -88,6 +89,7 @@
 int64_t maf_mprep_wreg_record_bytes(int32_t Cin, int32_t Cout, int32_t C1);
 int64_t maf_conv3s2_wreg_record_bytes(int32_t Cin, int32_t Cout);
 int maf_conv1x1_stats_supported(int32_t ksteps, int32_t tile_c);
+int maf_chain1x1_supported(int32_t c, int32_t mid, int32_t c_out, int32_t n_slots);
 
 int maf_op_launch(const maf_op_t* op, maf_stream_t stream);
 
diff --git a/maf-yolo_amd/config.py b/maf-yolo_amd/config.py
--- a/maf-yolo_amd/config.py
+++ b/maf-yolo_amd/config.py
@@ -4,6 +4,7 @@
     "dw_stage":          ("MAF_DW_STAGE", True, "tuner: offer dwconv_p2's staged-store form (tile_k + 128) as a candidate"),
     "fuse_mprep":        ("MAF_FUSE_MPREP", True, "MPRep's two branches as one launch where the kernel exists (tuned plans)"),
     "fuse_tail":         ("MAF_FUSE_TAIL", 1, "what Model.fuse_tail = 'auto' means: 0 off, 1 blocks of one bottleneck (default), 3 every instantiation (s / m opt-in)"),
+    "chain_1x1":         ("MAF_CHAIN_1X1", "auto", "what Model.chain_1x1 = 'auto' means: 0 the two launches, 1 the chained one_conv + conv2 wherever its kernel exists, auto = the tuner's measurement in tuned plans"),
     "split_cat":         ("MAF_SPLIT_CAT", True, "RepHDW behind the fused stem: one dense tensor per concat slot"),
     "mprep_wreg_min":    ("MAF_MPREP_WREG_MIN", 65536, "output pixels from which MPRep takes the register-weight 3x3 kernel"),
     "head_tail_256_max": ("MAF_HEAD_TAIL_256_MAX", 16384, "largest level (B * H * W pixels) whose 256-channel head runs as the fused tail (weights streamed through LDS per 16-pixel unit)"),
diff --git a/maf-yolo_amd/csrc/capi.hip b/maf-yolo_amd/csrc/capi.hip
--- a/maf-yolo_amd/csrc/capi.hip
+++ b/maf-yolo_amd/csrc/capi.hip
@@ -36,6 +36,7 @@
         case MAF_OP_CONV1DW: return maf_launch_conv1dw(op, s);
         case MAF_OP_HEADTAIL: return maf_launch_head_tail(op, s);
         case MAF_OP_STEM2: return maf_launch_stem2(op, s);
+        case MAF_OP_CHAIN1X1: return maf_launch_chain1x1(op, s);
         default: maf_set_error("maf_op_launch: unknown op kind"); return MAF_E_UNSUPPORTED;
     }
 }
diff --git a/maf-yolo_amd/csrc/chain1x1.hip b/maf-yolo_amd/csrc/chain1x1.hip
--- /dev/null
+++ b/maf-yolo_amd/csrc/chain1x1.hip
@@ -0,0 +1,233 @@
+#include "conv_stream_lds.inc.h"
+
+namespace {
+
+struct ChArgs {
+    const half_t* t2;
+    int t2s, t2c;
+    const half_t* x[3];
+    int xs[3], xc[3];
+    const unsigned char* rec;
+    half_t* out;
+    int out_stride, out_coff;
+    int M, nN;
+};
+
+__device__ __forceinline__ float ch_silu(float x) {
+    float v = maf_act<MAF_ACT_SILU>(x);
+    asm("" : "+v"(v));
+    return v;
+}
+
+template <int CT>
+__device__ __forceinline__ void ch_store(const f32x4_t (&acc)[CT], int r, half_t* op) {
+    uint32_t w[CT / 2];
+#pragma unroll
+    for (int c2 = 0; c2 < CT / 2; ++c2) {
+        const half2_t h = {(half_t)ch_silu(acc[2 * c2][r]), (half_t)ch_silu(acc[2 * c2 + 1][r])};
+        w[c2] = __builtin_bit_cast(uint32_t, h);
+    }
+    if constexpr (CT == 8) *reinterpret_cast<u32x4_t*>(op) = (u32x4_t){w[0], w[1], w[2], w[3 % (CT / 2)]};
+    else { *reinterpret_cast<u32x2_t*>(op) = (u32x2_t){w[0], w[1]}; *reinterpret_cast<uint32_t*>(op + 4) = w[2 % (CT / 2)]; }
+}
+
+template <int C, int NS, int CT, int NW>
+__global__ __launch_bounds__(NW * 64) void chain1x1_kernel(const ChArgs a) {
+    typedef Frag<half_t> F;
+    typedef F::type frag_t;
+    constexpr int KS1 = 3 * C / 32, T1 = C / 16, KY = C / 32, KX = (NS - 1) * KY, KS2 = KX + KY;
+    constexpr int N1 = KS1 * T1, N2 = KS2 * CT, NSTEP = N1 + N2;
+    static_assert(NSTEP * 1024 <= 160 * 1024, "both weight sets must fit LDS");
+    extern __shared__ __attribute__((aligned(16))) unsigned char wl_raw[];
+    const int tid = threadIdx.x, wave = tid >> 6, lane = tid & 63, g = lane >> 4, p = lane & 15;
+    const int nwg = gridDim.x / a.nN;
+    int n_tile, wg;
+    if ((nwg & 7) == 0) {
+        const int j = blockIdx.x >> 3;
+        n_tile = j % a.nN;
+        wg = (int)(blockIdx.x & 7) + 8 * (j / a.nN);
+    } else {
+        n_tile = blockIdx.x % a.nN;
+        wg = blockIdx.x / a.nN;
+    }
+    const int ntiles = (a.M + 15) >> 4;
+    {
+        const unsigned char* w2src = a.rec;
+        const unsigned char* w3src = a.rec + (size_t)(N1 + n_tile * N2) * 1024;
+        for (int f = wave; f < NSTEP; f += NW) {
+            const unsigned char* src;
+            if (f < N1) {
+                const int ks = f / T1, t = f - ks * T1;
+                src = w2src + (size_t)(t * KS1 + ks) * 1024;
+            } else {
+                const int f2 = f - N1, ks = f2 / CT, ct = f2 - ks * CT;
+                src = w3src + (size_t)(ct * KS2 + ks) * 1024;
+            }
+            __builtin_amdgcn_global_load_lds((const void __attribute__((address_space(1)))*)(src + lane * 16),
+                                             (void __attribute__((address_space(3)))*)(wl_raw + f * 1024), 16, 0, 0);
+        }
+    }
+    const float* b2 = reinterpret_cast<const float*>(a.rec + (size_t)(N1 + a.nN * N2) * 1024);
+    const float* b3 = b2 + C;
+    f32x4_t bias1[T1];
+#pragma unroll
+    for (int t = 0; t < T1; ++t) bias1[t] = *reinterpret_cast<const f32x4_t*>(b2 + 16 * t + 4 * g);
+    const int cl = n_tile * (16 * CT) + p * CT;
+    float bias2[CT];
+#pragma unroll
+    for (int ct = 0; ct < CT; ++ct) bias2[ct] = b3[cl + ct];
+
+    auto load_tile = [&](int t, frag_t (&ft)[KS1], frag_t (&fx)[KX]) {
+        int m = t * 16 + p;
+        m = m < a.M ? m : a.M - 1;
+        const half_t* q = a.t2 + (size_t)m * a.t2s + a.t2c + g * 8;
+#pragma unroll
+        for (int ks = 0; ks < KS1; ++ks) ft[ks] = ldg16<half_t>(q + ks * 32);
+#pragma unroll
+        for (int j = 0; j < NS - 1; ++j) {
+            const half_t* qx = a.x[j] + (size_t)m * a.xs[j] + a.xc[j] + g * 8;
+#pragma unroll
+            for (int k = 0; k < KY; ++k) fx[j * KY + k] = ldg16<half_t>(qx + k * 32);
+        }
+    };
+    uint32_t wbase[3];
+#pragma unroll
+    for (int k = 0; k < 3; ++k) wbase[k] = (uint32_t)(uintptr_t)(const __attribute__((address_space(3))) void*)(wl_raw + k * 65536 + lane * 16);
+
+    auto compute_store = [&](int t, const frag_t (&ft)[KS1], const frag_t (&fx)[KX]) {
+        f32x4_t acc1[T1], acc2[CT];
+        frag_t a2[KY];
+#pragma unroll
+        for (int i = 0; i < T1; ++i) acc1[i] = bias1[i];
+#pragma unroll
+        for (int ct = 0; ct < CT; ++ct) acc2[ct] = (f32x4_t){bias2[ct], bias2[ct], bias2[ct], bias2[ct]};
+        constexpr int RD = 6;
+        u32x4_t wr[RD + 1];
+        auto ld_step = [&](auto idx) {
+            constexpr int s_ = decltype(idx)::value;
+            if constexpr (s_ < NSTEP) sl_ds_read_b128<(s_ * 1024) % 65536>(wr[s_ % (RD + 1)], wbase[(s_ * 1024) / 65536]);
+        };
+        asm volatile("s_waitcnt lgkmcnt(0)" ::: "memory");
+        sl_static_for<RD>([&](auto idx) { ld_step(idx); });
+        sl_static_for<NSTEP>([&](auto idx) {
+            constexpr int s_ = decltype(idx)::value, sl = s_ % (RD + 1);
+            ld_step(std::integral_constant<int, s_ + RD>{});
+            constexpr int ahead = (NSTEP - 1 - s_) < RD ? (NSTEP - 1 - s_) : RD;
+            if constexpr (s_ == N1) {
+#pragma unroll
+                for (int j = 0; j < KY; ++j)
+#pragma unroll
+                    for (int r = 0; r < 4; ++r) {
+                        a2[j][r] = (half_t)ch_silu(acc1[2 * j][r]);
+                        a2[j][4 + r] = (half_t)ch_silu(acc1[2 * j + 1][r]);
+                    }
+            }
+            sl_wait_lgkm<ahead>(wr[sl]);
+            const frag_t wf = __builtin_bit_cast(frag_t, wr[sl]);
+            if constexpr (s_ < N1) {
+                constexpr int ks = s_ / T1, i = s_ % T1;
+                acc1[i] = F::mma(wf, ft[ks], acc1[i]);
+            } else {
+                constexpr int ks = (s_ - N1) / CT, ct = (s_ - N1) % CT;
+                if constexpr (ks < KX) acc2[ct] = F::mma(fx[ks], wf, acc2[ct]);
+                else acc2[ct] = F::mma(a2[ks - KX], wf, acc2[ct]);
+            }
+            __builtin_amdgcn_sched_barrier(0);
+        });
+#pragma unroll
+        for (int r = 0; r < 4; ++r) {
+            const int m = t * 16 + g * 4 + r;
+            if (m >= a.M) continue;
+            ch_store<CT>(acc2, r, a.out + (size_t)m * a.out_stride + a.out_coff + cl);
+        }
+    };
+
+    frag_t ta[KS1], xa[KX];
+    const int stride = nwg * NW;
+    int t = wg * NW + wave;
+    const bool any = t < ntiles;
+    if (any) load_tile(t, ta, xa);
+    asm volatile("s_waitcnt vmcnt(0)" ::: "memory");
+    __syncthreads();
+    if (!any) return;
+    frag_t tb[KS1], xb[KX];
+    while (true) {
+        const int t1 = t + stride;
+        load_tile(t1, tb, xb);
+        compute_store(t, ta, xa);
+        if (t1 >= ntiles) break;
+        const int t2 = t1 + stride;
+        load_tile(t2, ta, xa);
+        compute_store(t1, tb, xb);
+        if (t2 >= ntiles) break;
+        t = t2;
+    }
+}
+
+template <int C, int NS, int CT>
+int launch_chain(const ChArgs& a, int per_forced, hipStream_t s) {
+    constexpr int NW = 4;
+    constexpr int lds = (3 * C / 32 * (C / 16) + NS * (C / 32) * CT) * 1024;
+    static int occ = 0;
+    if (!occ) {
+        if (lds > 64 * 1024) {
+            int rc = maf_check_hip(hipFuncSetAttribute(reinterpret_cast<const void*>(&chain1x1_kernel<C, NS, CT, NW>), hipFuncAttributeMaxDynamicSharedMemorySize, lds), "hipFuncSetAttribute(chain1x1)");
+            if (rc) return rc;
+        }
+        int nb = 0;
+        int rc = maf_check_hip(hipOccupancyMaxActiveBlocksPerMultiprocessor(&nb, chain1x1_kernel<C, NS, CT, NW>, NW * 64, lds), "hipOccupancyMaxActiveBlocksPerMultiprocessor(chain1x1)");
+        if (rc) return rc;
+        occ = nb < 1 ? 1 : nb > 4 ? 4 : nb;
+    }
+    const int ntiles = (a.M + 15) >> 4;
+    const int most = (ntiles + NW - 1) / NW;
+    int per = most;
+    if (per_forced > 0) per = per_forced < most ? per_forced : most;
+    else {
+        const int cap = occ * 256 / a.nN > 0 ? occ * 256 / a.nN : 1;
+        if (per > cap) per = cap;
+    }
+    if (per >= 8 && a.nN > 1) per &= ~7;
+    hipLaunchKernelGGL((chain1x1_kernel<C, NS, CT, NW>), dim3(per * a.nN), dim3(NW * 64), lds, s, a);
+    return maf_check_hip(hipGetLastError(), "chain1x1 launch");
+}
+
+int chain_ct(int c) { return c == 64 ? 8 : c == 96 ? 6 : 0; }
+
+}
+
+extern "C" int maf_chain1x1_supported(int32_t c, int32_t mid, int32_t c_out, int32_t n_slots) {
+    if (c <= 0 || c % 32 != 0 || !chain_ct(c)) return 0;
+    if (mid != 3 * c || c_out != 2 * c || n_slots < 3 || n_slots > 4) return 0;
+    const int ct = chain_ct(c);
+    return (mid / 32 * (c / 16) + n_slots * (c / 32) * ct) * 1024 <= 160 * 1024 ? 1 : 0;
+}
+
+int maf_launch_chain1x1(const maf_op_t* op, hipStream_t s) {
+    MAF_REQUIRE(op->dtype == MAF_F16, "chain1x1: fp16 only");
+    const int c = op->nc, mid = op->Cin, c_out = op->Cout, ns = op->nsrc;
+    if (!maf_chain1x1_supported(c, mid, c_out, ns)) {
+        maf_set_error("chain1x1: no kernel for this shape (nc = c in {64, 96}, Cin = 3c, Cout = 2c, nsrc = slots in {3, 4}: both weight sets must fit the LDS)");
+        return MAF_E_UNSUPPORTED;
+    }
+    MAF_REQUIRE(op->act == MAF_ACT_SILU && !op->out_f32 && !op->out_pairs, "chain1x1: SiLU, fp16 NHWC output");
+    MAF_REQUIRE(op->w && op->out && op->B > 0 && op->H > 0 && op->W > 0 && (long long)op->B * op->H * op->W < (1ll << 31), "chain1x1: null pointer / bad dims");
+    MAF_REQUIRE(op->tile_c == 0 || op->tile_c == chain_ct(c), "chain1x1: tile_c = 0 or the channel tile of the width (8 for c = 64, 6 for c = 96)");
+    MAF_REQUIRE(op->tile_p == 0 || op->tile_p == 4, "chain1x1: tile_p = waves per workgroup: 0 / 4");
+    MAF_REQUIRE(op->tile_k >= 0, "chain1x1: tile_k = workgroups per channel tile (0 = the launcher's choice)");
+    ChArgs a = {};
+    for (int i = 0; i < ns; ++i) {
+        const maf_src_t& sr = op->src[i];
+        MAF_REQUIRE(sr.ptr && sr.mode == MAF_SRC_DIRECT && sr.C == (i ? c : mid) && sr.stride % 8 == 0 && sr.coff % 8 == 0 && sr.coff >= 0 && sr.coff + sr.C <= sr.stride,
+                    "chain1x1: src[0] = T2 (3c channels), src[1..] = the concat slots in front of y (c channels each); direct, 16-byte aligned");
+        if (i == 0) { a.t2 = static_cast<const half_t*>(sr.ptr); a.t2s = sr.stride; a.t2c = sr.coff; }
+        else { a.x[i - 1] = static_cast<const half_t*>(sr.ptr); a.xs[i - 1] = sr.stride; a.xc[i - 1] = sr.coff; }
+    }
+    MAF_REQUIRE(op->out_stride % 2 == 0 && op->out_coff % 8 == 0 && op->out_coff >= 0 && op->out_coff + c_out <= op->out_stride && op->out_stride % 8 == 0, "chain1x1: output slice must be 16-byte aligned inside its row");
+    a.rec = static_cast<const unsigned char*>(op->w);
+    a.out = static_cast<half_t*>(op->out); a.out_stride = op->out_stride; a.out_coff = op->out_coff;
+    a.M = op->B * op->H * op->W;
+    a.nN = c_out / (16 * chain_ct(c));
+    if (c == 64) return ns == 3 ? launch_chain<64, 3, 8>(a, op->tile_k, s) : launch_chain<64, 4, 8>(a, op->tile_k, s);
+    return ns == 3 ? launch_chain<96, 3, 6>(a, op->tile_k, s) : launch_chain<96, 4, 6>(a, op->tile_k, s);
+}
diff --git a/maf-yolo_amd/csrc/maf_common.h b/maf-yolo_amd/csrc/maf_common.h
--- a/maf-yolo_amd/csrc/maf_common.h
+++ b/maf-yolo_amd/csrc/maf_common.h
@@ -33,6 +33,7 @@
 int maf_launch_conv1dw(const maf_op_t* op, hipStream_t s);
 int maf_launch_head_tail(const maf_op_t* op, hipStream_t s);
 int maf_launch_stem2(const maf_op_t* op, hipStream_t s);
+int maf_launch_chain1x1(const maf_op_t* op, hipStream_t s);
 int maf_launch_conv3s2_lds(const maf_op_t* op, hipStream_t s);
 int maf_launch_conv3s2_wreg(const maf_op_t* op, hipStream_t s);
 int maf_dw_wgrad_mfma(const void* x, int x_stride, const void* dy, int dy_stride, int B, int H, int W, int C, int k, float* dw, int replicas, hipStream_t s);
diff --git a/maf-yolo_amd/engine.py b/maf-yolo_amd/engine.py
--- a/maf-yolo_amd/engine.py
+++ b/maf-yolo_amd/engine.py
@@ -11,7 +11,7 @@
 
 
 from .conv_variants import stream_lds_ok
-from .tuner import _TUNE_CACHE, choose_fusion, save_tune_cache, load_tune_cache, p2_wave_bytes
+from .tuner import _TUNE_CACHE, choose_fusion, choose_chain, save_tune_cache, load_tune_cache, p2_wave_bytes
 from . import tuner as _tuner, plan_report as _report
 
 _TORCH_DT = {lib.F16: torch.float16, lib.F32: torch.float32}
@@ -44,7 +44,7 @@
 
 
 class Plan:
-    def __init__(self, model, B, Hin, Win, dtype, in_dtype, device, fuse=None, fuse_head=None, fuse_tail=None):
+    def __init__(self, model, B, Hin, Win, dtype, in_dtype, device, fuse=None, fuse_head=None, fuse_tail=None, chain=None):
         assert Hin % 32 == 0 and Win % 32 == 0, "image sides must be multiples of 32 (stride of P5)"
         self.B, self.Hin, self.Win, self.dtype, self.in_dtype, self.device = B, Hin, Win, dtype, in_dtype, device
         self.es = _ESIZE[dtype]
@@ -67,6 +67,10 @@
         env_ft = str(cfg.fuse_tail)
         deep = 3 if env_ft == "3" else 1
         self.fuse_tail = (deep if ft == "auto" else 3 if ft else 0) if (env_ft != "0" and dtype == lib.F16) else 0
+        if chain is None:
+            ch = getattr(model, "chain_1x1", "auto")
+            chain = (str(cfg.chain_1x1) == "1") if ch in ("auto", "tune") else bool(ch)
+        self.chain = chain if dtype == lib.F16 else False
         self.split_cat = bool(getattr(model, "split_cat", cfg.split_cat))
         self.lanes = getattr(model, "multi_stream", False)
         if isinstance(self.lanes, bool):
@@ -203,7 +207,11 @@
                 tail = (depth <= self.fuse_tail and self._fuse_mode("%s.m.%d" % (p, depth - 1), kl, c_) == 1 and 2 <= depth + 1 <= 3
                         and m.conv2.fused()[0].shape[1] == (depth + 2) * c_
                         and lib.load().maf_bottleneck_tail_supported(kl, c_, depth + 1, node.cout) == 1)
-                nslot = depth + 1 if tail else depth + 2
+                ql = "%s.m.%d" % (p, depth - 1)
+                chain = (not tail and (self.chain is True or (isinstance(self.chain, dict) and ql in self.chain)) and self._fuse_mode(ql, kl, c_) in (0, 2)
+                         and m.conv2.fused()[0].shape[1] == (depth + 2) * c_
+                         and lib.load().maf_chain1x1_supported(c_, m.m[-1].conv1.conv.out_channels, node.cout, depth + 2) == 1)
+                nslot = depth + 1 if (tail or chain) else depth + 2
                 if split:
                     slot = [(self._alloc(x.H, x.W, c_), 0) for _ in range(nslot)]
                 else:
@@ -233,14 +241,16 @@
                                               tail_c3=node.cout, raw=_raw(*blk.conv1.fused(), *blk.conv2.fused(), *blk.one_conv.fused(), w3, b3),
                                               w=self._wput(rec), b=self._wput(b2p), aux=[self._wput(pack.pack_bottleneck_tail(w3, b3, c_, depth + 1))]))
                         continue
-                    (ob, oc) = slot[d + 2]
+                    last = chain and d == depth - 1
+                    (ob, oc) = (None, 0) if last else slot[d + 2]
                     if mode == 2:
                         rec, nmb = pack.pack_conv1dw(*blk.conv1.fused(), *blk.conv2.fused())
                         t2 = self._alloc(x.H, x.W, mid)
                         self._ops.append(dict(kind=lib.OP_CONV1DW, name=q + ".conv1dw", act=lib.ACT_SILU, H=x.H, W=x.W, Cin=c_, Cout=mid,
                                               ksize=blk.conv2.dwconv.kernel_size, segs=[Seg(ib, c_, ic)], out=t2, out_coff=0, raw=_raw(*blk.conv1.fused(), *blk.conv2.fused()), w=self._wput(rec),
                                               b=self._wput(torch.zeros(8))))
-                        self._conv1x1(q + ".one_conv", *blk.one_conv.fused(), TV([Seg(t2, mid)], x.H, x.W), ob, oc, lib.ACT_SILU)
+                        if not last:
+                            self._conv1x1(q + ".one_conv", *blk.one_conv.fused(), TV([Seg(t2, mid)], x.H, x.W), ob, oc, lib.ACT_SILU)
                         continue
                     if mode == 1:
                         rec, b2p, nmb, ct2 = pack.pack_bottleneck(*blk.conv1.fused(), *blk.conv2.fused(), *blk.one_conv.fused())
@@ -253,8 +263,17 @@
                     t1, t2 = self._alloc(x.H, x.W, mid), self._alloc(x.H, x.W, mid)
                     self._conv1x1(q + ".conv1", *blk.conv1.fused(), TV([Seg(ib, c_, ic)], x.H, x.W), t1, 0, lib.ACT_SILU)
                     self._dw(q + ".conv2", *blk.conv2.fused(), TV([Seg(t1, mid)], x.H, x.W), t2, lib.ACT_SILU)
-                    self._conv1x1(q + ".one_conv", *blk.one_conv.fused(), TV([Seg(t2, mid)], x.H, x.W), ob, oc, lib.ACT_SILU)
-                if not tail:
+                    if not last:
+                        self._conv1x1(q + ".one_conv", *blk.one_conv.fused(), TV([Seg(t2, mid)], x.H, x.W), ob, oc, lib.ACT_SILU)
+                if chain:
+                    (w2_, b2_), (w3, b3) = m.m[-1].one_conv.fused(), m.conv2.fused()
+                    ct = pack.chain1x1_tile_c(c_)
+                    out = self._alloc(x.H, x.W, node.cout)
+                    tl = self.chain.get(ql, (0, 0, 0)) if isinstance(self.chain, dict) else (0, 0, 0)
+                    self._ops.append(dict(kind=lib.OP_CHAIN1X1, name=ql + ".one_conv+conv2", act=lib.ACT_SILU, H=x.H, W=x.W, Cin=mid, Cout=node.cout, slot_c=c_,
+                                          segs=[Seg(t2, mid)] + [Seg(b_, c_, co_) for b_, co_ in slot], out=out, out_coff=0, pt=tl[0], ct=tl[1], tk=tl[2],
+                                          raw=_raw(w2_, b2_, w3, b3), w=self._wput(pack.pack_chain1x1(w2_, b2_, w3, b3, c_, depth + 2, ct)), b=0))
+                elif not tail:
                     out = self._alloc(x.H, x.W, node.cout)
                     cat_tv = TV([Seg(b_, c_, 0) for b_, _ in slot], x.H, x.W) if split else TV([Seg(cat, c_ * (depth + 2))], x.H, x.W)
                     self._conv1x1(p + ".conv2", *m.conv2.fused(), cat_tv, out, 0, lib.ACT_SILU)
@@ -470,6 +489,8 @@
             if r["kind"] == lib.OP_BOTTLENECK:
                 o.tile_k = r["tk"]
                 o.nc = r.get("tail_c3", 0)
+            if r["kind"] == lib.OP_CHAIN1X1:
+                o.tile_k, o.nc = r["tk"], r["slot_c"]
             if "pool1" in r:
                 o.tile_k, o.nc, o.reg_stride = r.get("pool1_tk", lib.CONV3_LDS), r["pool1"][0].shape[0], 0
             for k_, off in enumerate(r.get("aux", [])):
diff --git a/maf-yolo_amd/lib.py b/maf-yolo_amd/lib.py
--- a/maf-yolo_amd/lib.py
+++ b/maf-yolo_amd/lib.py
@@ -14,7 +14,7 @@
 NMS_SINGLE_LAUNCH = 2
 ACT_NONE, ACT_RELU, ACT_SILU, ACT_SIGMOID = 0, 1, 2, 3
 SRC_DIRECT, SRC_UP2, SRC_POOL2, SRC_SUB2, SRC_PAIRS = 0, 1, 2, 3, 4
-OP_STEM, OP_CONV1X1, OP_CONV3X3S2, OP_DWCONV, OP_SPPF_POOL, OP_DECODE, OP_BOTTLENECK, OP_CONV1DW, OP_HEADTAIL, OP_STEM2, OP_CONV3X3S2_DGRAD = range(11)
+OP_STEM, OP_CONV1X1, OP_CONV3X3S2, OP_DWCONV, OP_SPPF_POOL, OP_DECODE, OP_BOTTLENECK, OP_CONV1DW, OP_HEADTAIL, OP_STEM2, OP_CONV3X3S2_DGRAD, OP_CHAIN1X1 = range(12)
 CONV_GENERIC, CONV_LDS, CONV_STREAM, CONV_SPLITK, CONV_STREAM_LDS, CONV3_LDS, CONV3_WREG, CONV_DMA = range(1, 9)
 CONV_VARIANT_NAMES = {CONV_GENERIC: "generic", CONV_LDS: "lds", CONV_STREAM: "stream", CONV_SPLITK: "k4", CONV_STREAM_LDS: "streamlds", CONV3_LDS: "ldsall",
                       CONV3_WREG: "wreg", CONV_DMA: "dma"}
@@ -121,7 +121,7 @@
 
 
 EXPORTS = ["maf_last_error", "maf_version", "maf_op_size", "maf_op_launch", "maf_engine_create", "maf_engine_num_ops",
-           "maf_engine_run", "maf_engine_run_filtered", "maf_engine_run_graph", "maf_engine_run_timed", "maf_engine_destroy", "maf_nms_workspace_bytes", "maf_nms", "maf_nms_ex", "maf_nms_debug", "maf_pack_w1x1_bytes", "maf_pack_w1x1", "maf_pack_dw", "maf_pack_batch", "maf_pack_desc_size", "maf_ema_update", "maf_ema_desc_size", "maf_sgd_update", "maf_sgd_desc_size", "maf_nonfinite_check", "maf_range_desc_size", "maf_maxpool_forward", "maf_maxpool_backward", "maf_upsample2x_forward", "maf_upsample2x_backward", "maf_zero", "maf_grad_fold", "maf_add_sub2", "maf_colsum", "maf_dw_wgrad", "maf_dw_wgrad31", "maf_stem_train", "maf_image_to_nhwc8", "maf_bottleneck_record_bytes", "maf_bottleneck_tail_record_bytes", "maf_bottleneck_tail_supported", "maf_conv1dw_record_bytes", "maf_head_tail_record_bytes", "maf_stem2_record_bytes", "maf_conv3s2_lds_record_bytes", "maf_mprep_lds_record_bytes", "maf_mprep_wreg_record_bytes", "maf_conv3s2_wreg_record_bytes", "maf_conv1x1_stats_supported", "maf_coco_rows", "maf_conv1x1_wgrad", "maf_conv_wgrad", "maf_bn_forward", "maf_bn_backward", "maf_bn_backward_acc", "maf_set_deterministic", "maf_dw_branches", "maf_dw_branches_stats", "maf_bn_forward_ex", "maf_bn_replicas", "maf_bn_stats", "maf_bn_sum_forward", "maf_bn_sum_forward_stats", "maf_bn_sum_backward", "maf_tal_targets", "maf_tal_assign", "maf_atss_assign", "maf_loss_partial_rows", "maf_loss_decode", "maf_loss_terms",
+           "maf_engine_run", "maf_engine_run_filtered", "maf_engine_run_graph", "maf_engine_run_timed", "maf_engine_destroy", "maf_nms_workspace_bytes", "maf_nms", "maf_nms_ex", "maf_nms_debug", "maf_pack_w1x1_bytes", "maf_pack_w1x1", "maf_pack_dw", "maf_pack_batch", "maf_pack_desc_size", "maf_ema_update", "maf_ema_desc_size", "maf_sgd_update", "maf_sgd_desc_size", "maf_nonfinite_check", "maf_range_desc_size", "maf_maxpool_forward", "maf_maxpool_backward", "maf_upsample2x_forward", "maf_upsample2x_backward", "maf_zero", "maf_grad_fold", "maf_add_sub2", "maf_colsum", "maf_dw_wgrad", "maf_dw_wgrad31", "maf_stem_train", "maf_image_to_nhwc8", "maf_bottleneck_record_bytes", "maf_bottleneck_tail_record_bytes", "maf_bottleneck_tail_supported", "maf_conv1dw_record_bytes", "maf_head_tail_record_bytes", "maf_stem2_record_bytes", "maf_conv3s2_lds_record_bytes", "maf_mprep_lds_record_bytes", "maf_mprep_wreg_record_bytes", "maf_conv3s2_wreg_record_bytes", "maf_conv1x1_stats_supported", "maf_chain1x1_supported", "maf_coco_rows", "maf_conv1x1_wgrad", "maf_conv_wgrad", "maf_bn_forward", "maf_bn_backward", "maf_bn_backward_acc", "maf_set_deterministic", "maf_dw_branches", "maf_dw_branches_stats", "maf_bn_forward_ex", "maf_bn_replicas", "maf_bn_stats", "maf_bn_sum_forward", "maf_bn_sum_forward_stats", "maf_bn_sum_backward", "maf_tal_targets", "maf_tal_assign", "maf_atss_assign", "maf_loss_partial_rows", "maf_loss_decode", "maf_loss_terms",
            "maf_detect_join", "maf_detect_join_backward", "maf_nhwc_sum", "maf_stream_fork", "maf_stream_join", "maf_tape_fn_id", "maf_tape_fn_nargs", "maf_tape_rec_size", "maf_tape_run", "maf_tape_toggle",
            "maf_stream_create_masked", "maf_stream_destroy", "maf_letterbox", "maf_letterbox_lds_bytes", "maf_rescale_boxes",
            "maf_augment_resize", "maf_mosaic_affine", "maf_augment_sample_size", "maf_area_struct_sizes", "maf_resize_area",
@@ -202,6 +202,8 @@
     lib.maf_bn_replicas.restype = C.c_int32
     lib.maf_conv1x1_stats_supported.argtypes = [C.c_int32, C.c_int32]
     lib.maf_conv1x1_stats_supported.restype = C.c_int
+    lib.maf_chain1x1_supported.argtypes = [C.c_int32] * 4
+    lib.maf_chain1x1_supported.restype = C.c_int
     lib.maf_coco_rows.argtypes = [C.c_void_p, C.c_void_p, C.c_int32, C.c_int32, C.c_void_p, C.c_void_p, C.c_int32, C.c_void_p, C.c_void_p, C.c_void_p]
     lib.maf_conv1dw_record_bytes.argtypes = [C.c_int32] * 2
     lib.maf_conv1dw_record_bytes.restype = C.c_int64
diff --git a/maf-yolo_amd/model.py b/maf-yolo_amd/model.py
--- a/maf-yolo_amd/model.py
+++ b/maf-yolo_amd/model.py
@@ -123,6 +123,7 @@
         self.fuse_stem = True
         self.fuse_head = "auto"
         self.fuse_tail = "auto"
+        self.chain_1x1 = "auto"
         self.fuse_mprep = "auto"
         self.twin_convs = True
         self.autotune = False
@@ -341,7 +342,7 @@
         else:
             dt = lib.F32 if x.dtype == torch.float32 else lib.F16
         fuse_head = bool(getattr(self, "fuse_head", True)) and not head_feats
-        key = (B, H, W, dt, in_dt, x.device.index, fuse_head, slot, repr(getattr(self, "fuse_stem", True)), repr(self.fuse_bottlenecks), repr(getattr(self, "fuse_tail", "auto")), self.multi_stream, bool(getattr(self, "twin_convs", True)))
+        key = (B, H, W, dt, in_dt, x.device.index, fuse_head, slot, repr(getattr(self, "fuse_stem", True)), repr(self.fuse_bottlenecks), repr(getattr(self, "fuse_tail", "auto")), repr(getattr(self, "chain_1x1", "auto")), self.multi_stream, bool(getattr(self, "twin_convs", True)))
         ver = self.weights_version()
         if ver != self._plans_version:
             self._plans = {}
@@ -354,7 +355,11 @@
             if self.autotune and dt == lib.F16 and self.fuse_bottlenecks == "auto":
                 from .engine import choose_fusion
                 fuse = choose_fusion(self, B, H, W, dt, in_dt, x.device, x.contiguous())
-            plan = Plan(self, B, H, W, dt, in_dt, x.device, fuse=fuse, fuse_head=fuse_head)
+            chain = None
+            if self.autotune and dt == lib.F16 and getattr(self, "chain_1x1", "auto") in ("auto", "tune") and str(cfg.chain_1x1) == "auto":
+                from .engine import choose_chain
+                chain = choose_chain(self, B, H, W, dt, in_dt, x.device, x.contiguous(), fuse, fuse_head, measure=self.chain_1x1 == "tune")
+            plan = Plan(self, B, H, W, dt, in_dt, x.device, fuse=fuse, fuse_head=fuse_head, chain=chain)
             if self.autotune and dt == lib.F16:
                 plan.autotune(x.contiguous())
             self._plans[key] = plan
diff --git a/maf-yolo_amd/pack.py b/maf-yolo_amd/pack.py
--- a/maf-yolo_amd/pack.py
+++ b/maf-yolo_amd/pack.py
@@ -224,6 +224,29 @@
     return rec
 
 
+def chain1x1_tile_c(c):
+    return {64: 8, 96: 6}[c]
+
+
+def chain1x1_y_rows(c):
+    t, g, r = torch.meshgrid(torch.arange(c // 16), torch.arange(4), torch.arange(4), indexing="ij")
+    return (32 * (t // 2) + 8 * g + 4 * (t % 2) + r).reshape(-1)
+
+
+def pack_chain1x1(w2, b2, w3, b3, c, n_slots, tile_c):
+    w2 = w2.detach().float().cpu().reshape(w2.shape[0], -1)
+    w3 = w3.detach().float().cpu().reshape(w3.shape[0], -1)
+    mid, c_out = w2.shape[1], w3.shape[0]
+    assert w2.shape[0] == c and c % 32 == 0 and mid % 32 == 0 and w3.shape[1] == n_slots * c and c_out % (16 * tile_c) == 0
+    rows = chain1x1_y_rows(c)
+    f1 = w2[rows].view(c // 16, 16, mid // 32, 4, 8).permute(0, 2, 3, 1, 4).contiguous().half()
+    f2 = pack_matrix([w3], tile_c, lib.F16)
+    rec = torch.cat([f1.reshape(-1).view(torch.uint8), f2.reshape(-1).view(torch.uint8),
+                     b2.detach().float().cpu()[rows].contiguous().view(torch.uint8), b3.detach().float().cpu().contiguous().view(torch.uint8)])
+    assert rec.numel() == 2 * mid * c + 2 * n_slots * c * c_out + 4 * c + 4 * c_out
+    return rec
+
+
 def pack_stem2(w0, b0, w1, b1, w3=None, b3=None):
     w0 = w0.detach().float().cpu(); w1 = w1.detach().float().cpu()
     C0, C1 = w0.shape[0], w1.shape[0]
diff --git a/maf-yolo_amd/plan_report.py b/maf-yolo_amd/plan_report.py
--- a/maf-yolo_amd/plan_report.py
+++ b/maf-yolo_amd/plan_report.py
@@ -42,6 +42,8 @@
         return "head_tail_kernel<%d, %d>" % (o.Cin, 2 if o.Cin <= 128 else 1)
     if o.kind == lib.OP_STEM2:
         return "stem2_kernel<%d, %d, %d>" % (o.ksize, o.Cout, o.nc)
+    if o.kind == lib.OP_CHAIN1X1:
+        return "chain1x1_kernel<%d, %d, %d, 4>" % (o.nc, o.nsrc, pack.chain1x1_tile_c(o.nc))
     return {lib.OP_STEM: "stem_kernel", lib.OP_SPPF_POOL: "sppf_pool_lds_kernel", lib.OP_DECODE: "decode_kernel"}[o.kind]
 
 def algorithmic_bytes(plan, idx):
@@ -74,6 +76,8 @@
         if o.nc:
             return px * (o.nsrc * o.Cin + o.nc) * es + wts + (o.nsrc + 1) * o.Cin * o.nc * es
         return px * (o.Cin + o.Cout) * es + wts
+    if o.kind == lib.OP_CHAIN1X1:
+        return px * (o.Cin + (o.nsrc - 1) * o.nc + o.Cout) * es + (o.Cin * o.nc + o.nsrc * o.nc * o.Cout) * es
     if o.kind == lib.OP_SPPF_POOL:
         return 4 * px * o.src[0].C * es
     if o.kind == lib.OP_HEADTAIL:
@@ -101,6 +105,8 @@
     if o.kind == lib.OP_BOTTLENECK:
         mid = plan._ops[idx]["mid"]
         return 2 * px * (o.Cin * mid + o.ksize * o.ksize * mid + mid * o.Cout + (o.nsrc + 1) * o.Cin * o.nc)
+    if o.kind == lib.OP_CHAIN1X1:
+        return 2 * px * (o.Cin * o.nc + o.nsrc * o.nc * o.Cout)
     if o.kind == lib.OP_HEADTAIL:
         return 2 * px * (2 * o.Cin * o.Cin + o.Cin * (plan.nc + 4 * (plan.reg_max + 1)))
     return 0
diff --git a/maf-yolo_amd/tuner.py b/maf-yolo_amd/tuner.py
--- a/maf-yolo_amd/tuner.py
+++ b/maf-yolo_amd/tuner.py
@@ -39,6 +39,66 @@
             _TUNE_CACHE[sigs[n]] = (min(cost, key=cost.get),)
     del plan1
     return {n: _TUNE_CACHE[sigs[n]][0] for n in names}
+
+
+def chain_signature(dtype, B, o):
+    return ("chain", dtype, B, o.H, o.W, o.nc, o.Cin, o.Cout, o.nsrc)
+
+
+def chain_tiles(o):
+    ntile = -(-(o.B * o.H * o.W) // 16)
+    nN = o.Cout // (16 * pack.chain1x1_tile_c(o.nc))
+    out = [(4, pack.chain1x1_tile_c(o.nc), 0)]
+    for per in (512 // nN, 384 // nN, 256 // nN, 128 // nN):
+        if per < -(-ntile // 4) and (4, out[0][1], per) not in out:
+            out.append((4, out[0][1], per))
+    return out
+
+
+def choose_chain(model, B, H, W, dtype, in_dtype, device, x, fuse=None, fuse_head=None, reps=5, verbose=False, measure=True):
+    import numpy as np
+    from .engine import Plan
+    if not measure and not any(k[0] == "chain" for k in _TUNE_CACHE):
+        return {}
+    plan1 = Plan(model, B, H, W, dtype, in_dtype, device, fuse=fuse, fuse_head=fuse_head, chain=True)
+    idx = [i for i, o in enumerate(plan1.ops) if o.kind == lib.OP_CHAIN1X1]
+    sigs = {plan1.op_names[i]: chain_signature(dtype, B, plan1.ops[i]) for i in idx}
+    if measure and idx and not all(s_ in _TUNE_CACHE for s_ in sigs.values()):
+        L = lib.load()
+        pred = torch.empty(B, plan1.A, 5 + plan1.nc, dtype=torch.float32, device=device)
+
+        def timed(plan):
+            plan.run_timed(x, pred)
+            return dict(zip(plan.op_names, np.min([plan.run_timed(x, pred) for _ in range(reps)], 0)))
+        plan0 = Plan(model, B, H, W, dtype, in_dtype, device, fuse=fuse, fuse_head=fuse_head, chain=False)
+        plan0.autotune(x)
+        t0 = timed(plan0)
+        del plan0
+        plan1.autotune(x)
+        best = {}
+        for tiles in sorted({t_ for i in idx for t_ in chain_tiles(plan1.ops[i])}):
+            on = [i for i in idx if tiles in chain_tiles(plan1.ops[i])]
+            for i in on:
+                plan1.ops[i].tile_p, plan1.ops[i].tile_c, plan1.ops[i].tile_k = tiles
+            L.maf_engine_destroy(plan1._engine)
+            h = C.c_void_p()
+            lib.check(L.maf_engine_create(plan1.ops, len(plan1.ops), C.byref(h)))
+            plan1._engine = h
+            t1 = timed(plan1)
+            for i in on:
+                nm = plan1.op_names[i]
+                if nm not in best or t1[nm] < best[nm][0]:
+                    best[nm] = (t1[nm], tiles)
+        for i in idx:
+            nm = plan1.op_names[i]
+            q = nm[:-len(".one_conv+conv2")]
+            pair = t0[q + ".one_conv"] + t0[q[:q.index(".m.")] + ".conv2"]
+            _TUNE_CACHE[sigs[nm]] = ((1,) + best[nm][1]) if best[nm][0] < pair else (0, 0, 0, 0)
+            if verbose:
+                print("chain %-34s pair %.1fus chained %.1fus %r" % (nm, pair * 1e3, best[nm][0] * 1e3, best[nm][1]))
+    names = list(sigs)
+    del plan1
+    return {n[:-len(".one_conv+conv2")]: tuple(_TUNE_CACHE[sigs[n]][1:]) for n in names if _TUNE_CACHE.get(sigs[n], (0,))[0]}
 
 
 def save_tune_cache(path):
```

Result: slower. 17070 (-1.7%).
